# linkedin/gdmix

Hardware: AMD Instinct MI355X
Metric: random-effect entities converged/sec (higher is better)
Workload: dtype f64; 1 GPU; C2: synthetic 1000000 entities/GPU x avg 64 nnz (n~max(1,Poisson(16)), k=4 distinct uniform columns of D=1024, SURVEY 8(d) generator), per-entity L2 LR, L-BFGS m=10; build_id=8021e6e25780712a, workload_key=c2, entities_per_gpu=1000000, step=pack+solve, theta on device, parallelism=entity-shard x1

## Files before the change

gdmix_amd/csrc/re_api.hip:

```cpp
#include <stdarg.h>
#include <stdio.h>
#include <stdlib.h>
#include <string.h>
#include <time.h>

#include <errno.h>
#include <fcntl.h>
#include <sys/file.h>
#include <sys/stat.h>
#include <unistd.h>

#include <condition_variable>
#include <map>
#include <new>
#include <string>

#include <mutex>

#include "re_internal.hpp"
#include "re_solve_team.hpp"

namespace gdmix {

static thread_local char g_err[512] = "";

void set_error(const char* fmt, ...) {
  va_list ap;
  va_start(ap, fmt);
  vsnprintf(g_err, sizeof(g_err), fmt, ap);
  va_end(ap);
}

bool loss_code_ok(int code, const char* who) {
  if (code == GDMIX_RE_LOSS_LOGISTIC || code == GDMIX_RE_LOSS_SQUARED || code == GDMIX_RE_LOSS_POISSON) return true;
  set_error("%s: opts->loss = %d is no loss code (GDMIX_RE_LOSS_LOGISTIC 0, GDMIX_RE_LOSS_SQUARED 1, GDMIX_RE_LOSS_POISSON 2)", who, code);
  return false;
}

__global__ __launch_bounds__(WAVE) void publish_kernel(const uint32_t* __restrict__ src, int words, uint32_t* box_data, uint32_t* box_flag, uint32_t seq) {
  for (int i = threadIdx.x; i < words; i += WAVE) __hip_atomic_store(box_data + i, src[i], __ATOMIC_RELAXED, __HIP_MEMORY_SCOPE_SYSTEM);
  asm volatile("s_waitcnt vmcnt(0)" ::: "memory");
  if (threadIdx.x == 0) __hip_atomic_store(box_flag, seq, __ATOMIC_RELAXED, __HIP_MEMORY_SCOPE_SYSTEM);
}

static inline void cpu_relax() {
#if !defined(__HIP_DEVICE_COMPILE__)
  asm volatile("pause" ::: "memory");
#endif
}

static int mailbox_on() {
  static const int on = [] { const char* e = getenv("GDMIX_RE_MAILBOX"); return (e && atoi(e) == 0) ? 0 : 1; }();
  return on;
}

hipError_t post_small(gdmix_ctx_impl* ctx, int box, const void* dev_src, size_t bytes, void* host_dst, hipStream_t s, SmallFetch* f) {
  f->box = -1; f->seq = 0; f->bytes = bytes; f->host_dst = host_dst; f->s = s;
  if (!mailbox_on() || bytes % 4 || bytes > MAILBOX_BYTES - MAILBOX_DATA || box < 0 || box >= 4)
    return hipMemcpyAsync(host_dst, dev_src, bytes, hipMemcpyDeviceToHost, s);
  char* const base = reinterpret_cast<char*>(ctx->host_pinned) + MAILBOX_OFFSET + (size_t)box * MAILBOX_BYTES;
  uint32_t seq = ++ctx->mail_seq[box];
  if (seq == 0) seq = ++ctx->mail_seq[box];
  hipLaunchKernelGGL(publish_kernel, dim3(1), dim3(WAVE), 0, s, static_cast<const uint32_t*>(dev_src), (int)(bytes / 4),
                     reinterpret_cast<uint32_t*>(base + MAILBOX_DATA), reinterpret_cast<uint32_t*>(base), seq);
  f->box = box; f->seq = seq;
  return hipGetLastError();
}

hipError_t wait_small(gdmix_ctx_impl* ctx, const SmallFetch& f) {
  if (f.box < 0) return hipStreamSynchronize(f.s);
  char* const base = reinterpret_cast<char*>(ctx->host_pinned) + MAILBOX_OFFSET + (size_t)f.box * MAILBOX_BYTES;
  uint32_t* const flag = reinterpret_cast<uint32_t*>(base);
  timespec t0, t1;
  clock_gettime(CLOCK_MONOTONIC, &t0);
  while (__atomic_load_n(flag, __ATOMIC_ACQUIRE) != f.seq) {
    for (int k = 0; k < 16; ++k) cpu_relax();
    clock_gettime(CLOCK_MONOTONIC, &t1);
    if ((t1.tv_sec - t0.tv_sec) * 1000000L + (t1.tv_nsec - t0.tv_nsec) / 1000L > FETCH_SPIN_US) {
      hipError_t rc = hipStreamSynchronize(f.s);
      if (rc != hipSuccess) return rc;
      if (__atomic_load_n(flag, __ATOMIC_ACQUIRE) != f.seq) return hipErrorUnknown;
      break;
    }
  }
  memcpy(f.host_dst, base + MAILBOX_DATA, f.bytes);
  return hipSuccess;
}

}

using namespace gdmix;


namespace gdmix {
namespace {
constexpr int GATE_DEVICES = 64;
std::mutex g_gate_mu[GATE_DEVICES];
hipEvent_t g_gate_ev[GATE_DEVICES] = {};
bool g_gate_armed[GATE_DEVICES] = {};
}

class GridLock {
 public:
  explicit GridLock(const std::string& base) : base_(base) {}
  bool acquire() {
    std::unique_lock<std::mutex> g(mu_);
    if (!open_files()) return false;
    for (;;) {
      if (state_ == HELD) {
        if (!somebody_waits()) { ++count_; ++rides_; return true; }
        cv_.wait(g);
      } else if (state_ == ACQUIRING) {
        cv_.wait(g);
      } else {
        state_ = ACQUIRING;
        g.unlock();
        const bool ok = flock_retry(turn_fd_, LOCK_EX) && flock_retry(dev_fd_, LOCK_EX);
        flock_retry(turn_fd_, LOCK_UN);
        g.lock();
        if (!ok) { state_ = FREE; cv_.notify_all(); return false; }
        state_ = HELD;
        count_ = 1;
        ++takes_;
        cv_.notify_all();
        return true;
      }
    }
  }
  void release() {
    std::lock_guard<std::mutex> g(mu_);
    if (state_ != HELD || count_ <= 0) return;
    if (--count_ == 0) {
      flock_retry(dev_fd_, LOCK_UN);
      state_ = FREE;
      cv_.notify_all();
    }
  }
  void stats(long* takes, long* rides) {
    std::lock_guard<std::mutex> g(mu_);
    *takes = takes_;
    *rides = rides_;
  }

 private:
  enum State { FREE, ACQUIRING, HELD };
  static bool flock_retry(int fd, int op) {
    int rc;
    do rc = flock(fd, op); while (rc != 0 && errno == EINTR);
    return rc == 0;
  }
  static int open_one(const std::string& path) {
    const int fd = open(path.c_str(), O_RDWR | O_CREAT | O_CLOEXEC, 0666);
    if (fd >= 0) (void)fchmod(fd, 0666);
    return fd;
  }
  bool open_files() {
    if (dev_fd_ >= 0) return true;
    if (failed_) return false;
    dev_fd_ = open_one(base_ + ".lock");
    turn_fd_ = open_one(base_ + ".turn");
    probe_fd_ = open_one(base_ + ".turn");
    if (dev_fd_ < 0 || turn_fd_ < 0 || probe_fd_ < 0) {
      fprintf(stderr, "gdmix_re: cannot open %s.lock (%s): persistent grids of several processes on this device are not chained\n", base_.c_str(), strerror(errno));
      for (int* fd : {&dev_fd_, &turn_fd_, &probe_fd_}) { if (*fd >= 0) close(*fd); *fd = -1; }
      failed_ = true;
      return false;
    }
    return true;
  }
  bool somebody_waits() {
    if (flock(probe_fd_, LOCK_SH | LOCK_NB) == 0) { flock_retry(probe_fd_, LOCK_UN); return false; }
    return errno == EWOULDBLOCK;
  }
  std::string base_;
  std::mutex mu_;
  std::condition_variable cv_;
  State state_ = FREE;
  int count_ = 0, dev_fd_ = -1, turn_fd_ = -1, probe_fd_ = -1;
  bool failed_ = false;
  long takes_ = 0, rides_ = 0;
};

namespace {
std::mutex g_locks_mu;
std::map<std::string, GridLock*> g_locks;
GridLock* g_dev_lock[GATE_DEVICES] = {};
hipStream_t g_rel_stream[GATE_DEVICES] = {};
bool g_dev_lock_off[GATE_DEVICES] = {};

GridLock* grid_lock_by_key(const char* key) {
  std::lock_guard<std::mutex> g(g_locks_mu);
  auto it = g_locks.find(key);
  if (it != g_locks.end()) return it->second;
  const char* dir = getenv("GDMIX_RE_LOCK_DIR");
  std::string base = std::string(dir && *dir ? dir : "/tmp") + "/gdmix_re_grid_";
  for (const char* c = key; *c; ++c) base += (isalnum((unsigned char)*c) || *c == '.' || *c == '-') ? *c : '_';
  return g_locks[key] = new GridLock(base);
}

GridLock* grid_lock_of_device(int device) {
  if (g_dev_lock_off[device]) return nullptr;
  if (g_dev_lock[device]) return g_dev_lock[device];
  const char* e = getenv("GDMIX_RE_GRID_LOCK");
  char bus[64] = "";
  if ((e && atoi(e) == 0) || hipDeviceGetPCIBusId(bus, sizeof(bus), device) != hipSuccess || !bus[0] ||
      hipStreamCreateWithFlags(&g_rel_stream[device], hipStreamNonBlocking) != hipSuccess) {
    g_dev_lock_off[device] = true;
    return nullptr;
  }
  return g_dev_lock[device] = grid_lock_by_key(bus);
}

void grid_lock_release_cb(void* p) { static_cast<GridLock*>(p)->release(); }

std::mutex g_here_mu;
std::map<std::string, int> g_here_fd;

int presence_fd(int device) {
  char bus[64] = "";
  if (hipDeviceGetPCIBusId(bus, sizeof(bus), device) != hipSuccess || !bus[0]) return -1;
  std::lock_guard<std::mutex> g(g_here_mu);
  auto it = g_here_fd.find(bus);
  if (it != g_here_fd.end()) return it->second;
  const char* dir = getenv("GDMIX_RE_LOCK_DIR");
  std::string path = std::string(dir && *dir ? dir : "/tmp") + "/gdmix_re_grid_";
  for (const char* c = bus; *c; ++c) path += (isalnum((unsigned char)*c) || *c == '.' || *c == '-') ? *c : '_';
  path += ".here";
  const int fd = open(path.c_str(), O_RDWR | O_CREAT | O_CLOEXEC, 0666);
  if (fd >= 0) {
    (void)fchmod(fd, 0666);
    struct flock fl = {};
    fl.l_type = F_RDLCK; fl.l_whence = SEEK_SET; fl.l_start = 0; fl.l_len = 1;
    (void)fcntl(fd, F_SETLK, &fl);
  }
  return g_here_fd[bus] = fd;
}
}

void device_register_process(int device) {
  const char* e = getenv("GDMIX_RE_GRID_LOCK");
  if (!(e && atoi(e) == 0)) (void)presence_fd(device);
}

bool device_has_another_process(int device) {
  const char* e = getenv("GDMIX_RE_GRID_LOCK");
  if (e && atoi(e) == 0) return false;
  const int fd = presence_fd(device);
  if (fd < 0) return false;
  struct flock fl = {};
  fl.l_type = F_WRLCK; fl.l_whence = SEEK_SET; fl.l_start = 0; fl.l_len = 1;
  return fcntl(fd, F_GETLK, &fl) == 0 && fl.l_type != F_UNLCK;
}

ScopedGridGate::ScopedGridGate(int device, hipStream_t s) : device_(device >= 0 && device < GATE_DEVICES ? device : 0), s_(s), err_(hipSuccess), held_(nullptr) {
  g_gate_mu[device_].lock();
  if (!g_gate_ev[device_]) err_ = hipEventCreateWithFlags(&g_gate_ev[device_], hipEventDisableTiming);
  if (err_ == hipSuccess && g_gate_armed[device_]) err_ = hipStreamWaitEvent(s_, g_gate_ev[device_], 0);
  if (err_ == hipSuccess) {
    GridLock* const L = grid_lock_of_device(device_);
    if (L && L->acquire()) held_ = L;
  }
}

ScopedGridGate::~ScopedGridGate() {
  const bool recorded = g_gate_ev[device_] && hipEventRecord(g_gate_ev[device_], s_) == hipSuccess;
  if (recorded) g_gate_armed[device_] = true;
  if (held_) {
    GridLock* const L = static_cast<GridLock*>(held_);
    if (!(recorded && hipStreamWaitEvent(g_rel_stream[device_], g_gate_ev[device_], 0) == hipSuccess &&
          hipLaunchHostFunc(g_rel_stream[device_], grid_lock_release_cb, L) == hipSuccess)) {
      (void)hipStreamSynchronize(s_);
      L->release();
    }
  }
  g_gate_mu[device_].unlock();
}
}

extern "C" {

static int spread_default() {
  const char* e = getenv("GDMIX_RE_SPREAD");
  const int n = e ? atoi(e) : 4;
  return n > 1 ? n : 0;
}
GDMIX_API int gdmix_re_abi_version(void) { return GDMIX_RE_ABI_VERSION; }

GDMIX_API int gdmix_re_grid_lock_acquire(const char* key) {
  if (!key || !*key) { set_error("key is empty"); return GDMIX_RE_EINVAL; }
  return grid_lock_by_key(key)->acquire() ? GDMIX_RE_OK : GDMIX_RE_EINVAL;
}
GDMIX_API int gdmix_re_grid_lock_release(const char* key) {
  if (!key || !*key) { set_error("key is empty"); return GDMIX_RE_EINVAL; }
  grid_lock_by_key(key)->release();
  return GDMIX_RE_OK;
}
GDMIX_API int gdmix_re_grid_lock_stats(const char* key, int64_t* takes, int64_t* rides) {
  if (!key || !*key || !takes || !rides) { set_error("bad argument"); return GDMIX_RE_EINVAL; }
  long t = 0, r = 0;
  grid_lock_by_key(key)->stats(&t, &r);
  *takes = t;
  *rides = r;
  return GDMIX_RE_OK;
}

GDMIX_API const char* gdmix_re_last_error(void) { return g_err; }

GDMIX_API void gdmix_re_default_opts(gdmix_re_opts* o) {
  if (!o) return;
  o->l2 = 1.0; o->regularize_bias = 1; o->has_intercept = 1; o->m = 10; o->max_iter = 100;
  o->maxfun = 15000; o->maxls = 20; o->ftol = 1e-12; o->pgtol = 1e-5;
  o->variance_mode = GDMIX_RE_VAR_NONE; o->threshold = 1e-4;
  o->sum_loss = 0; o->loss = 0;
}

GDMIX_API int gdmix_re_create(int hip_device, gdmix_re_ctx** out) {
  if (!out) { set_error("out is NULL"); return GDMIX_RE_EINVAL; }
  *out = nullptr;
  int count = 0;
  HIP_TRY(hipGetDeviceCount(&count));
  if (hip_device < 0 || hip_device >= count) {
    set_error("HIP device %d not present (%d visible)", hip_device, count);
    return GDMIX_RE_EHIP;
  }
  HIP_TRY(hipSetDevice(hip_device));
  hipDeviceProp_t prop;
  HIP_TRY(hipGetDeviceProperties(&prop, hip_device));
  if (strncmp(prop.gcnArchName, "gfx950", 6) != 0) {
    set_error("device %d is %s; this library only carries gfx950 (MI355X) code", hip_device, prop.gcnArchName);
    return GDMIX_RE_EHIP;
  }
  gdmix_re_ctx* c = new (std::nothrow) gdmix_re_ctx();
  if (!c) { set_error("out of host memory"); return GDMIX_RE_ENOMEM; }
  c->impl.device = hip_device;
  c->impl.num_cus = prop.multiProcessorCount;
  device_register_process(hip_device);
  c->impl.tall_adapt_limit = c->impl.num_cus * 3 / 2;
  if (const char* e = getenv("GDMIX_RE_TALL_ADAPT")) c->impl.tall_adapt_limit = atoi(e) > 0 ? atoi(e) : 0;
  c->impl.scratch = nullptr;
  c->impl.scratch_bytes = 0;
  c->impl.host_pinned = nullptr;
  c->impl.wave_lds_limit = 65536;
  c->impl.kernel_mask = 7;
  c->impl.timing = 0;
  c->impl.giant_nnz = 16777216;
  c->impl.team_nnz = 16384;
  c->impl.tall_min_n = GDMIX_RE_TALL_MIN_N_DEFAULT;
  c->impl.tall_split_n = GDMIX_RE_TALL_SPLIT_N_DEFAULT;
  c->impl.tall_split_set = 0;
  c->impl.tall_team_n = GDMIX_RE_TALL_TEAM_N_DEFAULT;
  c->impl.tall_team_limit = c->impl.num_cus / 4 < TALL_TEAM_MAX ? c->impl.num_cus / 4 : TALL_TEAM_MAX;
  c->impl.tall_mid_n = 0;
  if (const char* e = getenv("GDMIX_RE_TALL_MID")) { if (atoi(e) == 1) c->impl.tall_mid_n = -(c->impl.num_cus * TALL_MID_WGS); else if (atoi(e) > 1) c->impl.tall_mid_n = -atoi(e); }
  if (c->impl.num_cus < 8 * TALL_TEAM_C) c->impl.tall_team_n = 0;
  if (const char* e = getenv("GDMIX_RE_TALL_TEAM")) { if (atoi(e) == 0) c->impl.tall_team_n = 0; }
  if (const char* e = getenv("GDMIX_RE_TALL_TEAM_LIMIT")) { if (atoi(e) > 0 && atoi(e) <= TALL_TEAM_MAX) c->impl.tall_team_limit = atoi(e); }
  c->impl.spread = spread_default();
  c->impl.narrow = 1;
  if (const char* e = getenv("GDMIX_RE_NARROW")) c->impl.narrow = atoi(e) != 0 ? 1 : 0;
  c->impl.grid_sync = nullptr;
  c->impl.big_tmp = nullptr;
  c->impl.big_tmp_bytes = 0;
  c->impl.eval_small_set = 0; c->impl.eval_small_max = 64;
  c->impl.eval_tmp = nullptr; c->impl.eval_tmp_bytes = 0;
  c->impl.sel_small_set = 0; c->impl.sel_small_max = 1024; c->impl.sel_plan_ws = nullptr;
  c->impl.cap_small_set = 0; c->impl.cap_small_max = 128; c->impl.cap_plan_ws = nullptr;
  c->impl.n_side = 0; c->impl.side_fork = nullptr;
  c->impl.aux_ev[0] = c->impl.aux_ev[1] = nullptr;
  c->impl.defer_unique = 0; c->impl.unique_pending = false; c->impl.unique_ev = nullptr;
  for (int k = 0; k < gdmix_ctx_impl::MAX_SIDE; ++k) { c->impl.side[k] = nullptr; c->impl.side_join[k] = nullptr; }
  for (int k = 0; k < GDMIX_RE_NUM_CLASSES; ++k) { c->impl.ev0[k] = nullptr; c->impl.ev1[k] = nullptr; c->impl.ev_used[k] = false; }
  for (uint32_t& q : c->impl.mail_seq) q = 0;
  hipError_t rc = hipHostMalloc(reinterpret_cast<void**>(&c->impl.host_pinned), HOST_PINNED_BYTES, hipHostMallocMapped | hipHostMallocCoherent);
  if (rc == hipSuccess) memset(c->impl.host_pinned, 0, HOST_PINNED_BYTES);
  if (rc != hipSuccess) {
    set_error("hipHostMalloc failed: %s", hipGetErrorString(rc));
    delete c;
    return GDMIX_RE_EHIP;
  }
  {
    const char* e = getenv("GDMIX_RE_SIDE_STREAM");
    int want = e ? atoi(e) : 3;
    if (want > gdmix_ctx_impl::MAX_SIDE) want = gdmix_ctx_impl::MAX_SIDE;
    if (want > 0) {
      rc = hipEventCreateWithFlags(&c->impl.side_fork, hipEventDisableTiming);
      for (int k = 0; k < 2 && rc == hipSuccess; ++k) rc = hipEventCreateWithFlags(&c->impl.aux_ev[k], hipEventDisableTiming);
      if (rc == hipSuccess) rc = hipEventCreateWithFlags(&c->impl.unique_ev, hipEventDisableTiming);
      for (int k = 0; k < want && rc == hipSuccess; ++k) {
        rc = hipStreamCreateWithFlags(&c->impl.side[k], hipStreamNonBlocking);
        if (rc == hipSuccess) rc = hipEventCreateWithFlags(&c->impl.side_join[k], hipEventDisableTiming);
        if (rc == hipSuccess) c->impl.n_side = k + 1;
      }
      if (rc != hipSuccess) {
        set_error("creating the side streams failed: %s", hipGetErrorString(rc));
        gdmix_re_destroy(c);
        return GDMIX_RE_EHIP;
      }
    }
  }
  rc = hipMalloc(&c->impl.grid_sync, GridSyncLayout::BYTES);
  if (rc != hipSuccess) {
    set_error("hipMalloc failed: %s", hipGetErrorString(rc));
    (void)hipHostFree(c->impl.host_pinned);
    delete c;
    return GDMIX_RE_EHIP;
  }
  *out = c;
  return GDMIX_RE_OK;
}

GDMIX_API void gdmix_re_destroy(gdmix_re_ctx* ctx) {
  if (!ctx) return;
  if (ctx->impl.unique_pending && ctx->impl.unique_ev) (void)hipEventSynchronize(ctx->impl.unique_ev);
  if (ctx->impl.unique_ev) (void)hipEventDestroy(ctx->impl.unique_ev);
  if (ctx->impl.grid_sync) (void)hipFree(ctx->impl.grid_sync);
  if (ctx->impl.big_tmp) (void)hipFree(ctx->impl.big_tmp);
  if (ctx->impl.eval_tmp) (void)hipFree(ctx->impl.eval_tmp);
  if (ctx->impl.host_pinned) (void)hipHostFree(ctx->impl.host_pinned);
  if (ctx->impl.side_fork) (void)hipEventDestroy(ctx->impl.side_fork);
  for (int k = 0; k < 2; ++k) if (ctx->impl.aux_ev[k]) (void)hipEventDestroy(ctx->impl.aux_ev[k]);
  for (int k = 0; k < gdmix_ctx_impl::MAX_SIDE; ++k) {
    if (ctx->impl.side_join[k]) (void)hipEventDestroy(ctx->impl.side_join[k]);
    if (ctx->impl.side[k]) (void)hipStreamDestroy(ctx->impl.side[k]);
  }
  for (int k = 0; k < GDMIX_RE_NUM_CLASSES; ++k) {
    if (ctx->impl.ev0[k]) (void)hipEventDestroy(ctx->impl.ev0[k]);
    if (ctx->impl.ev1[k]) (void)hipEventDestroy(ctx->impl.ev1[k]);
  }
  delete ctx;
}

GDMIX_API size_t gdmix_re_pack_workspace_bytes(int64_t E, int64_t N, int64_t Z) {
  if (E < 0 || N < 0 || Z < 0) return 0;
  return pack_workspace_bytes(E, N, Z);
}

GDMIX_API int gdmix_re_pack(gdmix_re_ctx* ctx, const gdmix_re_raw_batch* raw_dev, int has_intercept, void* workspace,
                  size_t workspace_bytes, gdmix_re_packed* out, void* stream) {
  if (!ctx || !raw_dev || !out || (!workspace && workspace_bytes)) { set_error("NULL argument"); return GDMIX_RE_EINVAL; }
  if (raw_dev->E > 0 && (!raw_dev->ent_row_ptr || !raw_dev->row_nnz_ptr || !raw_dev->y || !raw_dev->offset)) {
    set_error("raw batch has NULL arrays");
    return GDMIX_RE_EINVAL;
  }
  if (raw_dev->Z > 0 && (!raw_dev->col_global || !raw_dev->val)) { set_error("raw batch has NULL arrays"); return GDMIX_RE_EINVAL; }
  HIP_TRY(hipSetDevice(ctx->impl.device));
  HIP_TRY(join_unique(&ctx->impl, static_cast<hipStream_t>(stream)));
  return pack_impl(&ctx->impl, raw_dev, has_intercept, workspace, workspace_bytes, out, static_cast<hipStream_t>(stream));
}

GDMIX_API int gdmix_re_set_defer_unique(gdmix_re_ctx* ctx, int enabled) {
  if (!ctx) { set_error("ctx is NULL"); return GDMIX_RE_EINVAL; }
  ctx->impl.defer_unique = (enabled && ctx->impl.n_side > 0) ? 1 : 0;
  return GDMIX_RE_OK;
}

GDMIX_API int gdmix_re_pack_join(gdmix_re_ctx* ctx, void* stream) {
  if (!ctx) { set_error("ctx is NULL"); return GDMIX_RE_EINVAL; }
  HIP_TRY(hipSetDevice(ctx->impl.device));
  HIP_TRY(join_unique(&ctx->impl, static_cast<hipStream_t>(stream)));
  return GDMIX_RE_OK;
}

static int slots_for(const gdmix_re_packed* b, const gdmix_re_opts* o, size_t* slot_doubles) {
  *slot_doubles = block_slot_doubles(b->max_p, b->max_n, o->m);
  size_t bytes = *slot_doubles * 8;
  size_t by_budget = ((size_t)4 << 30) / (bytes ? bytes : 1);
  size_t slots = 1024;
  if (slots > by_budget) slots = by_budget;
  if (slots < 8) slots = 8;
  if ((int64_t)slots > b->E) slots = (size_t)(b->E > 0 ? b->E : 1);
  return (int)slots;
}

static int64_t var_small_p(const gdmix_re_packed* b) { return b->max_p < VAR_FULL_MAX_P ? b->max_p : VAR_FULL_MAX_P; }

static int var_slots_for(const gdmix_re_packed* b) {
  size_t bytes = var_full_slot_doubles(var_small_p(b)) * 8;
  size_t slots = ((size_t)2 << 30) / (bytes ? bytes : 1);
  if (slots > 2048) slots = 2048;
  if (slots < 4) slots = 4;
  slots &= ~(size_t)3;
  return (int)slots;
}

GDMIX_API size_t gdmix_re_solve_scratch_bytes(const gdmix_re_packed* batch, const gdmix_re_opts* opts) {
  if (!batch || !opts || batch->E == 0) return 0;
  size_t slot_doubles;
  int slots = slots_for(batch, opts, &slot_doubles);
  size_t need = (size_t)slots * slot_doubles * 8;
  if (opts->variance_mode == GDMIX_RE_VAR_FULL && batch->max_p <= VAR_FULL_BIG_MAX_P) {
    size_t v = (size_t)var_slots_for(batch) * var_full_slot_doubles(var_small_p(batch)) * 8;
    if (v > need) need = v;
    if (batch->max_p > VAR_FULL_MAX_P) {
      v = var_full_big_doubles(batch->max_p, batch->max_n) * 8;
      if (v > need) need = v;
    }
  }
  return need;
}

GDMIX_API int gdmix_re_set_wave_lds_limit(gdmix_re_ctx* ctx, int bytes) {
  if (!ctx || bytes < 0) { set_error("bad argument"); return GDMIX_RE_EINVAL; }
  ctx->impl.wave_lds_limit = bytes > 65536 ? 65536 : bytes;
  return GDMIX_RE_OK;
}

GDMIX_API int gdmix_re_set_kernel_mask(gdmix_re_ctx* ctx, int mask) {
  if (!ctx) { set_error("ctx is NULL"); return GDMIX_RE_EINVAL; }
  ctx->impl.kernel_mask = mask & 7;
  return GDMIX_RE_OK;
}

GDMIX_API int gdmix_re_set_giant_nnz(gdmix_re_ctx* ctx, int64_t nnz) {
  if (!ctx || nnz < 0) { set_error("bad argument"); return GDMIX_RE_EINVAL; }
  ctx->impl.giant_nnz = nnz;
  return GDMIX_RE_OK;
}

GDMIX_API int gdmix_re_set_team_nnz(gdmix_re_ctx* ctx, int64_t nnz) {
  if (!ctx || nnz < 0) { set_error("bad argument"); return GDMIX_RE_EINVAL; }
  ctx->impl.team_nnz = nnz;
  return GDMIX_RE_OK;
}

GDMIX_API int gdmix_re_set_tall_min_n(gdmix_re_ctx* ctx, int min_n) {
  if (!ctx || min_n < 0) { set_error("bad argument"); return GDMIX_RE_EINVAL; }
  ctx->impl.tall_min_n = min_n;
  return GDMIX_RE_OK;
}

GDMIX_API int gdmix_re_set_spread(gdmix_re_ctx* ctx, int queues) {
  if (!ctx || queues < 0) { set_error("bad argument"); return GDMIX_RE_EINVAL; }
  ctx->impl.spread = queues > 1 ? queues : 0;
  return GDMIX_RE_OK;
}

GDMIX_API int gdmix_re_set_narrow(gdmix_re_ctx* ctx, int on) {
  if (!ctx) { set_error("ctx is NULL"); return GDMIX_RE_EINVAL; }
  ctx->impl.narrow = on ? 1 : 0;
  return GDMIX_RE_OK;
}

GDMIX_API int gdmix_re_set_tall_team_n(gdmix_re_ctx* ctx, int team_n) {
  if (!ctx) { set_error("bad argument"); return GDMIX_RE_EINVAL; }
  ctx->impl.tall_team_n = ctx->impl.num_cus < 8 * TALL_TEAM_C ? 0 : team_n;
  return GDMIX_RE_OK;
}

GDMIX_API int gdmix_re_device_shared(gdmix_re_ctx* ctx) {
  if (!ctx) { set_error("ctx is NULL"); return GDMIX_RE_EINVAL; }
  return device_has_another_process(ctx->impl.device) ? 1 : 0;
}

GDMIX_API int gdmix_re_set_tall_mid_n(gdmix_re_ctx* ctx, int mid_n) {
  if (!ctx) { set_error("bad argument"); return GDMIX_RE_EINVAL; }
  ctx->impl.tall_mid_n = mid_n < 0 ? -(ctx->impl.num_cus * TALL_MID_WGS) : mid_n;
  return GDMIX_RE_OK;
}

GDMIX_API int gdmix_re_set_tall_split_n(gdmix_re_ctx* ctx, int split_n) {
  if (!ctx || split_n < 0) { set_error("bad argument"); return GDMIX_RE_EINVAL; }
  ctx->impl.tall_split_n = split_n > 0 ? split_n : GDMIX_RE_TALL_SPLIT_N_DEFAULT;
  ctx->impl.tall_split_set = split_n > 0 ? 1 : 0;
  return GDMIX_RE_OK;
}

GDMIX_API int gdmix_re_set_timing(gdmix_re_ctx* ctx, int enabled) {
  if (!ctx) { set_error("ctx is NULL"); return GDMIX_RE_EINVAL; }
  if (enabled && !ctx->impl.ev0[0]) {
    HIP_TRY(hipSetDevice(ctx->impl.device));
    for (int k = 0; k < GDMIX_RE_NUM_CLASSES; ++k) {
      HIP_TRY(hipEventCreate(&ctx->impl.ev0[k]));
      HIP_TRY(hipEventCreate(&ctx->impl.ev1[k]));
    }
  }
  ctx->impl.timing = enabled ? 1 : 0;
  return GDMIX_RE_OK;
}

GDMIX_API int gdmix_re_last_solve_ms(gdmix_re_ctx* ctx, float* ms_out) {
  if (!ctx || !ms_out) { set_error("NULL argument"); return GDMIX_RE_EINVAL; }
  for (int k = 0; k < GDMIX_RE_NUM_CLASSES; ++k) {
    ms_out[k] = 0.0f;
    if (ctx->impl.ev_used[k]) {
      HIP_TRY(hipEventSynchronize(ctx->impl.ev1[k]));
      HIP_TRY(hipEventElapsedTime(&ms_out[k], ctx->impl.ev0[k], ctx->impl.ev1[k]));
    }
  }
  return GDMIX_RE_OK;
}

GDMIX_API int gdmix_re_set_scratch(gdmix_re_ctx* ctx, void* scratch, size_t bytes) {
  if (!ctx) { set_error("ctx is NULL"); return GDMIX_RE_EINVAL; }
  ctx->impl.scratch = scratch;
  ctx->impl.scratch_bytes = bytes;
  return GDMIX_RE_OK;
}

static int run_variance_full(gdmix_re_ctx* ctx, const gdmix_re_packed* b, const BatchDev& B, const SolveParams& P, const double* theta,
                             double* variance, hipStream_t s) {
  const size_t vslot = var_full_slot_doubles(var_small_p(b));
  int vslots = var_slots_for(b);
  size_t avail = ctx->impl.scratch ? ctx->impl.scratch_bytes : 0;
  void* base = ctx->impl.scratch;
  if (b->scratch_bytes > avail) { avail = b->scratch_bytes; base = b->scratch; }
  if ((size_t)vslots * vslot * 8 > avail) vslots = (int)(avail / (vslot * 8)) & ~3;
  if (vslots < 4) {
    set_error("variance_mode FULL needs >= %zu bytes of scratch (gdmix_re_set_scratch)", 4 * vslot * 8);
    return GDMIX_RE_ENOMEM;
  }
  HIP_TRY(launch_variance_full(B, b->E, P, theta, variance, static_cast<double*>(base), vslot, vslots, var_small_p(b), s));
  if (b->max_p > VAR_FULL_MAX_P) {
    if (var_full_big_doubles(b->max_p, b->max_n) * 8 > avail) {
      set_error("variance_mode FULL with p = %d needs >= %zu bytes of scratch (gdmix_re_set_scratch)", b->max_p,
                var_full_big_doubles(b->max_p, b->max_n) * 8);
      return GDMIX_RE_ENOMEM;
    }
    HIP_TRY(launch_variance_full_big(&ctx->impl, B, b->E, P, theta, variance, static_cast<double*>(base), b->max_p, b->max_n, s));
  }
  return GDMIX_RE_OK;
}

}

namespace {

struct Slots { double* scratch = nullptr; size_t doubles = 0; int n = 0; };

int size_slots(const gdmix_ctx_impl* ci, const gdmix_re_packed* b, const gdmix_re_opts* opts, int n_slot_users, Slots* out) {
  if (n_slot_users <= 0) return GDMIX_RE_OK;
  out->n = slots_for(b, opts, &out->doubles);
  const size_t need = (size_t)out->n * out->doubles * 8;
  if (ci->scratch && ci->scratch_bytes >= need) out->scratch = static_cast<double*>(ci->scratch);
  else if (b->scratch && b->scratch_bytes >= need) out->scratch = static_cast<double*>(b->scratch);
  else {
    size_t avail = ci->scratch ? ci->scratch_bytes : 0;
    void* base = ci->scratch;
    if (b->scratch_bytes > avail) { avail = b->scratch_bytes; base = b->scratch; }
    out->n = (int)(avail / (out->doubles * 8));
    if (out->n < 1) {
      set_error("%d entities need a scratch slot: provide >= %zu bytes via gdmix_re_set_scratch", n_slot_users, out->doubles * 8);
      return GDMIX_RE_ENOMEM;
    }
    out->scratch = static_cast<double*>(base);
  }
  return GDMIX_RE_OK;
}

template <class F>
int timed(gdmix_ctx_impl* ci, int c, hipStream_t s, F&& launch) {
  if (ci->timing) HIP_TRY(hipEventRecord(ci->ev0[c], s));
  const hipError_t rc = launch();
  if (rc != hipSuccess) { set_error("launch of class %d (%s) failed: %s", c, kClasses[c].name, hipGetErrorString(rc)); return GDMIX_RE_EHIP; }
  if (ci->timing) { HIP_TRY(hipEventRecord(ci->ev1[c], s)); ci->ev_used[c] = true; }
  return GDMIX_RE_OK;
}

hipError_t launch_class(const gdmix_ctx_impl* ci, const gdmix_re_packed* b, const BatchDev& B, const OutDev& O, const SolveParams& P,
                        const double* theta0, const Launch& L, int lean_merged, hipStream_t s) {
  const ClassDesc& d = kClasses[L.c];
  switch (d.kind) {
    case KIND_WLDS:
      return launch_solve_wave(B, O, P, theta0, L.begin, L.count, d.lds, s);
    case KIND_TALL_T: {
      const char* xe = getenv("GDMIX_RE_XCD_BARRIER");
      return launch_solve_tall_team(B, O, P, theta0, L.begin, L.count, ci->num_cus, b->Z, GridSyncLayout::tall_tail(ci, d.tall_variant),
                                    GridSyncLayout::tall_team_buf(ci), (xe && atoi(xe) == 0) ? 0 : 1, s);
    }
    case KIND_TALL_L: case KIND_TALL_S: case KIND_TALL_M: case KIND_TALL:
      return launch_solve_tall(d.tall_variant, B, O, P, theta0, L.begin, L.count, ci->num_cus, b->Z, GridSyncLayout::tall_tail(ci, d.tall_variant),
                               GridSyncLayout::tall_ticket(ci, d.tall_variant), d.kind == KIND_TALL_S ? lean_merged : 0, s);
    default: {
      if (d.lanes <= 0) return hipErrorInvalidValue;
      const int nn = (L.c == NARROW_HOST_CLASS && L.narrow > 0) ? (L.narrow < L.count ? L.narrow : L.count) : 0;
      if (hipError_t rc = launch_solve_quad(NARROW_LANES, NARROW_EPL, B, O, P, theta0, L.begin, nn, NARROW_NCAP, NARROW_ZCAP, s); rc != hipSuccess) return rc;
      return launch_solve_quad(d.lanes, d.epl, B, O, P, theta0, L.begin + nn, L.count - nn, d.ncap, d.zcap, s);
    }
  }
}

int team_count(int tier_max, unsigned long long total_nnz, unsigned long long largest_nnz, int entities, int slots, int num_cus) {
  const unsigned long long ratio = largest_nnz ? total_nnz / largest_nnz : 1;
  int teams = 1;
  while (teams * 2 <= tier_max && (unsigned long long)(teams * 2) <= ratio) teams *= 2;
  if (entities <= 16) {
    int want = 1;
    while (want * 2 <= entities && want * 2 <= tier_max && want * 2 <= teams * 4) want *= 2;
    if (want > teams) teams = want;
  }
  if (const char* ev = getenv("GDMIX_RE_TEAMS")) teams = atoi(ev);
  if (teams > TEAM_MAX_TEAMS) teams = TEAM_MAX_TEAMS;
  while (teams > 1 && (slots < teams || num_cus % teams)) teams >>= 1;
// ... 153 lines not shown
```

gdmix_amd/csrc/re_internal.hpp:

```cpp
#pragma once
#include <hip/hip_runtime.h>
#include <stdint.h>
#include <stddef.h>

#include <type_traits>

#include "../../include/gdmix_re.h"
#include "re_solve_core.hpp"
#include "re_solve_wreg.hpp"
#include "re_solve_quad.hpp"

namespace gdmix {

enum { KIND_WREG1 = 0, KIND_WREG2 = 1, KIND_WREG4 = 2, KIND_WLDS = 3, KIND_BLOCK = 4, KIND_QUAD2 = 5, KIND_QUAD4 = 6, KIND_PAIR4 = 7, KIND_QUAD3 = 8, KIND_PAIR3 = 9, KIND_WREG8 = 10,
       KIND_G64_3 = 11, KIND_G64_4 = 12, KIND_G128_4 = 13, KIND_G256_4 = 14, KIND_G512_4 = 15, KIND_GRID = 16, KIND_G128_3 = 17, KIND_G256_3 = 18,
       KIND_TALL = 20, KIND_TALL_S = 21, KIND_TALL_L = 22, KIND_TALL_T = 23, KIND_TALL_M = 24 };

__host__ __device__ constexpr int group_lanes(int kind) {
  return (kind == KIND_QUAD2 || kind == KIND_QUAD3 || kind == KIND_QUAD4) ? 16 : ((kind == KIND_PAIR3 || kind == KIND_PAIR4) ? 32 :
         ((kind == KIND_G64_3 || kind == KIND_G64_4) ? 64 : ((kind == KIND_G128_4 || kind == KIND_G128_3) ? 128 : ((kind == KIND_G256_4 || kind == KIND_G256_3) ? 256 : (kind == KIND_G512_4 ? 512 : 0)))));
}
__host__ __device__ constexpr int group_epl(int kind) {
  return kind == KIND_QUAD2 ? 2 : ((kind == KIND_QUAD3 || kind == KIND_PAIR3 || kind == KIND_G64_3 || kind == KIND_G128_3 || kind == KIND_G256_3) ? 3 : (group_lanes(kind) > 0 ? 4 : 0));
}
// ... 59 lines not shown
    grp_class(KIND_G128_4, 128, 4, 128, 1024, "re_solve_grp_kernel<128,4> n<=128 nnz<=1024"),
    grp_class(KIND_G128_4, 128, 4, 1024, 3072, "re_solve_grp_kernel<128,4> n<=1024 nnz<=3072"),
    grp_class(KIND_G256_3, 256, 3, 256, 2048, "re_solve_grp_kernel<256,3> n<=256 nnz<=2048"),
    grp_class(KIND_G256_3, 256, 3, 2048, 4096, "re_solve_grp_kernel<256,3> n<=2048 nnz<=4096"),
    grp_class(KIND_G256_4, 256, 4, 256, 2048, "re_solve_grp_kernel<256,4> n<=256 nnz<=2048"),
    grp_class(KIND_G256_4, 256, 4, 2048, 4096, "re_solve_grp_kernel<256,4> n<=2048 nnz<=4096"),
    grp_class(KIND_G512_4, 512, 4, 512, 4096, "re_solve_grp_kernel<512,4> n<=512 nnz<=4096"),
    wave_class(24576, "re_solve_wave_kernel lds<=24K"),
    wave_class(65536, "re_solve_wave_kernel lds<=64K"),
    tall_class(KIND_TALL_T, TALL_VARIANT_TEAM, 0, 0, 0, "re_solve_tall_team_kernel<8> x4 p<=64"),
    tall_class(KIND_TALL_L, TALL_VARIANT_LEAN, 4, WAVE, 0, "re_solve_tall_kernel<1> lean p<=64"),
    tall_class(KIND_TALL_S, TALL_VARIANT_SMALL, 3, WAVE, 2, "re_solve_tall_kernel<1> p<=64"),
    tall_class(KIND_TALL_M, TALL_VARIANT_MID, 2, 8 / TALL_MID_WGS * WAVE, -1, "re_solve_tall_kernel<4> p<=64"),
    tall_class(KIND_TALL, TALL_VARIANT_LARGE, 1, 4 * TALL_NW / 8 * WAVE, 1, "re_solve_tall_kernel<8> p<=64"),
    team_class(KIND_BLOCK, "re_solve_team_kernel workgroup"),
    team_class(KIND_GRID, "re_solve_team_kernel 128 teams"),
    team_class(KIND_GRID, "re_solve_team_kernel 32 teams"),
    team_class(KIND_GRID, "re_solve_team_kernel 8 teams"),
    team_class(KIND_GRID, "re_solve_team_kernel device-wide")};
constexpr int class_of_kind(int kind) {
  for (int c = 0; c < GDMIX_RE_NUM_CLASSES; ++c)
    if (kClasses[c].kind == kind) return c;
  return -1;
}
constexpr int TALL_T_CLASS = class_of_kind(KIND_TALL_T);
constexpr int TALL_L_CLASS = class_of_kind(KIND_TALL_L);
constexpr int TALL_S_CLASS = class_of_kind(KIND_TALL_S);
constexpr int TALL_M_CLASS = class_of_kind(KIND_TALL_M);
constexpr int TALL_CLASS = class_of_kind(KIND_TALL);
constexpr int BLOCK_CLASS = class_of_kind(KIND_BLOCK);
constexpr int TEAM128_CLASS = BLOCK_CLASS + 1;
constexpr int TEAM32_CLASS = BLOCK_CLASS + 2;
constexpr int TEAM8_CLASS = BLOCK_CLASS + 3;
constexpr int GIANT_CLASS = BLOCK_CLASS + 4;
constexpr int tall_class_of_rank(int rank) {
  for (int c = 0; c < GDMIX_RE_NUM_CLASSES; ++c)
    if (kClasses[c].tall_rank == rank) return c;
  return -1;
}
constexpr bool class_table_consistent() {
  for (int k = 0; k < TALL_VARIANTS; ++k)
    if (tall_class_of_rank(k) < 0) return false;

  for (int c = 0; c < GDMIX_RE_NUM_CLASSES; ++c) {
    const ClassDesc& d = kClasses[c];
    if (d.lanes != group_lanes(d.kind) || d.epl != group_epl(d.kind)) return false;
    if ((d.tall_variant >= 0) != (c >= TALL_T_CLASS && c < BLOCK_CLASS) || (d.tall_variant >= 0) != (d.tall_rank >= 0)) return false;
    if (c > BLOCK_CLASS && d.kind != KIND_GRID) return false;
    if (c < TALL_T_CLASS && d.lds <= 0) return false;
  }
  return true;
}
static_assert(class_table_consistent(), "group_lanes / group_epl and the class constants describe kClasses");
static_assert(GIANT_CLASS == GDMIX_RE_NUM_CLASSES - 1 && BLOCK_CLASS - TALL_T_CLASS == TALL_VARIANTS, "the tall classes, the block class, three tiers and the giant class end the table");
static_assert(TALL_L_CLASS + 1 == TALL_S_CLASS, "a merged lean class sits right in front of the one-wavefront class in `order`");
constexpr int NARROW_HOST_CLASS = 9;
static_assert(kClasses[NARROW_HOST_CLASS].kind == KIND_PAIR3 && kClasses[NARROW_HOST_CLASS].ncap == 32 && kClasses[NARROW_HOST_CLASS].zcap == 128 &&
              class_of_kind(KIND_PAIR3) == NARROW_HOST_CLASS, "the narrow kernel takes its entities from <32,3> n<=32 nnz<=128");
constexpr int NARROW_LANES = 16, NARROW_EPL = 5, NARROW_NCAP = 24, NARROW_ZCAP = 96;
constexpr int NARROW_FLAG = 0x100;
static_assert(NARROW_FLAG > GDMIX_RE_NUM_CLASSES, "the mark is no class index");
__host__ __device__ constexpr bool narrow_fits(int p, int n, int z) { return p <= NARROW_LANES * NARROW_EPL && n <= NARROW_NCAP && z <= NARROW_ZCAP; }
constexpr int BLOCK_NW = 4;
#ifndef GDMIX_TEAM_BLOCK_NW
#define GDMIX_TEAM_BLOCK_NW 8
#endif
constexpr int TEAM_BLOCK_NW = GDMIX_TEAM_BLOCK_NW;
constexpr int TEAM_GRID_NW = 8;

struct ClassTable {
  int kind[GDMIX_RE_NUM_CLASSES];
  int lds_bytes[GDMIX_RE_NUM_CLASSES];
  int ncap[GDMIX_RE_NUM_CLASSES];
  int zcap[GDMIX_RE_NUM_CLASSES];
  int64_t giant_nnz;
  int64_t team_nnz;
  int tall_min_n;
  int tall_split_n;
  int tall_adapt_limit;
  int tall_team_n;
  int tall_team_limit;
  int narrow;
  int tall_mid_n;
};
constexpr int TALL_ADAPT_STEPS = 3;
__host__ __device__ constexpr int tall_adapt_n(int k) { return k == 0 ? 512 : (k == 1 ? 1024 : 2048); }
constexpr int TALL_TEAM_STEPS = 3;
constexpr int TALL_MID_STEPS = 6;
__host__ __device__ constexpr int tall_mid_step(int k) { return k == 0 ? 256 : (k == 1 ? 384 : (k == 2 ? 512 : (k == 3 ? 768 : (k == 4 ? 1024 : 1536)))); }
struct TallRouting {
  int32_t tall_ge[TALL_ADAPT_STEPS];
  int32_t split;
  int32_t team_ge[TALL_TEAM_STEPS];
  int32_t team_from;
  int32_t mid_ge[TALL_MID_STEPS];
  int32_t mid_from;
};
struct ClassCounts {
  int32_t count[GDMIX_RE_NUM_CLASSES];
  int32_t base[GDMIX_RE_NUM_CLASSES];
  int32_t cursor[GDMIX_RE_NUM_CLASSES];
  TallRouting tall;
  int32_t narrow_count;
  int32_t row3_free[TEAM128_CLASS - 1 - (int)(sizeof(TallRouting) / sizeof(int32_t))];
  int32_t team_largest_nnz[GDMIX_RE_NUM_CLASSES - TEAM128_CLASS];
  unsigned long long team_nnz_total[GDMIX_RE_NUM_CLASSES];
  __host__ __device__ int32_t& largest_nnz(int c) { return team_largest_nnz[c - TEAM128_CLASS]; }
  __host__ __device__ const int32_t& largest_nnz(int c) const { return team_largest_nnz[c - TEAM128_CLASS]; }
};
static_assert(sizeof(ClassCounts) == 6 * GDMIX_RE_NUM_CLASSES * sizeof(int32_t), "gdmix_re_packed::class_count is documented as [6*NUM_CLASSES]");
static_assert(offsetof(ClassCounts, count) == 0 && offsetof(ClassCounts, base) == 1 * GDMIX_RE_NUM_CLASSES * sizeof(int32_t) &&
              offsetof(ClassCounts, cursor) == 2 * GDMIX_RE_NUM_CLASSES * sizeof(int32_t) && offsetof(ClassCounts, tall) == 3 * GDMIX_RE_NUM_CLASSES * sizeof(int32_t) &&
              offsetof(ClassCounts, team_largest_nnz) == (3 * GDMIX_RE_NUM_CLASSES + TEAM128_CLASS) * sizeof(int32_t) &&
              offsetof(ClassCounts, team_nnz_total) == 4 * GDMIX_RE_NUM_CLASSES * sizeof(int32_t), "the rows of the count record");
static_assert(offsetof(TallRouting, mid_from) / sizeof(int32_t) < (size_t)TEAM128_CLASS, "row 3: the last threshold slot stays below the team tiers' columns");
static_assert(offsetof(ClassCounts, narrow_count) == (3 * GDMIX_RE_NUM_CLASSES + GDMIX_RE_NARROW_COUNT_WORD) * sizeof(int32_t) && GDMIX_RE_NARROW_COUNT_WORD < TEAM128_CLASS,
              "row 3: the narrow count sits where include/gdmix_re.h says, below the team tiers' columns");

struct BatchDev {
  const int64_t* ent_row_ptr;
  const int64_t* ent_nnz_ptr;
  const int64_t* ent_feat_ptr;
  const int32_t* row_ptr;
  const int32_t* csr_col;
  const float* csr_val;
  const int32_t* col_ptr;
  const int32_t* csc_row;
  const float* csc_val;
  const float* y;
  const float* offset;
  const float* weight;
  const int32_t* order;
};
inline BatchDev batch_dev(const gdmix_re_packed* b) {
  BatchDev B;
  B.ent_row_ptr = b->ent_row_ptr; B.ent_nnz_ptr = b->ent_nnz_ptr; B.ent_feat_ptr = b->ent_feat_ptr;
  B.row_ptr = b->row_ptr; B.csr_col = b->csr_col; B.csr_val = b->csr_val;
  B.col_ptr = b->col_ptr; B.csc_row = b->csc_row; B.csc_val = b->csc_val;
  B.y = b->y; B.offset = b->offset; B.weight = b->weight; B.order = b->order;
  return B;
}

struct OutDev {
  double* theta;
  double* theta_thr;
  double* variance;
  double* fval;
  double* gnorm;
  int32_t* nit;
  int32_t* nfev;
  int32_t* status;
};

struct gdmix_ctx_impl {
  int device;
  int num_cus;
  void* scratch;
  size_t scratch_bytes;
  int32_t* host_pinned;
  uint32_t mail_seq[4];
  int wave_lds_limit;
  int kernel_mask;
  int timing;
  int64_t giant_nnz;
  int64_t team_nnz;
  int tall_min_n;
  int tall_split_n;
  int tall_adapt_limit;
  int tall_split_set;
  int tall_team_n;
  int tall_team_limit;
  int tall_mid_n;
  int narrow;
  int spread;
  void* grid_sync;
  void* big_tmp;
  size_t big_tmp_bytes;
  static constexpr int MAX_SIDE = 4;
  hipStream_t side[MAX_SIDE];
  int n_side;
  hipEvent_t side_fork, side_join[MAX_SIDE];
  hipEvent_t aux_ev[2];
  int defer_unique;
  bool unique_pending;
  hipEvent_t unique_ev;
  hipEvent_t ev0[GDMIX_RE_NUM_CLASSES], ev1[GDMIX_RE_NUM_CLASSES];
  bool ev_used[GDMIX_RE_NUM_CLASSES];
  int eval_small_set, eval_small_max;
  void* eval_tmp;
  size_t eval_tmp_bytes;
  const void* ds_plan_ws;
  int64_t ds_plan_rows, ds_plan_kept, ds_plan_nnz;
  int sel_small_set, sel_small_max;
  const void* sel_plan_ws;
  int64_t sel_plan_E, sel_plan_N, sel_plan_Z, sel_plan_D, sel_plan_nnz;
  int cap_small_set, cap_small_max;
  const void* cap_plan_ws;
  int64_t cap_plan_rows, cap_plan_entities, cap_plan_bound, cap_plan_kept, cap_plan_nnz;
};

constexpr size_t HOST_PINNED_BYTES = 8192;
constexpr size_t MAILBOX_OFFSET = 4096, MAILBOX_BYTES = 1024, MAILBOX_DATA = 64;
constexpr int FETCH_SPIN_US = 400;
constexpr size_t COUNTS_READBACK_WORDS = 256;
static_assert(sizeof(ClassCounts) <= MAILBOX_BYTES - MAILBOX_DATA, "a larger count record falls back to copy + synchronise in post_small");
static_assert(COUNTS_READBACK_WORDS * sizeof(int32_t) + sizeof(ClassCounts) <= MAILBOX_OFFSET, "the read-back areas end where the mailboxes begin");
struct SmallFetch { int box; uint32_t seq; size_t bytes; void* host_dst; hipStream_t s; };
hipError_t post_small(gdmix_ctx_impl* ctx, int box, const void* dev_src, size_t bytes, void* host_dst, hipStream_t s, SmallFetch* f);
hipError_t wait_small(gdmix_ctx_impl* ctx, const SmallFetch& f);
inline hipError_t fetch_small(gdmix_ctx_impl* ctx, int box, const void* dev_src, size_t bytes, void* host_dst, hipStream_t s) {
  SmallFetch f;
  hipError_t rc = post_small(ctx, box, dev_src, bytes, host_dst, s, &f);
  return rc != hipSuccess ? rc : wait_small(ctx, f);
}

}

struct gdmix_re_ctx {
  gdmix::gdmix_ctx_impl impl;
};

namespace gdmix {

__host__ __device__ inline size_t wave_lds_bytes(int p, int n, int nnz, int d, int m, bool has_w) {
  size_t dbl = (size_t)(5 + 2 * m) * p + n + 2 * m;
  size_t w32 = (size_t)4 * nnz + (n + 1) + (d + 1) + (has_w ? 3 : 2) * (size_t)n;
  return ((dbl * 8 + w32 * 4) + 15) & ~(size_t)15;
}

inline size_t block_slot_doubles(int64_t max_p, int64_t max_n, int m) {
  return (size_t)5 * max_p + (size_t)2 * m * ((max_p + 63) & ~(int64_t)63) + max_n + 2 * m + 8 + 256 * 64;
}

struct SideJoin {
  gdmix_ctx_impl* ci; hipStream_t main; unsigned used = 0;
  hipError_t use(int k) {
    if (used & (1u << k)) return hipSuccess;
    const hipError_t rc = hipStreamWaitEvent(ci->side[k], ci->side_fork, 0);
    if (rc == hipSuccess) used |= 1u << k;
    return rc;
  }
  void join() {
    for (int k = 0; k < ci->n_side; ++k) {
      if (!(used & (1u << k))) continue;
      if (hipEventRecord(ci->side_join[k], ci->side[k]) != hipSuccess || hipStreamWaitEvent(main, ci->side_join[k], 0) != hipSuccess)
        (void)hipStreamSynchronize(ci->side[k]);
    }
    used = 0;
  }
  ~SideJoin() { join(); }
};

int make_class_table(const gdmix_ctx_impl* ci, const gdmix_re_opts* opts, ClassTable* out);
int route(gdmix_ctx_impl* ci, const gdmix_re_packed* b, const ClassTable& tab, const gdmix_re_opts* opts, hipStream_t s, const ClassCounts** host);
struct Launch { int c, begin, count, stream, narrow; };
struct LaunchPlan {
  Launch launch[GDMIX_RE_NUM_CLASSES];
  int n;
  int lean_merged;
  bool fork;
};
LaunchPlan plan_launches(const ClassCounts& counts, int num_cus, int n_side, int spread, int lean_rounds);
hipError_t launch_solve_quad(int g, int epl, const BatchDev& B, const OutDev& O, const SolveParams& o, const double* theta0,
                             int begin, int count, int ncap, int zcap, hipStream_t s);
hipError_t launch_solve_wave(const BatchDev& B, const OutDev& O, const SolveParams& o, const double* theta0,
                             int begin, int count, int lds_bytes, hipStream_t s);
hipError_t launch_solve_block(const BatchDev& B, const OutDev& O, const SolveParams& o, const double* theta0,
                              int begin, int count, double* scratch, size_t slot_doubles, int slots,
                              int64_t max_p, hipStream_t s);
hipError_t launch_solve_grid(const BatchDev& B, const OutDev& O, const SolveParams& o, const double* theta0,
                             int begin, int count, double* scratch, size_t slot_doubles, int64_t max_p,
                             void* sync_buf, int blocks, int teams, hipStream_t s);
constexpr int TALL_TAIL_BYTES = 256;
hipError_t launch_solve_tall(int variant, const BatchDev& B, const OutDev& O, const SolveParams& o, const double* theta0, int begin, int count,
                             int num_cus, int64_t Z, void* tail_buf, unsigned* ticket, int front_small, hipStream_t s);
hipError_t launch_solve_tall_team(const BatchDev& B, const OutDev& O, const SolveParams& o, const double* theta0, int begin, int count,
                                  int num_cus, int64_t Z, void* tail_buf, void* team_buf, int xcd_fast, hipStream_t s);
void launch_sort_class(int32_t* list, int count, const int64_t* ent_nnz_ptr, hipStream_t s);
static_assert(LOSS_LOGISTIC == GDMIX_RE_LOSS_LOGISTIC && LOSS_SQUARED == GDMIX_RE_LOSS_SQUARED && LOSS_POISSON == GDMIX_RE_LOSS_POISSON,
              "the device's loss codes are the header's");
bool loss_code_ok(int code, const char* who);
template <class F>
inline hipError_t with_loss(int code, F&& f) {
  switch (code) {
    case LOSS_LOGISTIC: return f(std::integral_constant<int, LOSS_LOGISTIC>{});
    case LOSS_SQUARED: return f(std::integral_constant<int, LOSS_SQUARED>{});
    case LOSS_POISSON: return f(std::integral_constant<int, LOSS_POISSON>{});
    default: return hipErrorInvalidValue;
  }
}
template <class F>
inline void with_flag(bool flag, F&& f) {
  if (flag) f(std::bool_constant<true>{});
  else f(std::bool_constant<false>{});
}
inline int grid_for(int64_t count, int per_block, int cap) {
  const int64_t g = (count + per_block - 1) / per_block;
  return g > cap ? cap : (g < 1 ? 1 : (int)g);
}
inline SolveParams solve_params(const gdmix_re_opts& o) {
  SolveParams P;
  P.l2 = o.l2; P.ftol = o.ftol; P.pgtol = o.pgtol; P.threshold = o.threshold;
  P.regularize_bias = o.regularize_bias; P.has_intercept = o.has_intercept ? 1 : 0; P.m = o.m; P.max_iter = o.max_iter;
  P.maxfun = o.maxfun; P.maxls = o.maxls; P.variance_mode = o.variance_mode;
  P.sum_loss = o.sum_loss ? 1 : 0; P.loss = o.loss;
  return P;
}
inline SolveParams fe_solve_params(const gdmix_re_opts& o) {
  SolveParams P = solve_params(o);
  P.threshold = 0.0; P.variance_mode = 0; P.sum_loss = 1;
  return P;
}

template <bool PINNED>
class HipBuf {
 public:
  HipBuf() = default;
  HipBuf(HipBuf&& o) noexcept : p_(o.release()) {}
  HipBuf& operator=(HipBuf&& o) noexcept {
    if (this != &o) { reset(); p_ = o.release(); }
    return *this;
  }
  HipBuf(const HipBuf&) = delete;
  HipBuf& operator=(const HipBuf&) = delete;
  ~HipBuf() { reset(); }
  hipError_t alloc(size_t bytes) {
    reset();
    const hipError_t rc = PINNED ? hipHostMalloc(&p_, bytes, hipHostMallocDefault) : hipMalloc(&p_, bytes);
    if (rc != hipSuccess) p_ = nullptr;
    return rc;
  }
  void* get() const { return p_; }
  template <class T>
  T* as(size_t byte_offset = 0) const { return reinterpret_cast<T*>(static_cast<char*>(p_) + byte_offset); }
  explicit operator bool() const { return p_ != nullptr; }
  void* release() { void* p = p_; p_ = nullptr; return p; }
  void reset() {
    if (p_) (void)(PINNED ? hipHostFree(p_) : hipFree(p_));
    p_ = nullptr;
  }
 private:
  void* p_ = nullptr;
};
using DevBuf = HipBuf<false>;
using PinnedBuf = HipBuf<true>;

hipError_t launch_variance_simple(const BatchDev& B, const SolveParams& o, const double* theta, double* variance, int begin, int count,
                                  double* scratch, size_t slot_doubles, int slots, hipStream_t s);
hipError_t launch_variance_full(const BatchDev& B, int64_t E, const SolveParams& o, const double* theta, double* variance,
                                double* scratch, size_t slot_doubles, int slots, int64_t max_p, hipStream_t s);
constexpr int64_t VAR_FULL_MAX_P = 2048;
constexpr int64_t VAR_FULL_BIG_MAX_P = 16384;
constexpr int VAR_BIG_BUILD_GROUPS = 128;
size_t var_full_big_doubles(int64_t max_p, int64_t max_n);
hipError_t launch_variance_full_big(gdmix_ctx_impl* ci, const BatchDev& B, int64_t E, const SolveParams& o, const double* theta,
                                    double* variance, double* scratch, int64_t max_p, int64_t max_n, hipStream_t s);
size_t hessian_dense_scratch_doubles(int64_t n);
hipError_t launch_hessian_dense(gdmix_ctx_impl* ci, const BatchDev& B, int64_t n, int64_t d, int ic, const double* theta, double* H, int64_t ld,
                                double* scratch, hipStream_t s, int loss = LOSS_LOGISTIC);
hipError_t launch_variance_of_hessian(gdmix_ctx_impl* ci, double* H, double* M, int64_t p, int64_t ld, double l2, int64_t unreg, double* variance,
                                      hipStream_t s);
inline size_t var_full_slot_doubles(int64_t max_p) { return (size_t)2 * max_p * max_p + max_p + 8; }
hipError_t launch_score(const BatchDev& B, int64_t E, int64_t N, int ic, const double* theta, const uint8_t* has_model,
                        float* logit, float* per_coord, hipStream_t s);

inline hipError_t join_unique(gdmix_ctx_impl* ci, hipStream_t s) {
  if (!ci->unique_pending) return hipSuccess;
  const hipError_t q = hipEventQuery(ci->unique_ev);
  if (q == hipSuccess) { ci->unique_pending = false; return hipSuccess; }
  if (q != hipErrorNotReady) return q;
  return hipStreamWaitEvent(s, ci->unique_ev, 0);
}

size_t pack_workspace_bytes(int64_t E, int64_t N, int64_t Z);
int pack_impl(gdmix_ctx_impl* ctx, const gdmix_re_raw_batch* raw, int has_intercept, void* ws, size_t ws_bytes,
              gdmix_re_packed* out, hipStream_t s);
struct BigPackArgs {
  const int64_t* ent_row_ptr;
  const int64_t* ent_nnz_ptr;
  const int64_t* row_nnz_ptr;
  const int64_t* col_global;
  const float* val;
  int ic;
  int32_t* row_ptr;
  int32_t* csr_col;
  int32_t* col_ptr;
  int32_t* csc_row;
  float* csc_val;
  int32_t* uniq_sparse;
  int32_t* d_cnt;
  const int32_t* big_list;
  int n_big;
  int64_t big_nnz;
  int* max_p;
  int* err;
};
int pack_big_entities(gdmix_ctx_impl* ctx, const BigPackArgs& a, hipStream_t s, hipStream_t aux);

hipError_t launch_partition_ids(const int64_t* ids, int64_t count, int32_t num_partitions, int32_t* out,
                                hipStream_t s);

void set_error(const char* fmt, ...);
int eval_tmp(gdmix_ctx_impl* ci, size_t bytes, hipStream_t s, void** out);

#define HIP_TRY(expr)                                                                        \
  do {                                                                                       \
    hipError_t _rc = (expr);                                                                 \
// ... 36 lines not shown
```

gdmix_amd/csrc/re_owlqn.hip:

```cpp
#include <math.h>

#include "re_internal.hpp"
#include "re_owlqn.hpp"

namespace gdmix {

__host__ __device__ inline size_t owlqn_lds_bytes(int p, int n, int nnz, int d, int m, bool has_w) {
  return (wave_lds_bytes(p, n, nnz, d, m, has_w) + (size_t)(OWL_P_VECTORS - 5) * 8 * p + 15) & ~(size_t)15;
}

inline size_t owlqn_slot_doubles(int64_t max_p, int64_t max_n, int m) {
  return (size_t)(OWL_P_VECTORS + 2 * m) * max_p + (size_t)2 * m + max_n + 8;
}

static int owlqn_slots_for(const gdmix_re_packed* b, const gdmix_re_opts* o, size_t* slot_doubles) {
  *slot_doubles = owlqn_slot_doubles(b->max_p, b->max_n, o->m);
  const size_t bytes = *slot_doubles * 8;
  size_t slots = 1024;
  const size_t by_budget = ((size_t)4 << 30) / (bytes ? bytes : 1);
  if (slots > by_budget) slots = by_budget;
  if (slots < 8) slots = 8;
  if ((int64_t)slots > b->E) slots = (size_t)(b->E > 0 ? b->E : 1);
  return (int)slots;
}
// ... 73 lines not shown
  W.x = dp; dp += p;
  W.g = dp; dp += p;
  W.pg = dp; dp += p;
  W.d = dp; dp += p;
  W.xt = dp; dp += p;
  W.gt = dp; dp += p;
  W.ws = dp; dp += (size_t)m * p;
  W.wy = dp; dp += (size_t)m * p;
  W.rs = dp; dp += n;
  W.alpha = dp; dp += m;
  W.rho = dp; dp += m;
  float* fp = reinterpret_cast<float*>(dp);
  float* s_csr_val = fp; fp += nnz;
  float* s_csc_val = fp; fp += nnz;
  float* s_y = fp; fp += n;
  float* s_o = fp; fp += n;
  float* s_w = nullptr;
  if (B.weight) { s_w = fp; fp += n; }
  int32_t* ip = reinterpret_cast<int32_t*>(fp);
  int32_t* s_csr_col = ip; ip += nnz;
  int32_t* s_csc_row = ip; ip += nnz;
  int32_t* s_row_ptr = ip; ip += n + 1;
  int32_t* s_col_ptr = ip; ip += d + 1;

  for (int k = lane; k < nnz; k += WAVE) {
    s_csr_val[k] = B.csr_val[z0 + k];
    s_csr_col[k] = B.csr_col[z0 + k];
    s_csc_val[k] = B.csc_val[z0 + k];
    s_csc_row[k] = B.csc_row[z0 + k];
  }
  for (int i = lane; i < n; i += WAVE) {
    s_y[i] = B.y[r0 + i];
    s_o[i] = B.offset[r0 + i];
    if (s_w) s_w[i] = B.weight[r0 + i];
  }
  for (int i = lane; i <= n; i += WAVE) s_row_ptr[i] = B.row_ptr[r0 + e + i];
  for (int i = lane; i <= d; i += WAVE) s_col_ptr[i] = B.col_ptr[z0 + e + i];
  for (int j = lane; j < p; j += WAVE) W.xt[j] = theta0 ? theta0[c0 + j] : 0.0;

  WaveGroup grp{lane};
  grp.sync();
  EntityView P{n, d, p, ic, s_row_ptr, s_csr_col, s_csr_val, s_col_ptr, s_csc_row, s_csc_val, s_y, s_o, s_w};
  SolveStats st;
  owlqn_solve<LOSS>(grp, P, o, l1, W, st);
  owlqn_write_results(grp, O, o, e, c0, p, W.x, st);
  if (o.variance_mode == GDMIX_RE_VAR_SIMPLE && O.variance) {
    Work V{};
    V.x = W.x; V.rs = W.rs;
    variance_simple<false, LOSS>(grp, P, o, V, O.variance + c0);
  }
}

template <int LOSS>
__global__ __launch_bounds__(WAVE* BLOCK_NW) void re_owlqn_block_kernel(BatchDev B, OutDev O, SolveParams o, double l1, const double* __restrict__ theta0,
                                                                         int64_t last, int count, double* scratch, size_t slot_doubles, int64_t max_p) {
  __shared__ double red[2 * BLOCK_NW];
  const int ic = o.has_intercept ? 1 : 0;
  const int m = o.m;
  double* slot = scratch + (size_t)blockIdx.x * slot_doubles;
  for (int idx = blockIdx.x; idx < count; idx += gridDim.x) {
    const int64_t e = B.order[last - idx];
    const int64_t r0 = B.ent_row_ptr[e], z0 = B.ent_nnz_ptr[e], f0 = B.ent_feat_ptr[e];
    const int n = (int)(B.ent_row_ptr[e + 1] - r0);
    const int d = (int)(B.ent_feat_ptr[e + 1] - f0);
    const int p = d + ic;
    const int64_t c0 = f0 + e * ic;
    double* dp = slot;
    OwlWork W;
    W.x = dp; dp += max_p;
    W.g = dp; dp += max_p;
    W.pg = dp; dp += max_p;
    W.d = dp; dp += max_p;
    W.xt = dp; dp += max_p;
    W.gt = dp; dp += max_p;
    W.ws = dp; dp += (size_t)m * max_p;
    W.wy = dp; dp += (size_t)m * max_p;
    W.alpha = dp; dp += m;
    W.rho = dp; dp += m;
    W.rs = dp;
    BlockGroup<BLOCK_NW> grp{(int)threadIdx.x, red, 0};
    for (int j = grp.tid; j < p; j += grp.NT) W.xt[j] = theta0 ? theta0[c0 + j] : 0.0;
    grp.sync();
    EntityView P{n, d, p, ic, B.row_ptr + r0 + e, B.csr_col + z0, B.csr_val + z0, B.col_ptr + z0 + e,
                 B.csc_row + z0, B.csc_val + z0, B.y + r0, B.offset + r0, B.weight ? B.weight + r0 : nullptr};
    SolveStats st;
    owlqn_solve<LOSS>(grp, P, o, l1, W, st);
    owlqn_write_results(grp, O, o, e, c0, p, W.x, st);
    if (o.variance_mode == GDMIX_RE_VAR_SIMPLE && O.variance) {
      Work V{};
      V.x = W.x; V.rs = W.rs;
      variance_simple<false, LOSS>(grp, P, o, V, O.variance + c0);
    }
    grp.sync();
  }
}

static hipError_t launch_owlqn_wave(const BatchDev& B, const OutDev& O, const SolveParams& o, double l1, const double* theta0, const int32_t* list, int count,
                                    int lds_bytes, hipStream_t s) {
  if (count <= 0) return hipSuccess;
  return with_loss(o.loss, [&](auto L) {
    constexpr int LOSS = decltype(L)::value;
    static DynLdsOnce lds_attr;
    if (hipError_t rc = lds_attr.set(reinterpret_cast<const void*>(re_owlqn_wave_kernel<LOSS>)); rc != hipSuccess) return rc;
    hipLaunchKernelGGL(re_owlqn_wave_kernel<LOSS>, dim3(count), dim3(WAVE), (size_t)lds_bytes, s, B, O, o, l1, theta0, list, count);
    return hipGetLastError();
  });
}

static hipError_t launch_owlqn_block(const BatchDev& B, const OutDev& O, const SolveParams& o, double l1, const double* theta0, int64_t last, int count,
                                     double* scratch, size_t slot_doubles, int slots, int64_t max_p, hipStream_t s) {
  if (count <= 0) return hipSuccess;
  const int grid = count < slots ? count : slots;
  return with_loss(o.loss, [&](auto L) {
    hipLaunchKernelGGL(re_owlqn_block_kernel<decltype(L)::value>, dim3(grid), dim3(WAVE * BLOCK_NW), 0, s, B, O, o, l1, theta0, last, count, scratch,
                       slot_doubles, max_p);
    return hipGetLastError();
  });
}

}

using namespace gdmix;

extern "C" {

GDMIX_API size_t gdmix_re_solve_l1_scratch_bytes(const gdmix_re_packed* batch, const gdmix_re_opts* opts) {
  if (!batch || !opts || batch->E == 0) return 0;
  size_t slot_doubles;
  const int slots = owlqn_slots_for(batch, opts, &slot_doubles);
  const size_t own = (size_t)slots * slot_doubles * 8;
  const size_t plain = gdmix_re_solve_scratch_bytes(batch, opts);
  return own > plain ? own : plain;
}

GDMIX_API int gdmix_re_solve_l1(gdmix_re_ctx* ctx, const gdmix_re_packed* b, const gdmix_re_opts* opts, double l1, const double* theta0,
                                const gdmix_re_result* out, void* stream) {
  if (!ctx || !b || !opts || !out) { set_error("NULL argument"); return GDMIX_RE_EINVAL; }
  if (!(l1 >= 0.0) || isinf(l1)) { set_error("gdmix_re_solve_l1: l1 must be finite and >= 0"); return GDMIX_RE_EINVAL; }
  if (l1 == 0.0) return gdmix_re_solve(ctx, b, opts, theta0, out, stream);
  if (opts->sum_loss) { set_error("gdmix_re_solve_l1: sum_loss is the fixed effect's objective (gdmix_fe_set_l1 is its elastic net)"); return GDMIX_RE_EINVAL; }
  if (opts->m < 1 || opts->max_iter < 0 || opts->maxls < 1) { set_error("bad solver options (m, max_iter, maxls)"); return GDMIX_RE_EINVAL; }
  if (!loss_code_ok(opts->loss, "gdmix_re_solve_l1")) return GDMIX_RE_EINVAL;
  if (opts->variance_mode == GDMIX_RE_VAR_FULL && !out->theta) { set_error("variance_mode FULL needs out->theta"); return GDMIX_RE_EINVAL; }
  if (opts->variance_mode != GDMIX_RE_VAR_NONE && !out->variance) { set_error("variance requested but out->variance is NULL"); return GDMIX_RE_EINVAL; }
  if (b->E == 0) return GDMIX_RE_OK;
  if (b->E > 0x7fffffffLL) { set_error("gdmix_re_solve_l1: 2^31 entities or more"); return GDMIX_RE_ERANGE; }
  gdmix_ctx_impl* const ci = &ctx->impl;
  hipStream_t const s = static_cast<hipStream_t>(stream);
  HIP_TRY(hipSetDevice(ci->device));
  for (int c = 0; c < GDMIX_RE_NUM_CLASSES; ++c) ci->ev_used[c] = false;

  const int ic = opts->has_intercept ? 1 : 0;
  int32_t* const counts = b->class_count;
  const int small_lds = ci->wave_lds_limit < OWL_SMALL_LDS ? ci->wave_lds_limit : OWL_SMALL_LDS;
  HIP_TRY(hipMemsetAsync(counts, 0, sizeof(ClassCounts), s));
  hipLaunchKernelGGL(re_owlqn_route_kernel, dim3(grid_for(b->E, 256, 2048)), dim3(256), 0, s, b->ent_row_ptr, b->ent_nnz_ptr, b->ent_feat_ptr, b->E, ic,
                     opts->m, b->weight != nullptr, ci->wave_lds_limit, small_lds, b->order, b->cls_tmp, counts);
  HIP_TRY(hipGetLastError());
  int32_t* const hc = ci->host_pinned + COUNTS_READBACK_WORDS;
  HIP_TRY(fetch_small(ci, 0, counts, OWL_COUNT_WORDS * sizeof(int32_t), hc, s));
  const int n_wave = hc[OWL_COUNT_WAVE], n_block = hc[OWL_COUNT_BLOCK], wave_lds = hc[OWL_MAX_WAVE_LDS];
  const int n_small = hc[OWL_COUNT_WAVE_SMALL], n_large = hc[OWL_COUNT_WAVE_LARGE];
  if (n_small < 0 || n_large < 0 || n_block < 0 || n_small + n_large != n_wave || (int64_t)n_wave + n_block != b->E || wave_lds < 0 || wave_lds > 65536) {
    set_error("gdmix_re_solve_l1: the routing counted %d + %d of %lld entities (LDS %d)", n_wave, n_block, (long long)b->E, wave_lds);
    return GDMIX_RE_EHIP;
  }

  SolveParams P = solve_params(*opts);
  P.sum_loss = 0;
  const BatchDev B = batch_dev(b);
  const OutDev O{out->theta, out->theta_thr, opts->variance_mode == GDMIX_RE_VAR_SIMPLE ? out->variance : nullptr, out->fval, out->gnorm, out->nit,
                 out->nfev, out->status};

  double* scratch = nullptr;
  size_t slot_doubles = 0;
  int slots = 0;
  if (n_block > 0) {
    slots = owlqn_slots_for(b, opts, &slot_doubles);
    size_t avail = ci->scratch ? ci->scratch_bytes : 0;
    void* base = ci->scratch;
    if (b->scratch_bytes > avail) { avail = b->scratch_bytes; base = b->scratch; }
    if ((size_t)slots * slot_doubles * 8 > avail) slots = (int)(avail / (slot_doubles * 8));
    if (slots < 1) {
      set_error("%d entities need a scratch slot: provide >= %zu bytes via gdmix_re_set_scratch", n_block, slot_doubles * 8);
      return GDMIX_RE_ENOMEM;
    }
    scratch = static_cast<double*>(base);
  }

  {
    SideJoin side_join{ci, s};
    hipStream_t q[3] = {s, s, s};
    const int live = (n_block > 0) + (n_large > 0) + (n_small > 0);
    if (live > 1 && ci->n_side > 0) {
      HIP_TRY(hipEventRecord(ci->side_fork, s));
      int k = 0;
      if (n_block > 0) { HIP_TRY(side_join.use(k)); q[0] = ci->side[k]; k = k + 1 < ci->n_side ? k + 1 : k; }
      if (n_large > 0 && n_small > 0) { HIP_TRY(side_join.use(k)); q[1] = ci->side[k]; }
    }
    hipError_t rc = launch_owlqn_block(B, O, P, l1, theta0, b->E - 1, n_block, scratch, slot_doubles, slots, b->max_p, q[0]);
    if (rc != hipSuccess) { set_error("launch of re_owlqn_block_kernel failed: %s", hipGetErrorString(rc)); return GDMIX_RE_EHIP; }
    rc = launch_owlqn_wave(B, O, P, l1, theta0, b->order, n_large, wave_lds, q[1]);
    if (rc == hipSuccess) rc = launch_owlqn_wave(B, O, P, l1, theta0, b->cls_tmp, n_small, small_lds, q[2]);
    if (rc != hipSuccess) { set_error("launch of re_owlqn_wave_kernel failed: %s", hipGetErrorString(rc)); return GDMIX_RE_EHIP; }
  }
  if (opts->variance_mode == GDMIX_RE_VAR_FULL) {
    const int rc = gdmix_re_variance_full(ctx, b, opts, out->theta, out->variance, stream);
    if (rc != GDMIX_RE_OK) return rc;
  }
  HIP_TRY(join_unique(ci, s));
  return GDMIX_RE_OK;
}

}
```

gdmix_amd/csrc/re_pack.hip:

```cpp
#include <stdarg.h>
#include <stdio.h>
#include <stdlib.h>

#include "re_internal.hpp"

namespace gdmix {

constexpr int PACK_WAVES = 4;
#ifndef GDMIX_PACK_LDS_KEYS
#define GDMIX_PACK_LDS_KEYS 256
#endif
constexpr int PACK_LDS_KEYS = GDMIX_PACK_LDS_KEYS;

struct PackStats {
  unsigned long long D;
  int max_p, max_n, max_nnz, err;
  int n_big, n_mid;
  unsigned long long big_nnz;
  int n_mid2, pad;
};

constexpr int64_t PACK_FAN_MAX_ENTITIES = 1 << 18;
constexpr int PACK_CAP1 = PACK_LDS_KEYS, PACK_CAP2 = 512, PACK_CAP3 = 1024;
__device__ __forceinline__ unsigned long long wave_sum_u64(unsigned long long v) {
// ... 545 lines not shown
        for (int l = lane + WAVE; l < d[q]; l += WAVE) unique_global[f0[q] + l] = uniq_sparse[z0[q] + l];
      }
    }
  }
}

constexpr int SCAN_CHUNK = 2048;

__global__ __launch_bounds__(256) void scan_reduce_kernel(const int32_t* __restrict__ in, int64_t count,
                                                          long long* __restrict__ block_sums) {
  __shared__ long long part[4];
  const int64_t base = (int64_t)blockIdx.x * SCAN_CHUNK;
  long long s = 0;
  for (int k = threadIdx.x; k < SCAN_CHUNK; k += 256) {
    const int64_t i = base + k;
    if (i < count) s += in[i];
  }
  double sd = wave_sum((double)s);
  if ((threadIdx.x & 63) == 0) part[threadIdx.x >> 6] = (long long)sd;
  __syncthreads();
  if (threadIdx.x == 0) block_sums[blockIdx.x] = part[0] + part[1] + part[2] + part[3];
}

__global__ __launch_bounds__(1024) void scan_blocksums_kernel(long long* __restrict__ block_sums, int nb, PackStats* __restrict__ stats) {
  __shared__ long long tsum[1024];
  const int tid = threadIdx.x;
  const int per = (nb + 1023) / 1024;
  const int b0 = tid * per, b1 = (b0 + per < nb) ? b0 + per : nb;
  long long mine = 0;
  for (int b = b0; b < b1; ++b) mine += block_sums[b];
  tsum[tid] = mine;
  __syncthreads();
  for (int off = 1; off < 1024; off <<= 1) {
    const long long v = (tid >= off) ? tsum[tid - off] : 0;
    __syncthreads();
    tsum[tid] += v;
    __syncthreads();
  }
  long long run = tsum[tid] - mine;
  for (int b = b0; b < b1; ++b) { const long long v = block_sums[b]; block_sums[b] = run; run += v; }
  if (tid == 1023) stats->D = (unsigned long long)tsum[1023];
}

__global__ __launch_bounds__(256) void scan_apply_kernel(const int32_t* __restrict__ in, int64_t count,
                                                         const long long* __restrict__ block_sums,
                                                         int64_t* __restrict__ out ) {
  __shared__ long long tsum[256];
  const int64_t base = (int64_t)blockIdx.x * SCAN_CHUNK + (int64_t)threadIdx.x * 8;
  long long v[8], s = 0;
#pragma unroll
  for (int k = 0; k < 8; ++k) { v[k] = (base + k < count) ? in[base + k] : 0; s += v[k]; }
  tsum[threadIdx.x] = s;
  __syncthreads();
  for (int off = 1; off < 256; off <<= 1) {
    long long add = (threadIdx.x >= off) ? tsum[threadIdx.x - off] : 0;
    __syncthreads();
    tsum[threadIdx.x] += add;
    __syncthreads();
  }
  long long run = block_sums[blockIdx.x] + tsum[threadIdx.x] - s;
#pragma unroll
  for (int k = 0; k < 8; ++k) {
    if (base + k < count) out[base + k] = run;
    run += v[k];
    if (base + k == count - 1) out[count] = run;
  }
}

static size_t align_up(size_t x) { return (x + 255) & ~(size_t)255; }

struct PackLayout {
  size_t ent_nnz_ptr, ent_feat_ptr, row_ptr, csr_col, col_ptr, csc_row, csc_val, unique_global, order, cls_tmp,
      d_cnt, class_count, block_sums, stats, sort_key, uniq_sparse, big_list, mid_list, mid2_list, total;
};

static PackLayout pack_layout(int64_t E, int64_t N, int64_t Z) {
  PackLayout L;
  size_t off = 0;
  auto take = [&](size_t bytes) { size_t o = off; off = align_up(off + bytes); return o; };
  L.ent_nnz_ptr = take((size_t)(E + 1) * 8);
  L.ent_feat_ptr = take((size_t)(E + 1) * 8);
  L.row_ptr = take((size_t)(N + E + 1) * 4);
  L.csr_col = take((size_t)(Z + 1) * 4);
  L.col_ptr = take((size_t)(Z + E + 1) * 4);
  L.csc_row = take((size_t)(Z + 1) * 4);
  L.csc_val = take((size_t)(Z + 1) * 4);
  L.unique_global = take((size_t)(Z + 1) * 4);
  L.order = take((size_t)(E + 1) * 4);
  L.cls_tmp = take((size_t)(E + 1) * 4);
  L.d_cnt = take((size_t)(E + 1) * 4);
  L.class_count = take(sizeof(ClassCounts));
  L.block_sums = take((size_t)((E + 1) / SCAN_CHUNK + 2) * 8);
  L.stats = take(sizeof(PackStats));
  L.sort_key = take((size_t)(Z + 1) * 8);
  L.uniq_sparse = take((size_t)(Z + 1) * 4);
  L.big_list = take((size_t)(E + 1) * 4);
  L.mid_list = take((size_t)(E + 1) * 4);
  L.mid2_list = take((size_t)(E + 1) * 4);
  L.total = off;
  return L;
}

size_t pack_workspace_bytes(int64_t E, int64_t N, int64_t Z) { return pack_layout(E, N, Z).total; }

static bool debug_sync() {
  static int v = -1;
  if (v < 0) { const char* e = getenv("GDMIX_RE_DEBUG_SYNC"); v = (e && e[0] == '1') ? 1 : 0; }
  return v == 1;
}
#define DBG_STAGE(name)                                                        \
  do {                                                                         \
    if (debug_sync()) {                                                        \
      hipError_t _e = hipStreamSynchronize(s);                                 \
      fprintf(stderr, "[gdmix_re] %s: %s\n", name, hipGetErrorString(_e));     \
      fflush(stderr);                                                          \
    }                                                                          \
  } while (0)

static int pack_bitmap_on() {
  const char* e = getenv("GDMIX_PACK_BITMAP");
  return (e && atoi(e) == 0) ? 0 : 1;
}

int pack_impl(gdmix_ctx_impl* ctx, const gdmix_re_raw_batch* raw, int has_intercept, void* ws, size_t ws_bytes,
              gdmix_re_packed* out, hipStream_t s) {
  const int64_t E = raw->E, N = raw->N, Z = raw->Z;
  if (E < 0 || N < 0 || Z < 0) { set_error("negative batch dimension"); return GDMIX_RE_EINVAL; }
  if (E > 0x7ffffff0ll) { set_error("more than 2^31 entities in one batch"); return GDMIX_RE_ERANGE; }
  const PackLayout L = pack_layout(E, N, Z);
  if (ws_bytes < L.total) {
    set_error("pack workspace too small: %zu < %zu", ws_bytes, L.total);
    return GDMIX_RE_ENOMEM;
  }
  char* base = static_cast<char*>(ws);
  const int ic = has_intercept ? 1 : 0;
  out->E = E; out->N = N; out->Z = Z; out->D = 0;
  out->ent_row_ptr = raw->ent_row_ptr;
  out->ent_nnz_ptr = reinterpret_cast<int64_t*>(base + L.ent_nnz_ptr);
  out->ent_feat_ptr = reinterpret_cast<int64_t*>(base + L.ent_feat_ptr);
  out->row_ptr = reinterpret_cast<int32_t*>(base + L.row_ptr);
  out->csr_col = reinterpret_cast<int32_t*>(base + L.csr_col);
  out->csr_val = const_cast<float*>(raw->val);
  out->col_ptr = reinterpret_cast<int32_t*>(base + L.col_ptr);
  out->csc_row = reinterpret_cast<int32_t*>(base + L.csc_row);
  out->csc_val = reinterpret_cast<float*>(base + L.csc_val);
  out->unique_global = reinterpret_cast<int32_t*>(base + L.unique_global);
  out->y = raw->y; out->offset = raw->offset; out->weight = raw->weight;
  out->order = reinterpret_cast<int32_t*>(base + L.order);
  out->class_count = reinterpret_cast<int32_t*>(base + L.class_count);
  out->cls_tmp = reinterpret_cast<int32_t*>(base + L.cls_tmp);
  out->scratch = base + L.sort_key;
  out->scratch_bytes = (size_t)(Z + 1) * 8;
  out->max_p = ic; out->max_n = 0; out->max_nnz = 0;
  if (E == 0) return GDMIX_RE_OK;

  int32_t* d_cnt = reinterpret_cast<int32_t*>(base + L.d_cnt);
  long long* block_sums = reinterpret_cast<long long*>(base + L.block_sums);
  PackStats* stats = reinterpret_cast<PackStats*>(base + L.stats);
  unsigned long long* sort_key = reinterpret_cast<unsigned long long*>(base + L.sort_key);

  HIP_TRY(hipMemsetAsync(stats, 0, sizeof(PackStats), s));
  int32_t* uniq_sparse = reinterpret_cast<int32_t*>(base + L.uniq_sparse);
  int32_t* big_list = reinterpret_cast<int32_t*>(base + L.big_list);
  int32_t* mid_list = reinterpret_cast<int32_t*>(base + L.mid_list);
  int32_t* mid2_list = reinterpret_cast<int32_t*>(base + L.mid2_list);
  {
    int grid = (int)((E + 1 + ENTNNZ_THREADS - 1) / ENTNNZ_THREADS);
    if (grid > 1024) grid = 1024;
    hipLaunchKernelGGL(pack_entnnz_kernel, dim3(grid), dim3(ENTNNZ_THREADS), 0, s, raw->ent_row_ptr, raw->row_nnz_ptr, E,
                       out->ent_nnz_ptr, mid_list, mid2_list, big_list, stats);
  }
  DBG_STAGE("pack_entnnz_kernel");
  SideJoin side_join{ctx, s};
  PackStats* hs = reinterpret_cast<PackStats*>(ctx->host_pinned);
  const int ns = E <= PACK_FAN_MAX_ENTITIES ? ctx->n_side : 0;
  hipStream_t const sb = ns >= 1 ? ctx->side[0] : s;
  hipStream_t const s2 = ns >= 2 ? ctx->side[1] : (ns == 1 ? ctx->side[0] : s);
  hipStream_t const s3 = ns >= 3 ? ctx->side[2] : s2;
  SmallFetch counts;
  if (ns >= 1) {
    HIP_TRY(post_small(ctx, 3, stats, sizeof(PackStats), hs, s, &counts));
    HIP_TRY(hipEventRecord(ctx->side_fork, s));
    HIP_TRY(side_join.use(0));
  }
  static int pack_occupancy = 0;
  if (pack_occupancy == 0) {
    int occ = 0;
    if (hipOccupancyMaxActiveBlocksPerMultiprocessor(&occ, pack_entity_kernel<PACK_LDS_KEYS, PACK_WAVES>, WAVE * PACK_WAVES, 0) != hipSuccess || occ < 1) occ = 4;
    pack_occupancy = occ;
  }
  int eblocks = (int)((E + PACK_WAVES - 1) / PACK_WAVES);
  if (eblocks > ctx->num_cus * pack_occupancy) eblocks = ctx->num_cus * pack_occupancy;
  hipLaunchKernelGGL((pack_entity_kernel<PACK_LDS_KEYS, PACK_WAVES>), dim3(eblocks), dim3(WAVE * PACK_WAVES), 0, s,
                     (const int32_t*)nullptr, (const int*)nullptr, raw->ent_row_ptr,
                     raw->row_nnz_ptr, out->ent_nnz_ptr, raw->col_global, raw->val, E, ic, out->row_ptr, sort_key,
                     out->csr_col, out->col_ptr, out->csc_row, out->csc_val, uniq_sparse, d_cnt, stats, pack_bitmap_on());
  DBG_STAGE("pack_entity_kernel<256>");
  if (ns >= 1) HIP_TRY(wait_small(ctx, counts));
  if (ns == 0 || hs->n_mid > 0) {
    if (ns >= 2) HIP_TRY(side_join.use(1));
    hipLaunchKernelGGL((pack_entity_kernel<PACK_CAP2, 4>), dim3(ctx->num_cus * 4), dim3(WAVE * 4), 0, s2,
                       (const int32_t*)mid_list, (const int*)&stats->n_mid, raw->ent_row_ptr,
                       raw->row_nnz_ptr, out->ent_nnz_ptr, raw->col_global, raw->val, E, ic, out->row_ptr, sort_key,
                       out->csr_col, out->col_ptr, out->csc_row, out->csc_val, uniq_sparse, d_cnt, stats, pack_bitmap_on());
  }
  DBG_STAGE("pack_entity_kernel<512>");
  if (ns == 0 || hs->n_mid2 > 0) {
    if (ns >= 2) HIP_TRY(side_join.use(ns >= 3 ? 2 : 1));
    hipLaunchKernelGGL((pack_entity_kernel<PACK_CAP3, 2>), dim3(ctx->num_cus * 4), dim3(WAVE * 2), 0, s3,
                       (const int32_t*)mid2_list, (const int*)&stats->n_mid2, raw->ent_row_ptr,
                       raw->row_nnz_ptr, out->ent_nnz_ptr, raw->col_global, raw->val, E, ic, out->row_ptr, sort_key,
                       out->csr_col, out->col_ptr, out->csc_row, out->csc_val, uniq_sparse, d_cnt, stats, pack_bitmap_on());
  }
  DBG_STAGE("pack_entity_kernel<1024>");
  {
    if (ns == 0) HIP_TRY(fetch_small(ctx, 1, stats, sizeof(PackStats), hs, s));
    if (hs->n_big > 0) {
      BigPackArgs A{raw->ent_row_ptr, out->ent_nnz_ptr, raw->row_nnz_ptr, raw->col_global, raw->val, ic, out->row_ptr, out->csr_col,
                    out->col_ptr, out->csc_row, out->csc_val, uniq_sparse, d_cnt, big_list, hs->n_big,
                    (int64_t)hs->big_nnz, &stats->max_p, &stats->err};
      const int rc = pack_big_entities(ctx, A, sb, ns >= 1 ? s : sb);
      if (rc != GDMIX_RE_OK) return rc;
    }
  }
  side_join.join();
  DBG_STAGE("pack_big_entities");
  const int nb = (int)((E + SCAN_CHUNK - 1) / SCAN_CHUNK);
  hipLaunchKernelGGL(scan_reduce_kernel, dim3(nb), dim3(256), 0, s, d_cnt, E, block_sums);
  hipLaunchKernelGGL(scan_blocksums_kernel, dim3(1), dim3(1024), 0, s, block_sums, nb, stats);
  hipLaunchKernelGGL(scan_apply_kernel, dim3(nb), dim3(256), 0, s, d_cnt, E, block_sums, out->ent_feat_ptr);
  DBG_STAGE("scan kernels");
  const bool defer = ctx->defer_unique && ctx->n_side > 0;
  hipStream_t const sc = defer ? ctx->side[ctx->n_side - 1] : s;
  SmallFetch tail_fetch;
  if (defer) {
    HIP_TRY(post_small(ctx, 1, stats, sizeof(PackStats), hs, s, &tail_fetch));
    HIP_TRY(hipEventRecord(ctx->side_fork, s));
    HIP_TRY(hipStreamWaitEvent(sc, ctx->side_fork, 0));
  }
  {
    static int defer_wgs = 0;
    if (defer_wgs == 0) { const char* e = getenv("GDMIX_RE_DEFER_WGS"); defer_wgs = (e && atoi(e) > 0) ? atoi(e) : 4; }
    const int per_cu = defer ? defer_wgs : 16;
    int grid = (int)((E + 3) / 4);
    if (grid > ctx->num_cus * per_cu) grid = ctx->num_cus * per_cu;
    hipLaunchKernelGGL(pack_compact_unique_kernel, dim3(grid), dim3(256), 0, sc, out->ent_nnz_ptr, out->ent_feat_ptr, E,
                       uniq_sparse, out->unique_global);
  }
  DBG_STAGE("pack_compact_unique_kernel");
  HIP_TRY(hipGetLastError());
  if (defer) {
    HIP_TRY(hipEventRecord(ctx->unique_ev, sc));
    ctx->unique_pending = true;
    HIP_TRY(wait_small(ctx, tail_fetch));
  } else {
    HIP_TRY(fetch_small(ctx, 1, stats, sizeof(PackStats), hs, s));
  }
  if (hs->err) {
    if (defer) HIP_TRY(join_unique(ctx, s));
    set_error("pack: an entity exceeds a per-entity int32 limit or a feature index is outside [0, 2^31)");
    return hs->err;
  }
  out->D = (int64_t)hs->D;
  out->max_p = hs->max_p; out->max_n = hs->max_n; out->max_nnz = hs->max_nnz;
  return GDMIX_RE_OK;
}

__global__ void partition_ids_kernel(const int64_t* __restrict__ ids, int64_t count, int32_t num_partitions,
                                     int32_t* __restrict__ out) {
  for (int64_t i = (int64_t)blockIdx.x * blockDim.x + threadIdx.x; i < count; i += (int64_t)gridDim.x * blockDim.x) {
    const int64_t v = ids[i];
    unsigned long long mag = v < 0 ? (unsigned long long)(-(v + 1)) + 1ull : (unsigned long long)v;
    char digits[20];
    int nd = 0;
    do { digits[nd++] = (char)('0' + (int)(mag % 10ull)); mag /= 10ull; } while (mag);
    uint32_t h = 0;
    if (v < 0) h = 31u * h + (uint32_t)'-';
    for (int k = nd - 1; k >= 0; --k) h = 31u * h + (uint32_t)digits[k];
    const int32_t hs = (int32_t)h;
    const int32_t a = (hs == INT32_MIN) ? hs : (hs < 0 ? -hs : hs);
    out[i] = (int32_t)((int64_t)a % (int64_t)num_partitions);
  }
}

hipError_t launch_partition_ids(const int64_t* ids, int64_t count, int32_t num_partitions, int32_t* out,
                                hipStream_t s) {
  if (count <= 0) return hipSuccess;
  int grid = (int)((count + 255) / 256);
  if (grid > 4096) grid = 4096;
  hipLaunchKernelGGL(partition_ids_kernel, dim3(grid), dim3(256), 0, s, ids, count, num_partitions, out);
  return hipGetLastError();
}

}
```

gdmix_amd/csrc/re_prior.hip:

```cpp
#include <stdint.h>
#include <math.h>

#include "re_internal.hpp"
#include "re_search.hpp"

namespace gdmix {

constexpr int PRIOR_LONG_ROW = 32;

__device__ __forceinline__ float prior_one(float x, int32_t col, const double* __restrict__ mu, const double* __restrict__ sc, double& acc) {
  acc = fma((double)x, mu[col], acc);
  return (float)__dmul_rn((double)x, sc[col]);
}

__device__ __forceinline__ void prior_four(const float* __restrict__ val, const int32_t* __restrict__ col, int64_t j, const double* __restrict__ mu,
                                           const double* __restrict__ sc, float* __restrict__ out, double& acc) {
  const float4 v = *reinterpret_cast<const float4*>(val + j);
  const int4 c = *reinterpret_cast<const int4*>(col + j);
  float4 r;
  r.x = prior_one(v.x, c.x, mu, sc, acc);
  r.y = prior_one(v.y, c.y, mu, sc, acc);
  r.z = prior_one(v.z, c.z, mu, sc, acc);
  r.w = prior_one(v.w, c.w, mu, sc, acc);
  *reinterpret_cast<float4*>(out + j) = r;
// ... 13 lines not shown
  if (live) {
    const int64_t r0 = B.ent_row_ptr[e], z0 = B.ent_nnz_ptr[e];
    const int64_t c0 = B.ent_feat_ptr[e] + e * ic;
    const int32_t* rp = B.row_ptr + r0 + e + (g - r0);
    a = z0 + rp[0];
    b = z0 + rp[1];
    cb = c0 + ic;
    off = (double)B.offset[g];
    if (ic) acc = mean[c0];
  }
  const bool long_row = live && (b - a) > PRIOR_LONG_ROW;
  if (live && !long_row) {
    const double* __restrict__ mu = mean + cb;
    const double* __restrict__ sc = scale + cb;
    int64_t j = a;
    while (j < b) {
      if (VEC && (j & 3) == 0 && j + 4 <= b) {
        prior_four(B.csr_val, B.csr_col, j, mu, sc, val_out, acc);
        j += 4;
      } else {
        val_out[j] = prior_one(B.csr_val[j], B.csr_col[j], mu, sc, acc);
        ++j;
      }
    }
  }
  unsigned long long todo = __ballot(long_row);
  while (todo) {
    const int src = __ffsll((long long)todo) - 1;
    todo &= todo - 1;
    const int64_t ra = __shfl(a, src), rb = __shfl(b, src), rc = __shfl(cb, src);
    const double* __restrict__ mu = mean + rc;
    const double* __restrict__ sc = scale + rc;
    double part = 0.0;
    for (int64_t j = (ra & ~(int64_t)3) + 4 * lane; j < rb; j += 4 * WAVE) {
      if (VEC && j >= ra && j + 4 <= rb) {
        prior_four(B.csr_val, B.csr_col, j, mu, sc, val_out, part);
      } else {
        for (int k = 0; k < 4; ++k) {
          const int64_t jj = j + k;
          if (jj >= ra && jj < rb) val_out[jj] = prior_one(B.csr_val[jj], B.csr_col[jj], mu, sc, part);
        }
      }
    }
    const double total = wave_sum(part);
    if (lane == src) acc += total;
  }
  if (live) offset_out[g] = (float)(acc + off);
}

struct PriorColumn { int64_t e; int64_t col_end; double s; };
__device__ __forceinline__ PriorColumn prior_locate(const BatchDev& B, int64_t e_lo, int64_t e_hi, int ic, const double* __restrict__ scale, int64_t k) {
  PriorColumn L;
  L.e = entity_of_sample(B.ent_nnz_ptr, e_lo, e_hi, k);
  const int64_t z0 = B.ent_nnz_ptr[L.e], f0 = B.ent_feat_ptr[L.e];
  const int d = (int)(B.ent_feat_ptr[L.e + 1] - f0);
  const int32_t* __restrict__ cp = B.col_ptr + z0 + L.e;
  const int32_t rel = (int32_t)(k - z0);
  int lo = 0, hi = d - 1;
  while (lo < hi) {
    const int mid = (lo + hi + 1) >> 1;
    if (cp[mid] <= rel) lo = mid; else hi = mid - 1;
  }
  L.col_end = z0 + cp[lo + 1];
  L.s = scale[f0 + L.e * ic + ic + lo];
  return L;
}

template <bool VEC>
__global__ __launch_bounds__(256) void prior_csc_kernel(BatchDev B, int64_t E, int64_t Z, int ic, const double* __restrict__ scale,
                                                        float* __restrict__ val_out) {
  const int lane = threadIdx.x & (WAVE - 1);
  const int64_t t = (int64_t)blockIdx.x * blockDim.x + threadIdx.x;
  const int64_t kf = (t - lane) * 4;
  if (kf >= Z) return;
  const int64_t kl = (kf + 4 * WAVE - 1 < Z) ? kf + 4 * WAVE - 1 : Z - 1;
  const int64_t e_lo = wave_entity_of_sample(B.ent_nnz_ptr, 0, E - 1, kf, lane);
  const int64_t e_hi = wave_entity_of_sample(B.ent_nnz_ptr, e_lo, E - 1, kl, lane);
  const int64_t k0 = t * 4;
  if (k0 >= Z) return;
  PriorColumn L = prior_locate(B, e_lo, e_hi, ic, scale, k0);
  if (VEC && k0 + 4 <= Z && k0 + 4 <= L.col_end) {
    const float4 v = *reinterpret_cast<const float4*>(B.csc_val + k0);
    float4 r;
    r.x = (float)__dmul_rn((double)v.x, L.s);
    r.y = (float)__dmul_rn((double)v.y, L.s);
    r.z = (float)__dmul_rn((double)v.z, L.s);
    r.w = (float)__dmul_rn((double)v.w, L.s);
    *reinterpret_cast<float4*>(val_out + k0) = r;
    return;
  }
  const int64_t k1 = (k0 + 4 < Z) ? k0 + 4 : Z;
  for (int64_t k = k0; k < k1; ++k) {
    if (k >= L.col_end) L = prior_locate(B, L.e, e_hi, ic, scale, k);
    val_out[k] = (float)__dmul_rn((double)B.csc_val[k], L.s);
  }
}

__global__ __launch_bounds__(256) void prior_restore_kernel(int64_t P, const double* __restrict__ mean, const double* __restrict__ scale, double threshold,
                                                            const double* phi, const double* var_phi, double* theta, double* theta_thr, double* variance) {
#pragma clang fp contract(off)
  const int64_t j = (int64_t)blockIdx.x * blockDim.x + threadIdx.x;
  if (j >= P) return;
  const double s = scale[j];
  const double v = mean[j] + s * phi[j];
  const double var = (variance && var_phi) ? (s * s) * var_phi[j] : 0.0;
  if (theta) theta[j] = v;
  if (theta_thr) theta_thr[j] = (fabs(v) <= threshold) ? 0.0 : v;
  if (variance && var_phi) variance[j] = var;
}

static inline size_t prior_align(size_t bytes) { return (bytes + 255) & ~(size_t)255; }
static inline bool prior_aligned16(const void* p) { return (reinterpret_cast<uintptr_t>(p) & 15) == 0; }

}

using namespace gdmix;

extern "C" {

GDMIX_API size_t gdmix_re_prior_workspace_bytes(const gdmix_re_packed* packed) {
  if (!packed || packed->Z < 0 || packed->N < 0) return 0;
  return 2 * prior_align((size_t)packed->Z * sizeof(float)) + prior_align((size_t)packed->N * sizeof(float));
}

GDMIX_API int gdmix_re_prior_apply(gdmix_re_ctx* ctx, const gdmix_re_packed* packed, int has_intercept, const double* mean, const double* scale,
                                   void* workspace, size_t workspace_bytes, gdmix_re_packed* out, void* stream) {
  if (!ctx || !packed || !out) { set_error("gdmix_re_prior_apply: NULL argument"); return GDMIX_RE_EINVAL; }
  if (packed->E < 0 || packed->N < 0 || packed->Z < 0 || packed->D < 0) { set_error("gdmix_re_prior_apply: bad batch"); return GDMIX_RE_EINVAL; }
  const size_t need = gdmix_re_prior_workspace_bytes(packed);
  if (need > 0 && (!workspace || workspace_bytes < need)) {
    set_error("gdmix_re_prior_apply: workspace of %zu bytes, %zu needed (gdmix_re_prior_workspace_bytes)", workspace ? workspace_bytes : (size_t)0, need);
    return GDMIX_RE_ENOMEM;
  }
  if (!prior_aligned16(workspace)) { set_error("gdmix_re_prior_apply: the workspace must be 16-byte aligned"); return GDMIX_RE_EINVAL; }
  const int64_t E = packed->E, N = packed->N, Z = packed->Z;
  const int ic = has_intercept ? 1 : 0;
  if (E > 0 && N > 0) {
    if (!packed->ent_row_ptr || !packed->ent_nnz_ptr || !packed->ent_feat_ptr || !packed->row_ptr || !packed->offset ||
        (Z > 0 && (!packed->csr_col || !packed->csr_val || !packed->col_ptr || !packed->csc_val))) {
      set_error("gdmix_re_prior_apply: NULL array in the packed batch");
      return GDMIX_RE_EINVAL;
    }
    if ((packed->D + E * ic > 0) && (!mean || !scale)) { set_error("gdmix_re_prior_apply: NULL mean or scale"); return GDMIX_RE_EINVAL; }
    if ((N + 255) / 256 > 0x7fffffffLL || (Z + 1023) / 1024 > 0x7fffffffLL) { set_error("gdmix_re_prior_apply: too many samples or non-zeros"); return GDMIX_RE_ERANGE; }
  }
  char* w = static_cast<char*>(workspace);
  float* csr_out = reinterpret_cast<float*>(w);
  float* csc_out = reinterpret_cast<float*>(w + prior_align((size_t)Z * sizeof(float)));
  float* off_out = reinterpret_cast<float*>(w + 2 * prior_align((size_t)Z * sizeof(float)));
  gdmix_re_packed result = *packed;
  result.csr_val = csr_out;
  result.csc_val = csc_out;
  result.offset = off_out;
  if (E > 0 && N > 0) {
    HIP_TRY(hipSetDevice(ctx->impl.device));
    hipStream_t s = static_cast<hipStream_t>(stream);
    const BatchDev B = batch_dev(packed);
    const unsigned row_blocks = (unsigned)((N + 255) / 256);
    if (prior_aligned16(packed->csr_val) && prior_aligned16(packed->csr_col))
      hipLaunchKernelGGL((prior_csr_kernel<true>), dim3(row_blocks), dim3(256), 0, s, B, E, N, ic, mean, scale, csr_out, off_out);
    else
      hipLaunchKernelGGL((prior_csr_kernel<false>), dim3(row_blocks), dim3(256), 0, s, B, E, N, ic, mean, scale, csr_out, off_out);
    if (Z > 0) {
      const unsigned nz_blocks = (unsigned)((Z + 1023) / 1024);
      if (prior_aligned16(packed->csc_val))
        hipLaunchKernelGGL((prior_csc_kernel<true>), dim3(nz_blocks), dim3(256), 0, s, B, E, Z, ic, scale, csc_out);
      else
        hipLaunchKernelGGL((prior_csc_kernel<false>), dim3(nz_blocks), dim3(256), 0, s, B, E, Z, ic, scale, csc_out);
    }
    HIP_TRY(hipGetLastError());
  }
  *out = result;
  return GDMIX_RE_OK;
}

GDMIX_API int gdmix_re_prior_restore(gdmix_re_ctx* ctx, const gdmix_re_packed* packed, int has_intercept, const double* mean, const double* scale,
                                     double threshold, const double* phi, const double* var_phi, double* theta, double* theta_thr,
                                     double* variance, void* stream) {
  if (!ctx || !packed) { set_error("gdmix_re_prior_restore: NULL argument"); return GDMIX_RE_EINVAL; }
  if (packed->E < 0 || packed->D < 0) { set_error("gdmix_re_prior_restore: bad batch"); return GDMIX_RE_EINVAL; }
  const int64_t P = packed->D + (has_intercept ? packed->E : 0);
  if (P == 0) return GDMIX_RE_OK;
  if (!mean || !scale || !phi) { set_error("gdmix_re_prior_restore: NULL mean, scale or phi"); return GDMIX_RE_EINVAL; }
  if (variance && !var_phi) { set_error("gdmix_re_prior_restore: variance asked for without var_phi"); return GDMIX_RE_EINVAL; }
  if ((P + 255) / 256 > 0x7fffffffLL) { set_error("gdmix_re_prior_restore: too many coefficients"); return GDMIX_RE_ERANGE; }
  HIP_TRY(hipSetDevice(ctx->impl.device));
  hipLaunchKernelGGL(prior_restore_kernel, dim3((unsigned)((P + 255) / 256)), dim3(256), 0, static_cast<hipStream_t>(stream), P, mean, scale, threshold, phi,
                     var_phi, theta, theta_thr, variance);
  HIP_TRY(hipGetLastError());
  return GDMIX_RE_OK;
}

}
```

gdmix_amd/csrc/re_route.hip:

```cpp
#include <stdlib.h>

#include "re_internal.hpp"
#include "re_solve_team.hpp"

namespace gdmix {

int make_class_table(const gdmix_ctx_impl* ci, const gdmix_re_opts* opts, ClassTable* out) {
  ClassTable& tab = *out;
  for (int c = 0; c < GDMIX_RE_NUM_CLASSES; ++c) {
    const ClassDesc& d = kClasses[c];
    tab.kind[c] = d.kind;
    tab.ncap[c] = d.ncap;
    tab.zcap[c] = d.zcap;
    int lds = d.lds;
    const int gl = d.lanes;
    if (lds > 0 && gl > 0)
      lds = (gl >= WAVE ? 1 : WAVE / gl) * quad_layout(gl * d.epl, d.ncap, d.zcap, gl > WAVE ? gl / WAVE : 1).bytes;
    bool on = lds > 0 && (lds <= ci->wave_lds_limit || (gl > WAVE && ci->wave_lds_limit >= 65536 && lds <= 160 * 1024));
    if (gl > 0 && !(ci->kernel_mask & 4)) on = false;
    if (d.kind == KIND_WLDS && !(ci->kernel_mask & 2)) on = false;
    tab.lds_bytes[c] = on ? lds : 0;
  }
  tab.giant_nnz = opts->m <= TEAM_MCAP ? ci->giant_nnz : 0;
  tab.team_nnz = opts->m <= TEAM_MCAP ? ci->team_nnz : 0;
  tab.tall_min_n = ci->tall_min_n;
  tab.tall_split_n = ci->tall_split_n;
  tab.tall_adapt_limit = ci->tall_split_set ? 0 : ci->tall_adapt_limit;
  {
    const int tn = ci->tall_team_n;
    tab.tall_team_n = tn > 0 ? tn : -tn;
    if (tab.tall_team_n > 0 && tab.tall_team_n < TALL_TEAM_MIN_N) tab.tall_team_n = TALL_TEAM_MIN_N;
    tab.tall_team_limit = tn > 0 ? ci->tall_team_limit : 0;
  }
  tab.tall_mid_n = (ci->tall_mid_n < 0 && ci->tall_split_set) ? 0 : ci->tall_mid_n;
  tab.narrow = (ci->narrow && tab.lds_bytes[NARROW_HOST_CLASS] > 0 &&
                (WAVE / NARROW_LANES) * quad_layout(NARROW_LANES * NARROW_EPL, NARROW_NCAP, NARROW_ZCAP).bytes <= ci->wave_lds_limit) ? 1 : 0;
  if (opts->sum_loss) {
    if (opts->m > TEAM_MCAP) { set_error("sum_loss needs m <= %d", TEAM_MCAP); return GDMIX_RE_EINVAL; }
    if (opts->variance_mode != GDMIX_RE_VAR_NONE) { set_error("variance is not available with sum_loss"); return GDMIX_RE_EINVAL; }
    tab.giant_nnz = 1;
  }
  return GDMIX_RE_OK;
}

__global__ void re_classify_kernel(const int64_t* __restrict__ ent_row_ptr, const int64_t* __restrict__ ent_nnz_ptr,
                                   const int64_t* __restrict__ ent_feat_ptr, int64_t E, int ic, int m, bool has_w,
                                   ClassTable tab, int32_t* __restrict__ cls_out, ClassCounts* __restrict__ counts) {
  __shared__ int32_t local[GDMIX_RE_NUM_CLASSES];
  __shared__ int32_t tall_ge[TALL_ADAPT_STEPS], team_ge[TALL_TEAM_STEPS], mid_ge[TALL_MID_STEPS];
  if (threadIdx.x < GDMIX_RE_NUM_CLASSES) local[threadIdx.x] = 0;
  if (threadIdx.x < TALL_ADAPT_STEPS) tall_ge[threadIdx.x] = 0;
  if (threadIdx.x < TALL_TEAM_STEPS) team_ge[threadIdx.x] = 0;
  if (threadIdx.x < TALL_MID_STEPS) mid_ge[threadIdx.x] = 0;
  __syncthreads();
  for (int64_t e = (int64_t)blockIdx.x * blockDim.x + threadIdx.x; e < E; e += (int64_t)gridDim.x * blockDim.x) {
    const int n = (int)(ent_row_ptr[e + 1] - ent_row_ptr[e]);
    const int z = (int)(ent_nnz_ptr[e + 1] - ent_nnz_ptr[e]);
    const int d = (int)(ent_feat_ptr[e + 1] - ent_feat_ptr[e]);
    const int p = d + ic;
    int c = BLOCK_CLASS;
    const size_t wlds_bytes = wave_lds_bytes(p, n, z, d, m, has_w);
    for (int k = 0; k < BLOCK_CLASS; ++k) {
      if (tab.lds_bytes[k] <= 0) continue;
      const int kind = tab.kind[k];
      if (group_lanes(kind) > 0) {
        const int cap = group_lanes(kind) * group_epl(kind);
        if (m <= M_REG && p <= cap && n <= tab.ncap[k] && z <= tab.zcap[k]) { c = k; break; }
      } else if (kind == KIND_WLDS) {
        if (wlds_bytes <= (size_t)tab.lds_bytes[k]) { c = k; break; }
      }
    }
    if (tab.tall_min_n > 0 && m <= M_REG && p <= TALL_MAX_P && n >= tab.tall_min_n && !(tab.giant_nnz > 0 && z >= tab.giant_nnz)) c = (n >= tab.tall_split_n) ? TALL_CLASS
        : (tall_resident_bytes(1, tall_sets(1, p), d, n, z, has_w) <= (size_t)TALL_LEAN_ARENA ? TALL_L_CLASS : TALL_S_CLASS);
    else if (tab.giant_nnz > 0 && z >= tab.giant_nnz) c = GIANT_CLASS;
    else if (c == BLOCK_CLASS || (tab.team_nnz > 0 && z >= tab.team_nnz)) {
      if (tab.team_nnz > 0 && z >= tab.team_nnz)
        c = (z >= 128 * tab.team_nnz) ? TEAM8_CLASS : ((z >= 8 * tab.team_nnz) ? TEAM32_CLASS : TEAM128_CLASS);
    }
    cls_out[e] = (c == NARROW_HOST_CLASS && tab.narrow && narrow_fits(p, n, z)) ? (c | NARROW_FLAG) : c;
    atomicAdd(&local[c], 1);
    if (c == TALL_S_CLASS && tab.tall_adapt_limit > 0 && n >= tall_adapt_n(0)) {
#pragma unroll
      for (int k = 0; k < TALL_ADAPT_STEPS; ++k)
        if (n >= tall_adapt_n(k)) atomicAdd(&tall_ge[k], 1);
    }
    if (c == TALL_S_CLASS && tab.tall_mid_n < 0 && n >= tall_mid_step(0)) {
#pragma unroll
      for (int k = 0; k < TALL_MID_STEPS; ++k)
        if (n >= tall_mid_step(k)) atomicAdd(&mid_ge[k], 1);
    }
    if (c == TALL_S_CLASS && tab.tall_mid_n > 0 && n >= tab.tall_mid_n) atomicAdd(&mid_ge[0], 1);
    if (c == TALL_CLASS && tab.tall_team_n > 0 && n >= tab.tall_team_n) {
#pragma unroll
      for (int k = 0; k < TALL_TEAM_STEPS; ++k)
        if ((int64_t)n >= ((int64_t)tab.tall_team_n << k)) atomicAdd(&team_ge[k], 1);
    }
    if (c >= TEAM128_CLASS && c <= TEAM8_CLASS) {
      atomicAdd(&counts->team_nnz_total[c], (unsigned long long)z);
      atomicMax(&counts->largest_nnz(c), z);
    }
  }
  __syncthreads();
  if (threadIdx.x < GDMIX_RE_NUM_CLASSES && local[threadIdx.x]) atomicAdd(&counts->count[threadIdx.x], local[threadIdx.x]);
  if (threadIdx.x < TALL_ADAPT_STEPS && tall_ge[threadIdx.x]) atomicAdd(&counts->tall.tall_ge[threadIdx.x], tall_ge[threadIdx.x]);
  if (threadIdx.x < TALL_TEAM_STEPS && team_ge[threadIdx.x]) atomicAdd(&counts->tall.team_ge[threadIdx.x], team_ge[threadIdx.x]);
  if (threadIdx.x < TALL_MID_STEPS && mid_ge[threadIdx.x]) atomicAdd(&counts->tall.mid_ge[threadIdx.x], mid_ge[threadIdx.x]);
}

__global__ void class_base_kernel(ClassCounts* cc, int tall_adapt_limit, int tall_adapt_small, int tall_team_n, int tall_team_limit, int tall_mid_n) {
  if (threadIdx.x == 0 && blockIdx.x == 0) {
    int32_t* const count = cc->count;
    TallRouting& t = cc->tall;
    int team_from = 0;
    if (tall_team_n > 0) {
      if (tall_team_limit <= 0) { if (t.team_ge[0] > 0) team_from = tall_team_n; }
      else
        for (int k = 0; k < TALL_TEAM_STEPS && team_from == 0; ++k)
          if (t.team_ge[k] > 0 && t.team_ge[k] <= tall_team_limit) team_from = tall_team_n << k;
      if (team_from > 0) {
        const int moved = t.team_ge[team_from == tall_team_n ? 0 : (team_from == 2 * tall_team_n ? 1 : 2)];
        count[TALL_T_CLASS] += moved;
        count[TALL_CLASS] -= moved;
      }
    }
    t.team_from = team_from;
    int split = 0;
    if (tall_adapt_limit > 0 && count[TALL_S_CLASS] <= tall_adapt_small) {
      for (int k = 0; k < TALL_ADAPT_STEPS && split == 0; ++k)
        if (t.tall_ge[k] > 0 && count[TALL_CLASS] + t.tall_ge[k] <= tall_adapt_limit) {
          split = tall_adapt_n(k);
          count[TALL_CLASS] += t.tall_ge[k];
          count[TALL_S_CLASS] -= t.tall_ge[k];
        }
    }
    t.split = split;
    int mid_from = 0;
    const int gone = split > 0 ? t.tall_ge[split == tall_adapt_n(0) ? 0 : (split == tall_adapt_n(1) ? 1 : 2)] : 0;
    if (tall_mid_n > 0) {
      const int cnt = (split > 0 && split <= tall_mid_n) ? 0 : t.mid_ge[0] - gone;
      if (cnt > 0) { mid_from = tall_mid_n; count[TALL_M_CLASS] += cnt; count[TALL_S_CLASS] -= cnt; }
    } else if (tall_mid_n < 0 && count[TALL_S_CLASS] <= tall_adapt_small) {
      for (int k = 0; k < TALL_MID_STEPS && mid_from == 0; ++k) {
        if (split > 0 && tall_mid_step(k) >= split) break;
        const int cnt = t.mid_ge[k] - gone;
        if (cnt > 0 && cnt <= -tall_mid_n) { mid_from = tall_mid_step(k); count[TALL_M_CLASS] += cnt; count[TALL_S_CLASS] -= cnt; }
      }
    }
    t.mid_from = mid_from;
    int run = 0;
#pragma unroll
    for (int c = 0; c < GDMIX_RE_NUM_CLASSES; ++c) { cc->base[c] = run; run += count[c]; cc->cursor[c] = 0; }
  }
}

__global__ __launch_bounds__(256) void re_order_kernel(int32_t* __restrict__ cls, int64_t E, ClassCounts* __restrict__ cc,
                                                       int32_t* __restrict__ order, const int64_t* __restrict__ ent_row_ptr) {
  __shared__ int32_t cnt[GDMIX_RE_NUM_CLASSES], base[GDMIX_RE_NUM_CLASSES];
  __shared__ int32_t nar_cnt, nar_base;
  const int split = cc->tall.split;
  const int team_from = cc->tall.team_from;
  const int mid_from = cc->tall.mid_from;
  const int64_t chunk = (int64_t)blockDim.x * 8;
  for (int64_t start = (int64_t)blockIdx.x * chunk; start < E; start += (int64_t)gridDim.x * chunk) {
    if (threadIdx.x < GDMIX_RE_NUM_CLASSES) cnt[threadIdx.x] = 0;
    if (threadIdx.x == 0) nar_cnt = 0;
    __syncthreads();
    int c[8], pos[8];
    unsigned nar = 0;
#pragma unroll
    for (int k = 0; k < 8; ++k) {
      const int64_t e = start + (int64_t)k * blockDim.x + threadIdx.x;
      c[k] = (e < E) ? cls[e] : -1;
      if (c[k] >= NARROW_FLAG) { c[k] -= NARROW_FLAG; cls[e] = c[k]; nar |= 1u << k; }
      if (split > 0 && c[k] == TALL_S_CLASS && ent_row_ptr[e + 1] - ent_row_ptr[e] >= split) { c[k] = TALL_CLASS; cls[e] = TALL_CLASS; }
      else if (team_from > 0 && c[k] == TALL_CLASS && ent_row_ptr[e + 1] - ent_row_ptr[e] >= team_from) { c[k] = TALL_T_CLASS; cls[e] = TALL_T_CLASS; }
      else if (mid_from > 0 && c[k] == TALL_S_CLASS && ent_row_ptr[e + 1] - ent_row_ptr[e] >= mid_from) { c[k] = TALL_M_CLASS; cls[e] = TALL_M_CLASS; }
      pos[k] = (c[k] >= 0) ? atomicAdd((nar >> k) & 1u ? &nar_cnt : &cnt[c[k]], 1) : 0;
    }
    __syncthreads();
    if (threadIdx.x < GDMIX_RE_NUM_CLASSES)
      base[threadIdx.x] = cnt[threadIdx.x] ? atomicAdd(&cc->cursor[threadIdx.x], cnt[threadIdx.x]) : 0;
    if (threadIdx.x == GDMIX_RE_NUM_CLASSES) nar_base = nar_cnt ? atomicAdd(&cc->narrow_count, nar_cnt) : 0;
    __syncthreads();
#pragma unroll
    for (int k = 0; k < 8; ++k) {
      const int64_t e = start + (int64_t)k * blockDim.x + threadIdx.x;
      if (c[k] < 0) continue;
      const int seg = cc->base[c[k]];
      if ((nar >> k) & 1u) order[seg + nar_base + pos[k]] = (int32_t)e;
      else if (c[k] == NARROW_HOST_CLASS) order[seg + cc->count[c[k]] - 1 - (base[c[k]] + pos[k])] = (int32_t)e;
      else order[seg + base[c[k]] + pos[k]] = (int32_t)e;
    }
    __syncthreads();
  }
}

static hipError_t launch_classify(const gdmix_re_packed* b, int ic, int m, const ClassTable& tab, ClassCounts* counts, hipStream_t s) {
  int grid = (int)((b->E + 255) / 256);
  if (grid > 2048) grid = 2048;
  hipLaunchKernelGGL(re_classify_kernel, dim3(grid), dim3(256), 0, s, b->ent_row_ptr, b->ent_nnz_ptr,
                     b->ent_feat_ptr, b->E, ic, m, b->weight != nullptr, tab, b->cls_tmp, counts);
  return hipGetLastError();
}

static hipError_t launch_order(const gdmix_re_packed* b, ClassCounts* counts, hipStream_t s) {
  int grid = (int)((b->E + 2047) / 2048);
  if (grid > 2048) grid = 2048;
  hipLaunchKernelGGL(re_order_kernel, dim3(grid), dim3(256), 0, s, b->cls_tmp, b->E, counts, b->order, b->ent_row_ptr);
  return hipGetLastError();
}

int route(gdmix_ctx_impl* ci, const gdmix_re_packed* b, const ClassTable& tab, const gdmix_re_opts* opts, hipStream_t s,
          const ClassCounts** host) {
  ClassCounts* const cc = reinterpret_cast<ClassCounts*>(b->class_count);
  HIP_TRY(hipMemsetAsync(cc, 0, sizeof(ClassCounts), s));
  HIP_TRY(launch_classify(b, opts->has_intercept ? 1 : 0, opts->m, tab, cc, s));
  hipLaunchKernelGGL(class_base_kernel, dim3(1), dim3(1), 0, s, cc, tab.tall_adapt_limit, 16 * ci->num_cus, tab.tall_team_n, tab.tall_team_limit, tab.tall_mid_n);
  HIP_TRY(hipGetLastError());
  HIP_TRY(launch_order(b, cc, s));
  ClassCounts* const hc = reinterpret_cast<ClassCounts*>(ci->host_pinned + COUNTS_READBACK_WORDS);
  HIP_TRY(fetch_small(ci, 0, cc, sizeof(ClassCounts), hc, s));
  *host = hc;
  return GDMIX_RE_OK;
}

static bool class_is_small(const ClassDesc& d, int count, int num_cus) {
  const long waves = ((long)count * d.occ_lanes + WAVE - 1) / WAVE;
  return waves < (long)num_cus * 6;
}

LaunchPlan plan_launches(const ClassCounts& counts, int num_cus, int n_side, int spread, int lean_rounds) {
  LaunchPlan plan;
  plan.n = 0;
  const int lean = counts.count[TALL_L_CLASS];
  plan.lean_merged = (lean > 0 && lean < lean_rounds * num_cus * TALL_LEAN_WGS) ? lean : 0;
  int begin[GDMIX_RE_NUM_CLASSES], count[GDMIX_RE_NUM_CLASSES], n_launch_classes = 0;
  for (int c = 0; c < GDMIX_RE_NUM_CLASSES; ++c) { begin[c] = counts.base[c]; count[c] = counts.count[c]; }
  if (plan.lean_merged) { count[TALL_L_CLASS] = 0; begin[TALL_S_CLASS] -= plan.lean_merged; count[TALL_S_CLASS] += plan.lean_merged; }
  for (int c = 0; c < GDMIX_RE_NUM_CLASSES; ++c) n_launch_classes += (counts.count[c] > 0 && !(c == TALL_L_CLASS && plan.lean_merged)) ? 1 : 0;
  plan.fork = false;
  if (n_side > 0 && n_launch_classes > 1) {
    for (int c = 0; c < BLOCK_CLASS && !plan.fork; ++c) plan.fork = count[c] > 0 && class_is_small(kClasses[c], count[c], num_cus);
    if (spread > 1) plan.fork = true;
  }
  bool small[GDMIX_RE_NUM_CLASSES], any_large = false;
  for (int k = 0; k < TALL_VARIANTS + BLOCK_CLASS; ++k) {
    const int c = k < TALL_VARIANTS ? tall_class_of_rank(k) : k - TALL_VARIANTS;
    if (k >= TALL_VARIANTS && kClasses[c].tall_rank >= 0) continue;
    if (count[c] <= 0) continue;
    small[plan.n] = plan.fork && class_is_small(kClasses[c], count[c], num_cus);
    any_large = any_large || !small[plan.n];
    plan.launch[plan.n++] = Launch{c, begin[c], count[c], -1, c == NARROW_HOST_CLASS ? counts.narrow_count : 0};
  }
  int spread_rr = 0;
  for (int k = 0; k < plan.n; ++k) {
    Launch& L = plan.launch[k];
    if (small[k]) {
      const int side = kClasses[L.c].small_side;
      L.stream = side >= 0 ? side % n_side : (any_large ? 0 : -1);
    } else if (plan.fork && spread > 1) {
      const int nq = spread < n_side + 1 ? spread : n_side + 1;
      L.stream = spread_rr++ % nq - 1;
    }
  }
  return plan;
}

}
```

gdmix_amd/solver.py:

```python
import ctypes as C
import functools
import os
from dataclasses import dataclass
from typing import Optional

import numpy as np

from .batch import RawBatch, WireRawBatch

_HERE = os.path.dirname(os.path.abspath(__file__))
LIB_PATH = os.path.join(_HERE, "libgdmix_re.so")

NUM_CLASSES = 40
STATUS_NAMES = ("PGTOL", "FACTR", "MAXITER", "MAXFUN", "ABNORMAL")
VAR_NONE, VAR_SIMPLE, VAR_FULL = 0, 1, 2
VARIANCE_MODES = {None: VAR_NONE, "simple": VAR_SIMPLE, "SIMPLE": VAR_SIMPLE, "full": VAR_FULL, "FULL": VAR_FULL,
                  0: VAR_NONE, 1: VAR_SIMPLE, 2: VAR_FULL}


class GdmixReError(RuntimeError):
    pass


class _RawBatch(C.Structure):
    _fields_ = [("E", C.c_int64), ("N", C.c_int64), ("Z", C.c_int64),
                ("ent_row_ptr", C.c_void_p), ("row_nnz_ptr", C.c_void_p), ("col_global", C.c_void_p),
                ("val", C.c_void_p), ("y", C.c_void_p), ("offset", C.c_void_p), ("weight", C.c_void_p)]


class _WireBatch(C.Structure):
    _fields_ = [("E", C.c_int64), ("N", C.c_int64), ("Z", C.c_int64), ("ent_n", C.c_void_p), ("row_nnz", C.c_void_p),
                ("row_nnz_width", C.c_int32), ("y_width", C.c_int32), ("col_width", C.c_int32), ("reserved", C.c_int32),
                ("col_global", C.c_void_p), ("val", C.c_void_p),
                ("y", C.c_void_p), ("offset", C.c_void_p), ("weight", C.c_void_p)]


class _Packed(C.Structure):
    _fields_ = [("E", C.c_int64), ("N", C.c_int64), ("Z", C.c_int64), ("D", C.c_int64),
                ("ent_row_ptr", C.c_void_p), ("ent_nnz_ptr", C.c_void_p), ("ent_feat_ptr", C.c_void_p),
                ("row_ptr", C.c_void_p), ("csr_col", C.c_void_p), ("csr_val", C.c_void_p),
                ("col_ptr", C.c_void_p), ("csc_row", C.c_void_p), ("csc_val", C.c_void_p),
                ("unique_global", C.c_void_p), ("y", C.c_void_p), ("offset", C.c_void_p), ("weight", C.c_void_p),
                ("order", C.c_void_p), ("cls_tmp", C.c_void_p), ("class_count", C.c_void_p),
                ("scratch", C.c_void_p), ("scratch_bytes", C.c_size_t),
                ("max_p", C.c_int32), ("max_n", C.c_int32), ("max_nnz", C.c_int32)]


class _Opts(C.Structure):
    _fields_ = [("l2", C.c_double), ("regularize_bias", C.c_int32), ("has_intercept", C.c_int32),
                ("m", C.c_int32), ("max_iter", C.c_int32), ("maxfun", C.c_int32), ("maxls", C.c_int32),
                ("ftol", C.c_double), ("pgtol", C.c_double), ("variance_mode", C.c_int32),
                ("threshold", C.c_double), ("sum_loss", C.c_int32), ("loss", C.c_int32)]


class _Result(C.Structure):
    _fields_ = [("theta", C.c_void_p), ("theta_thr", C.c_void_p), ("variance", C.c_void_p),
                ("fval", C.c_void_p), ("gnorm", C.c_void_p), ("nit", C.c_void_p), ("nfev", C.c_void_p),
                ("status", C.c_void_p)]


class _EvalOut(C.Structure):
    _fields_ = [("two_u", C.c_void_p), ("n_pos", C.c_void_p), ("n_neg", C.c_void_p), ("n_nan", C.c_void_p), ("sse", C.c_void_p), ("auc", C.c_void_p)]


class _EvalAcc(C.Structure):
    _fields_ = [("keys", C.c_void_p), ("capacity", C.c_int64), ("count", C.c_int64), ("state", C.c_void_p)]


EVAL_ACC_STATE_BYTES = 33024


class _EvalPlOut(C.Structure):
    _fields_ = [("pl", C.c_void_p), ("n", C.c_void_p), ("n_nan", C.c_void_p)]


class _EvalPlAcc(C.Structure):
    _fields_ = [("state", C.c_void_p), ("count", C.c_int64)]


class _EvalPlTotals(C.Structure):
    _fields_ = [("pl", C.c_double), ("n", C.c_int64), ("n_nan", C.c_int64)]


EVAL_PL_STATE_BYTES = 33024
EVAL_LL_STATE_BYTES = EVAL_PL_STATE_BYTES
EVAL_LL_TERM_EPS = 1.5e-16
EVAL_TOPK_MAX = 4


class _EvalTopkOut(C.Structure):
    _fields_ = [("hits_sure", C.c_void_p), ("slots", C.c_void_p), ("tie_pos", C.c_void_p), ("tie_size", C.c_void_p)]


class _DownsampleOpts(C.Structure):
    _fields_ = [("rate", C.c_double), ("seed", C.c_uint64), ("negatives_only", C.c_int32), ("reserved", C.c_int32)]


class _DownsampleCounts(C.Structure):
    _fields_ = [("rows", C.c_int64), ("kept", C.c_int64), ("kept_nnz", C.c_int64), ("positives", C.c_int64), ("negatives_kept", C.c_int64)]


class _DownsampleOut(C.Structure):
    _fields_ = [("N", C.c_int64), ("Z", C.c_int64), ("ent_row_ptr", C.c_void_p), ("row_nnz_ptr", C.c_void_p), ("col_global", C.c_void_p),
                ("val", C.c_void_p), ("y", C.c_void_p), ("offset", C.c_void_p), ("weight", C.c_void_p)]


class _CapOpts(C.Structure):
    _fields_ = [("upper_bound", C.c_int64), ("seed", C.c_uint64)]


class _CapCounts(C.Structure):
    _fields_ = [("entities", C.c_int64), ("capped", C.c_int64), ("rows", C.c_int64), ("kept", C.c_int64), ("kept_nnz", C.c_int64),
                ("largest", C.c_int64)]


class _SelectCounts(C.Structure):
    _fields_ = [("entities", C.c_int64), ("affected", C.c_int64), ("features", C.c_int64), ("kept", C.c_int64), ("dropped", C.c_int64),
                ("kept_nnz", C.c_int64)]


class _SelectOut(C.Structure):
    _fields_ = [("Z", C.c_int64), ("row_nnz_ptr", C.c_void_p), ("col_global", C.c_void_p), ("val", C.c_void_p)]


class _GroupOut(C.Structure):
    _fields_ = [("row_of", C.c_void_p), ("present", C.c_void_p), ("ent_row_ptr", C.c_void_p), ("row_nnz_ptr", C.c_void_p), ("col_global", C.c_void_p),
                ("val", C.c_void_p)]


class _GroupCounts(C.Structure):
    _fields_ = [("rows", C.c_int64), ("grouped", C.c_int64), ("grouped_nnz", C.c_int64), ("entities", C.c_int64), ("left_out", C.c_int64)]


COMBINE_MAX = 8


class _EvalTotals(C.Structure):
    _fields_ = [("two_u", C.c_uint64), ("n", C.c_int64), ("n_pos", C.c_int64), ("n_neg", C.c_int64), ("n_nan", C.c_int64), ("sse", C.c_double)]


EXPORTED_SYMBOLS = (
    "gdmix_re_abi_version", "gdmix_re_build_id", "gdmix_re_device_shared", "gdmix_re_grid_lock_acquire", "gdmix_re_grid_lock_release", "gdmix_re_grid_lock_stats", "gdmix_re_last_error", "gdmix_re_default_opts", "gdmix_re_create",
    "gdmix_re_destroy", "gdmix_re_pack_workspace_bytes", "gdmix_re_pack", "gdmix_re_set_defer_unique", "gdmix_re_pack_join", "gdmix_re_solve",
    "gdmix_re_solve_l1", "gdmix_re_solve_l1_scratch_bytes",
    "gdmix_re_solve_scratch_bytes", "gdmix_re_set_scratch", "gdmix_re_variance_full", "gdmix_re_set_wave_lds_limit", "gdmix_re_score",
    "gdmix_re_widen_workspace_bytes", "gdmix_re_widen", "gdmix_re_set_timing", "gdmix_re_last_solve_ms", "gdmix_re_set_kernel_mask", "gdmix_re_set_giant_nnz", "gdmix_re_set_team_nnz", "gdmix_re_set_tall_min_n", "gdmix_re_set_tall_split_n", "gdmix_re_set_tall_team_n", "gdmix_re_set_tall_mid_n", "gdmix_re_set_spread", "gdmix_re_set_narrow",
    "gdmix_fe_create", "gdmix_fe_destroy", "gdmix_fe_eval", "gdmix_fe_reduce_buffer", "gdmix_fe_step", "gdmix_fe_step_async", "gdmix_fe_step_status", "gdmix_fe_solve", "gdmix_fe_result",
    "gdmix_fe_last_eval_ms", "gdmix_fe_stream_bytes", "gdmix_fe_score", "gdmix_fe_hessian_diag", "gdmix_fe_hessian_dense_scratch_bytes", "gdmix_fe_hessian_dense", "gdmix_fe_hessian_dense_loss",
    "gdmix_fe_variance_of_hessian", "gdmix_fe_restart", "gdmix_fe_set_prior", "gdmix_fe_set_l1", "gdmix_fe_set_optimizer", "gdmix_fe_set_bounds", "gdmix_fe_products", "gdmix_fe_hessian_vec", "gdmix_fe_score_models_workspace_bytes", "gdmix_fe_score_models",
    "gdmix_re_eval_workspace_bytes", "gdmix_re_eval_entities", "gdmix_re_set_eval_small_max", "gdmix_re_eval_acc_reset", "gdmix_re_eval_acc_add",
    "gdmix_re_eval_acc_workspace_bytes", "gdmix_re_eval_acc_finish",
    "gdmix_re_eval_pl_entities", "gdmix_re_eval_pl_acc_reset", "gdmix_re_eval_pl_acc_add", "gdmix_re_eval_pl_acc_finish",
    "gdmix_re_eval_topk_workspace_bytes", "gdmix_re_eval_topk_entities",
    "gdmix_re_eval_ll_entities", "gdmix_re_eval_ll_acc_reset", "gdmix_re_eval_ll_acc_add", "gdmix_re_eval_ll_acc_finish",
    "gdmix_re_join_features", "gdmix_re_score_models_workspace_bytes", "gdmix_re_score_models",
    "gdmix_re_prior_workspace_bytes", "gdmix_re_prior_apply", "gdmix_re_prior_restore",
    "gdmix_re_feature_extent", "gdmix_re_feature_moments", "gdmix_re_feature_scale_expand",
    "gdmix_re_downsample_workspace_bytes", "gdmix_re_downsample_plan", "gdmix_re_downsample_apply",
    "gdmix_re_select_workspace_bytes", "gdmix_re_select_plan", "gdmix_re_select_apply", "gdmix_re_set_select_small_max",
    "gdmix_re_cap_workspace_bytes", "gdmix_re_cap_plan", "gdmix_re_cap_apply", "gdmix_re_set_cap_small_max",
    "gdmix_re_group_workspace_bytes", "gdmix_re_group_rows", "gdmix_re_rows_gather_f32", "gdmix_re_rows_scatter_f32", "gdmix_re_offsets_combine",
    "gdmix_re_class_kernel_name", "gdmix_java_string_hash", "gdmix_java_partition_id",
    "gdmix_java_partition_ids_i64")

_lib = None


def load_library():
    global _lib
    if _lib is not None:
        return _lib
    if not os.path.exists(LIB_PATH):
        raise GdmixReError(
            f"{LIB_PATH} is missing: build it with `python -m gdmix_amd.build` "
            "(there is no CPU fallback for the random-effect solve)")
    try:
        import torch
    except Exception:
        pass
    from . import build as _build
    stale = _build.check_library(LIB_PATH, _build.source_id, "csrc/*.hip, *.hpp")
    if stale:
        raise GdmixReError(stale)
    lib = C.CDLL(LIB_PATH)
    lib.gdmix_re_abi_version.restype = C.c_int
    lib.gdmix_re_build_id.restype = C.c_char_p
    lib.gdmix_re_device_shared.argtypes = [C.c_void_p]
    lib.gdmix_re_grid_lock_acquire.argtypes = [C.c_char_p]
    lib.gdmix_re_grid_lock_release.argtypes = [C.c_char_p]
    lib.gdmix_re_grid_lock_stats.argtypes = [C.c_char_p, C.POINTER(C.c_int64), C.POINTER(C.c_int64)]
    lib.gdmix_re_last_error.restype = C.c_char_p
    lib.gdmix_re_default_opts.argtypes = [C.POINTER(_Opts)]
    lib.gdmix_re_default_opts.restype = None
    lib.gdmix_re_create.argtypes = [C.c_int, C.POINTER(C.c_void_p)]
    lib.gdmix_re_destroy.argtypes = [C.c_void_p]
    lib.gdmix_re_destroy.restype = None
    lib.gdmix_re_pack_workspace_bytes.argtypes = [C.c_int64, C.c_int64, C.c_int64]
    lib.gdmix_re_pack_workspace_bytes.restype = C.c_size_t
    lib.gdmix_re_pack.argtypes = [C.c_void_p, C.POINTER(_RawBatch), C.c_int, C.c_void_p, C.c_size_t,
                                  C.POINTER(_Packed), C.c_void_p]
    lib.gdmix_re_set_defer_unique.argtypes = [C.c_void_p, C.c_int]
    lib.gdmix_re_pack_join.argtypes = [C.c_void_p, C.c_void_p]
    lib.gdmix_re_widen_workspace_bytes.argtypes = [C.c_int64, C.c_int64, C.c_int64]
    lib.gdmix_re_widen_workspace_bytes.restype = C.c_size_t
    lib.gdmix_re_widen.argtypes = [C.c_void_p, C.POINTER(_WireBatch), C.c_void_p, C.c_size_t, C.POINTER(_RawBatch), C.c_void_p]
    lib.gdmix_re_solve.argtypes = [C.c_void_p, C.POINTER(_Packed), C.POINTER(_Opts), C.c_void_p,
                                   C.POINTER(_Result), C.c_void_p]
    lib.gdmix_re_variance_full.argtypes = [C.c_void_p, C.POINTER(_Packed), C.POINTER(_Opts), C.c_void_p, C.c_void_p, C.c_void_p]
    lib.gdmix_re_solve_scratch_bytes.argtypes = [C.POINTER(_Packed), C.POINTER(_Opts)]
    lib.gdmix_re_solve_scratch_bytes.restype = C.c_size_t
    lib.gdmix_re_solve_l1.argtypes = [C.c_void_p, C.POINTER(_Packed), C.POINTER(_Opts), C.c_double, C.c_void_p,
                                      C.POINTER(_Result), C.c_void_p]
    lib.gdmix_re_solve_l1_scratch_bytes.argtypes = [C.POINTER(_Packed), C.POINTER(_Opts)]
    lib.gdmix_re_solve_l1_scratch_bytes.restype = C.c_size_t
    lib.gdmix_re_set_scratch.argtypes = [C.c_void_p, C.c_void_p, C.c_size_t]
    lib.gdmix_re_set_wave_lds_limit.argtypes = [C.c_void_p, C.c_int]
    lib.gdmix_re_set_kernel_mask.argtypes = [C.c_void_p, C.c_int]
    lib.gdmix_re_set_giant_nnz.argtypes = [C.c_void_p, C.c_int64]
    lib.gdmix_fe_create.argtypes = [C.c_void_p, C.POINTER(_Packed), C.c_int64, C.POINTER(_Opts), C.c_void_p,
                                    C.POINTER(C.c_void_p), C.c_void_p]
    lib.gdmix_fe_destroy.argtypes = [C.c_void_p]
    lib.gdmix_fe_destroy.restype = None
    lib.gdmix_fe_eval.argtypes = [C.c_void_p, C.c_void_p]
    lib.gdmix_fe_reduce_buffer.argtypes = [C.c_void_p, C.POINTER(C.c_int64)]
    lib.gdmix_fe_reduce_buffer.restype = C.c_void_p
    lib.gdmix_fe_step.argtypes = [C.c_void_p, C.c_void_p, C.POINTER(C.c_int32)]
    lib.gdmix_fe_step_async.argtypes = [C.c_void_p, C.c_void_p, C.POINTER(C.c_int64)]
    lib.gdmix_fe_step_status.argtypes = [C.c_void_p, C.c_int64, C.POINTER(C.c_int32)]
    lib.gdmix_fe_solve.argtypes = [C.c_void_p, C.c_void_p, C.c_int32, C.c_int64, C.POINTER(C.c_int32), C.POINTER(C.c_int64)]
    lib.gdmix_fe_hessian_diag.argtypes = [C.c_void_p, C.c_void_p, C.c_void_p]
    lib.gdmix_fe_stream_bytes.argtypes = [C.c_void_p, C.POINTER(C.c_int64), C.POINTER(C.c_int64)]
    lib.gdmix_fe_result.argtypes = [C.c_void_p, C.c_void_p, C.POINTER(C.c_double), C.POINTER(C.c_double),
                                    C.POINTER(C.c_int32), C.POINTER(C.c_int32), C.c_void_p]
    lib.gdmix_fe_score.argtypes = [C.c_void_p, C.c_int64, C.c_void_p, C.c_void_p, C.c_void_p, C.c_void_p, C.c_void_p, C.c_int64, C.c_int,
                                   C.c_void_p, C.c_void_p, C.c_void_p]
    lib.gdmix_fe_hessian_dense_scratch_bytes.argtypes = [C.POINTER(_Packed)]
    lib.gdmix_fe_hessian_dense_scratch_bytes.restype = C.c_size_t
    lib.gdmix_fe_hessian_dense.argtypes = [C.c_void_p, C.POINTER(_Packed), C.c_int, C.c_void_p, C.c_void_p, C.c_int64, C.c_void_p, C.c_size_t, C.c_void_p]
    lib.gdmix_fe_hessian_dense_loss.argtypes = [C.c_void_p, C.POINTER(_Packed), C.c_int, C.c_int, C.c_void_p, C.c_void_p, C.c_int64, C.c_void_p, C.c_size_t,
                                                C.c_void_p]
    lib.gdmix_fe_variance_of_hessian.argtypes = [C.c_void_p, C.c_void_p, C.c_int64, C.c_int64, C.c_double, C.c_int64, C.c_void_p, C.c_void_p, C.c_void_p]
    lib.gdmix_fe_last_eval_ms.argtypes = [C.c_void_p, C.POINTER(C.c_float), C.POINTER(C.c_float)]
    lib.gdmix_fe_restart.argtypes = [C.c_void_p, C.POINTER(_Opts), C.c_void_p, C.c_void_p]
    lib.gdmix_fe_set_prior.argtypes = [C.c_void_p, C.c_void_p, C.c_void_p, C.c_void_p]
    lib.gdmix_fe_set_l1.argtypes = [C.c_void_p, C.c_double, C.c_void_p]
    lib.gdmix_fe_set_optimizer.argtypes = [C.c_void_p, C.c_int, C.c_void_p]
    lib.gdmix_fe_set_bounds.argtypes = [C.c_void_p, C.c_void_p, C.c_void_p, C.c_void_p]
    lib.gdmix_fe_products.argtypes = [C.c_void_p, C.POINTER(C.c_int64), C.c_void_p]
    lib.gdmix_fe_hessian_vec.argtypes = [C.c_void_p, C.c_void_p, C.c_void_p, C.c_void_p]
    lib.gdmix_fe_score_models_workspace_bytes.argtypes = [C.c_int64, C.c_int]
    lib.gdmix_fe_score_models_workspace_bytes.restype = C.c_size_t
    lib.gdmix_fe_score_models.argtypes = [C.c_void_p, C.c_int64, C.c_void_p, C.c_void_p, C.c_void_p, C.c_void_p, C.POINTER(C.c_void_p), C.c_int, C.c_int64,
                                          C.c_int, C.c_void_p, C.c_void_p, C.c_void_p, C.c_size_t, C.c_void_p]
    lib.gdmix_re_set_team_nnz.argtypes = [C.c_void_p, C.c_int64]
    lib.gdmix_re_set_tall_min_n.argtypes = [C.c_void_p, C.c_int]
    lib.gdmix_re_set_tall_split_n.argtypes = [C.c_void_p, C.c_int]
    lib.gdmix_re_set_tall_team_n.argtypes = [C.c_void_p, C.c_int]
    lib.gdmix_re_set_tall_mid_n.argtypes = [C.c_void_p, C.c_int]
    lib.gdmix_re_set_spread.argtypes = [C.c_void_p, C.c_int]
    lib.gdmix_re_set_narrow.argtypes = [C.c_void_p, C.c_int]
    lib.gdmix_re_set_timing.argtypes = [C.c_void_p, C.c_int]
    lib.gdmix_re_last_solve_ms.argtypes = [C.c_void_p, C.POINTER(C.c_float)]
    lib.gdmix_re_score.argtypes = [C.c_void_p, C.POINTER(_Packed), C.c_int, C.c_void_p, C.c_void_p,
                                   C.c_void_p, C.c_void_p, C.c_void_p]
    lib.gdmix_re_class_kernel_name.argtypes = [C.c_int]
    lib.gdmix_re_class_kernel_name.restype = C.c_char_p
    lib.gdmix_java_string_hash.argtypes = [C.c_void_p, C.c_int64]
    lib.gdmix_java_string_hash.restype = C.c_int32
    lib.gdmix_java_partition_id.argtypes = [C.c_void_p, C.c_int64, C.c_int32]
    lib.gdmix_java_partition_id.restype = C.c_int32
    lib.gdmix_java_partition_ids_i64.argtypes = [C.c_void_p, C.c_void_p, C.c_int64, C.c_int32, C.c_void_p, C.c_void_p]
    lib.gdmix_re_eval_workspace_bytes.argtypes = [C.c_int64, C.c_int64]
    lib.gdmix_re_eval_workspace_bytes.restype = C.c_size_t
    lib.gdmix_re_eval_entities.argtypes = [C.c_void_p, C.c_void_p, C.c_int64, C.c_int64, C.c_void_p, C.c_void_p, C.POINTER(_EvalOut), C.c_void_p,
                                           C.c_size_t, C.c_void_p]
    lib.gdmix_re_set_eval_small_max.argtypes = [C.c_void_p, C.c_int]
    lib.gdmix_re_eval_acc_reset.argtypes = [C.c_void_p, C.POINTER(_EvalAcc), C.c_void_p]
    lib.gdmix_re_eval_acc_add.argtypes = [C.c_void_p, C.POINTER(_EvalAcc), C.c_void_p, C.c_void_p, C.c_int64, C.c_void_p]
    lib.gdmix_re_eval_acc_workspace_bytes.argtypes = [C.c_int64]
    lib.gdmix_re_eval_acc_workspace_bytes.restype = C.c_size_t
    lib.gdmix_re_eval_acc_finish.argtypes = [C.c_void_p, C.POINTER(_EvalAcc), C.c_void_p, C.c_size_t, C.POINTER(_EvalTotals), C.c_void_p]
    lib.gdmix_re_eval_pl_entities.argtypes = [C.c_void_p, C.c_void_p, C.c_int64, C.c_int64, C.c_void_p, C.c_void_p, C.POINTER(_EvalPlOut), C.c_void_p]
    lib.gdmix_re_eval_pl_acc_reset.argtypes = [C.c_void_p, C.POINTER(_EvalPlAcc), C.c_void_p]
    lib.gdmix_re_eval_pl_acc_add.argtypes = [C.c_void_p, C.POINTER(_EvalPlAcc), C.c_void_p, C.c_void_p, C.c_int64, C.c_void_p]
    lib.gdmix_re_eval_pl_acc_finish.argtypes = [C.c_void_p, C.POINTER(_EvalPlAcc), C.POINTER(_EvalPlTotals), C.c_void_p]
    lib.gdmix_re_eval_ll_entities.argtypes = lib.gdmix_re_eval_pl_entities.argtypes
    lib.gdmix_re_eval_ll_acc_reset.argtypes = lib.gdmix_re_eval_pl_acc_reset.argtypes
    lib.gdmix_re_eval_ll_acc_add.argtypes = lib.gdmix_re_eval_pl_acc_add.argtypes
    lib.gdmix_re_eval_ll_acc_finish.argtypes = lib.gdmix_re_eval_pl_acc_finish.argtypes
    lib.gdmix_re_eval_topk_workspace_bytes.argtypes = [C.c_int64, C.c_int64]
    lib.gdmix_re_eval_topk_workspace_bytes.restype = C.c_size_t
    lib.gdmix_re_eval_topk_entities.argtypes = [C.c_void_p, C.c_void_p, C.c_int64, C.c_int64, C.c_void_p, C.c_void_p, C.POINTER(C.c_int32), C.c_int,
                                                C.POINTER(_EvalTopkOut), C.POINTER(_EvalOut), C.c_void_p, C.c_size_t, C.c_void_p]
    lib.gdmix_re_join_features.argtypes = [C.c_void_p, C.POINTER(_Packed), C.POINTER(_Packed), C.c_int, C.c_void_p, C.c_void_p, C.c_void_p, C.c_void_p]
    lib.gdmix_re_score_models_workspace_bytes.argtypes = [C.c_int64, C.c_int]
    lib.gdmix_re_score_models_workspace_bytes.restype = C.c_size_t
    lib.gdmix_re_score_models.argtypes = [C.c_void_p, C.POINTER(_Packed), C.c_int, C.POINTER(C.c_void_p), C.c_int, C.c_int64, C.c_void_p, C.c_void_p,
                                          C.c_void_p, C.c_void_p, C.c_void_p, C.c_size_t, C.c_void_p]
    lib.gdmix_re_prior_workspace_bytes.argtypes = [C.POINTER(_Packed)]
    lib.gdmix_re_prior_workspace_bytes.restype = C.c_size_t
    lib.gdmix_re_prior_apply.argtypes = [C.c_void_p, C.POINTER(_Packed), C.c_int, C.c_void_p, C.c_void_p, C.c_void_p, C.c_size_t, C.POINTER(_Packed), C.c_void_p]
    lib.gdmix_re_prior_restore.argtypes = [C.c_void_p, C.POINTER(_Packed), C.c_int, C.c_void_p, C.c_void_p, C.c_double, C.c_void_p, C.c_void_p, C.c_void_p,
                                           C.c_void_p, C.c_void_p, C.c_void_p]
    lib.gdmix_re_feature_extent.argtypes = [C.c_void_p, C.c_void_p, C.c_int, C.c_void_p, C.c_int64, C.c_int64, C.c_void_p, C.c_void_p, C.c_void_p, C.c_void_p]
    lib.gdmix_re_feature_moments.argtypes = [C.c_void_p, C.c_void_p, C.c_int, C.c_void_p, C.c_int64, C.c_int64, C.c_void_p, C.c_void_p, C.c_void_p, C.c_void_p,
                                             C.c_void_p, C.c_void_p]
    lib.gdmix_re_feature_scale_expand.argtypes = [C.c_void_p, C.POINTER(_Packed), C.c_int, C.c_void_p, C.c_int64, C.c_void_p, C.c_void_p]
    lib.gdmix_re_downsample_workspace_bytes.argtypes = [C.c_int64, C.c_int64]
    lib.gdmix_re_downsample_workspace_bytes.restype = C.c_size_t
    lib.gdmix_re_downsample_plan.argtypes = [C.c_void_p, C.POINTER(_RawBatch), C.c_void_p, C.POINTER(_DownsampleOpts), C.c_void_p, C.c_size_t,
                                             C.POINTER(_DownsampleCounts), C.c_void_p]
    lib.gdmix_re_downsample_apply.argtypes = [C.c_void_p, C.POINTER(_RawBatch), C.POINTER(_DownsampleOpts), C.c_void_p, C.c_size_t,
                                              C.POINTER(_DownsampleOut), C.c_void_p, C.c_void_p]
    lib.gdmix_re_select_workspace_bytes.argtypes = [C.c_int64, C.c_int64, C.c_int64]
    lib.gdmix_re_select_workspace_bytes.restype = C.c_size_t
    lib.gdmix_re_select_plan.argtypes = [C.c_void_p, C.POINTER(_Packed), C.c_double, C.c_void_p, C.c_size_t, C.c_void_p, C.c_void_p,
                                         C.POINTER(_SelectCounts), C.c_void_p]
    lib.gdmix_re_select_apply.argtypes = [C.c_void_p, C.POINTER(_RawBatch), C.POINTER(_Packed), C.c_void_p, C.POINTER(_SelectOut), C.c_void_p]
    lib.gdmix_re_set_select_small_max.argtypes = [C.c_void_p, C.c_int]
    lib.gdmix_re_cap_workspace_bytes.argtypes = [C.c_int64, C.c_int64]
    lib.gdmix_re_cap_workspace_bytes.restype = C.c_size_t
    lib.gdmix_re_cap_plan.argtypes = [C.c_void_p, C.POINTER(_RawBatch), C.c_void_p, C.POINTER(_CapOpts), C.c_void_p, C.c_size_t, C.POINTER(_CapCounts),
                                      C.c_void_p]
    lib.gdmix_re_cap_apply.argtypes = [C.c_void_p, C.POINTER(_RawBatch), C.POINTER(_CapOpts), C.c_void_p, C.c_size_t, C.POINTER(_DownsampleOut),
                                       C.c_void_p, C.c_void_p]
    lib.gdmix_re_set_cap_small_max.argtypes = [C.c_void_p, C.c_int]
    lib.gdmix_re_group_workspace_bytes.argtypes = [C.c_int64, C.c_int64]
    lib.gdmix_re_group_workspace_bytes.restype = C.c_size_t
    lib.gdmix_re_group_rows.argtypes = [C.c_void_p, C.c_int64, C.c_int64, C.c_int64, C.c_void_p, C.c_void_p, C.c_void_p, C.c_void_p, C.c_void_p, C.c_size_t,
                                        C.POINTER(_GroupOut), C.POINTER(_GroupCounts), C.c_void_p]
    lib.gdmix_re_rows_gather_f32.argtypes = [C.c_void_p, C.c_void_p, C.c_int64, C.c_void_p, C.c_int64, C.c_void_p, C.c_void_p]
    lib.gdmix_re_rows_scatter_f32.argtypes = [C.c_void_p, C.c_void_p, C.c_int64, C.c_void_p, C.c_int64, C.c_void_p, C.c_int, C.c_void_p]
    lib.gdmix_re_offsets_combine.argtypes = [C.c_void_p, C.c_void_p, C.c_int64, C.c_void_p, C.POINTER(C.c_void_p), C.c_int, C.c_int, C.c_void_p, C.c_int64,
                                             C.c_void_p]
    if lib.gdmix_re_abi_version() != 27:
        raise GdmixReError("libgdmix_re.so ABI version mismatch")
    _lib = lib
    return lib


def _check(rc, what):
    if rc != 0:
        msg = load_library().gdmix_re_last_error().decode("utf-8", "replace")
        raise GdmixReError(f"{what} failed ({rc}): {msg}")


LOSS_CODES = {"logistic": 0, "squared": 1, "poisson": 2}


@dataclass
class SolverOptions:
    l2: float = 1.0
    regularize_bias: bool = True
    has_intercept: bool = True
    m: int = 10
    max_iter: int = 100
    maxfun: int = 15000
    maxls: int = 20
    ftol: float = 1e-12
    pgtol: float = 1e-5
    variance_mode: int = VAR_NONE
    threshold: float = 1e-4
    sum_loss: bool = False
    linear: bool = False
    loss: str = None

    def loss_name(self):
        if self.loss is None:
            return "squared" if self.linear else "logistic"
        if self.linear:
            raise ValueError("SolverOptions: give either linear=True or loss=..., not both")
        if self.loss not in LOSS_CODES:
            raise ValueError(f"SolverOptions.loss must be one of {sorted(LOSS_CODES)}, not {self.loss!r}")
        return self.loss

    def loss_code(self):
        return LOSS_CODES[self.loss_name()]

    def to_c(self):
        return _Opts(float(self.l2), int(bool(self.regularize_bias)), int(bool(self.has_intercept)),
                     int(self.m), int(self.max_iter), int(self.maxfun), int(self.maxls), float(self.ftol),
                     float(self.pgtol), int(VARIANCE_MODES[self.variance_mode]), float(self.threshold),
                     int(bool(self.sum_loss)), self.loss_code())


def java_string_hash(s: str) -> int:
    cu = np.frombuffer(s.encode("utf-16-le"), dtype=np.uint16).copy()
    return int(load_library().gdmix_java_string_hash(cu.ctypes.data_as(C.c_void_p), cu.size))


def java_partition_id(s: str, num_partitions: int) -> int:
    cu = np.frombuffer(s.encode("utf-16-le"), dtype=np.uint16).copy()
    return int(load_library().gdmix_java_partition_id(cu.ctypes.data_as(C.c_void_p), cu.size, num_partitions))


class PackedBatch:

    def __init__(self, c_struct, tensors, raw_dev, has_intercept, join=None, parent=None):
        self.c = c_struct
        self._join = join
        self._parent = parent
        self._tensors = tensors
        self._raw_dev = raw_dev
        self.has_intercept = bool(has_intercept)
        self.E, self.N, self.Z, self.D = int(c_struct.E), int(c_struct.N), int(c_struct.Z), int(c_struct.D)
        self.P = self.D + (self.E if has_intercept else 0)
        self.max_p, self.max_n, self.max_nnz = int(c_struct.max_p), int(c_struct.max_n), int(c_struct.max_nnz)

    def _view(self, ptr, count, dtype):
        import torch
        ws = self._tensors["workspace"]
        own = self._tensors.get("prior_workspace")
        if own is not None and own.data_ptr() <= ptr < own.data_ptr() + own.numel():
# ... 60 lines not shown
        return fp + (np.arange(self.E + 1, dtype=np.int64) if self.has_intercept else 0)


def host_array(t):
    if not getattr(t, "is_cuda", False):
        return t.cpu().numpy()
    if t.numel() * t.element_size() < (1 << 20):
        return t.cpu().numpy()
    import torch
    h = torch.empty(t.shape, dtype=t.dtype, pin_memory=True)
    h.copy_(t, non_blocking=True)
    torch.cuda.current_stream().synchronize()
    return h.numpy()


class SolveResult:
    def __init__(self, tensors, E, P):
        self._t = tensors
        self.E, self.P = E, P

    def __getattr__(self, k):
        t = self.__dict__.get("_t", {})
        if k in t:
            return t[k]
        raise AttributeError(k)

    def to_host(self, keys=None):
        out, staged = {}, []
        for k, v in self._t.items():
            if keys is not None and k not in keys:
                continue
            if v is None:
                out[k] = None
            elif v.is_cuda and v.numel() * v.element_size() >= (1 << 20):
                import torch
                h = torch.empty(v.shape, dtype=v.dtype, pin_memory=True)
                h.copy_(v, non_blocking=True)
                staged.append((k, h))
            else:
                out[k] = v.cpu().numpy()
        if staged:
            import torch
            torch.cuda.current_stream().synchronize()
            for k, h in staged:
                out[k] = h.numpy()
        return out


def _serialised(fn):
    import functools

    @functools.wraps(fn)
    def wrapper(self, *a, **k):
        with self._ctx_lock:
            return fn(self, *a, **k)
    return wrapper


class REDeviceSolver:

    def __init__(self, device: int = 0):
        import torch
        if not torch.cuda.is_available():
            raise GdmixReError("no HIP device visible: the random-effect solve runs on MI355X only "
                               "(there is no CPU fallback)")
        self.torch = torch
        self.lib = load_library()
        self.tall_team_n = self.TALL_TEAM_N_DEFAULT
        self.device_index = int(device)
        self.device = torch.device("cuda", self.device_index)
        torch.cuda.set_device(self.device)
        torch.zeros(1, device=self.device)
        h = C.c_void_p()
        import threading
        self._ctx_lock = threading.RLock()
        _check(self.lib.gdmix_re_create(self.device_index, C.byref(h)), "gdmix_re_create")
        self._h = h
        self._scratch = None
        self._pack_gen = 0
        self.set_defer_unique(os.environ.get("GDMIX_RE_DEFER_UNIQUE", "1") != "0")

    @_serialised
    def set_defer_unique(self, enabled: bool):
        _check(self.lib.gdmix_re_set_defer_unique(self._h, int(bool(enabled))), "gdmix_re_set_defer_unique")

    @_serialised
    def pack_join(self, stream=None):
        if getattr(self, "_h", None):
            _check(self.lib.gdmix_re_pack_join(self._h, self._stream() if stream is None else stream), "gdmix_re_pack_join")

    @_serialised
    def _pack_join_of(self, gen, pack_stream, dropping=False):
        if gen == self._pack_gen:
            self.pack_join(pack_stream if dropping else None)

    @_serialised
    def close(self):
        if getattr(self, "_h", None):
            self.lib.gdmix_re_destroy(self._h)
            self._h = None

    def __del__(self):
        try:
            self.close()
        except Exception:
            pass

    def set_wave_lds_limit(self, nbytes: int):
        _check(self.lib.gdmix_re_set_wave_lds_limit(self._h, int(nbytes)), "set_wave_lds_limit")

    def set_kernel_mask(self, mask: int):
        _check(self.lib.gdmix_re_set_kernel_mask(self._h, int(mask)), "set_kernel_mask")

    def set_giant_nnz(self, nnz: int):
        _check(self.lib.gdmix_re_set_giant_nnz(self._h, int(nnz)), "set_giant_nnz")

    def set_team_nnz(self, nnz: int):
        _check(self.lib.gdmix_re_set_team_nnz(self._h, int(nnz)), "set_team_nnz")

    TALL_MIN_N_DEFAULT = 32

    def set_tall_min_n(self, min_n: int):
        _check(self.lib.gdmix_re_set_tall_min_n(self._h, int(min_n)), "set_tall_min_n")

    def set_tall_split_n(self, split_n: int):
        _check(self.lib.gdmix_re_set_tall_split_n(self._h, int(split_n)), "set_tall_split_n")

    TALL_TEAM_N_DEFAULT = 8192
    TALL_SPLIT_N_DEFAULT = 4096

    def pin_routing(self):
        self.set_tall_split_n(self.TALL_SPLIT_N_DEFAULT)
        self.set_tall_team_n(-self.TALL_TEAM_N_DEFAULT)

    def set_tall_team_n(self, team_n: int):
        _check(self.lib.gdmix_re_set_tall_team_n(self._h, int(team_n)), "set_tall_team_n")
        self.tall_team_n = int(team_n)

    def device_shared(self) -> bool:
        rc = self.lib.gdmix_re_device_shared(self._h)
        if rc < 0:
            _check(rc, "gdmix_re_device_shared")
        return bool(rc)

    def set_tall_mid_n(self, mid_n: int):
        _check(self.lib.gdmix_re_set_tall_mid_n(self._h, int(mid_n)), "set_tall_mid_n")

    def set_spread(self, queues: int):
        _check(self.lib.gdmix_re_set_spread(self._h, int(queues)), "set_spread")

    def set_narrow(self, on: bool):
        _check(self.lib.gdmix_re_set_narrow(self._h, int(bool(on))), "set_narrow")

    NARROW_COUNT_WORD = 15

    def narrow_count(self, packed: PackedBatch) -> int:
        row3 = packed._view(packed.c.class_count, 4 * NUM_CLASSES, self.torch.int32)[3 * NUM_CLASSES:].cpu().numpy()
        return int(row3[self.NARROW_COUNT_WORD])

    def set_timing(self, enabled: bool):
        _check(self.lib.gdmix_re_set_timing(self._h, int(bool(enabled))), "set_timing")

    def last_solve_ms(self):
        ms = (C.c_float * NUM_CLASSES)()
        _check(self.lib.gdmix_re_last_solve_ms(self._h, ms), "last_solve_ms")
        return [float(x) for x in ms]

    def _stream(self):
        return C.c_void_p(self.torch.cuda.current_stream(self.device).cuda_stream)

    def upload(self, raw: RawBatch):
        t = self.torch
        dev = self.device
        d = dict(ent_row_ptr=t.from_numpy(raw.ent_row_ptr).to(dev), row_nnz_ptr=t.from_numpy(raw.row_nnz_ptr).to(dev),
                 col_global=t.from_numpy(raw.col_global).to(dev), val=t.from_numpy(raw.val).to(dev),
                 y=t.from_numpy(raw.y).to(dev), offset=t.from_numpy(raw.offset).to(dev),
                 weight=None if raw.weight is None else t.from_numpy(raw.weight).to(dev))
        d["E"], d["N"], d["Z"] = raw.E, raw.N, raw.Z
        return d

    WIRE_ARRAYS = ("ent_n", "row_nnz", "col_global", "val", "y", "offset", "weight")

    def upload_wire(self, wire, pinned=None):
        t = self.torch
        d = {k: wire[k] for k in ("E", "N", "Z", "row_nnz_width", "y_width", "col_width")}
        for k in self.WIRE_ARRAYS:
            a = wire[k]
            if a is None:
                d[k] = None
                continue
            if isinstance(a, t.Tensor):
                d[k] = a.to(self.device, non_blocking=True)
                continue
            if pinned is not None:
                h = pinned[k][:a.size]
                h.numpy()[...] = a
                d[k] = h.to(self.device, non_blocking=True)
            else:
                d[k] = t.from_numpy(a).to(self.device)
        return d

    def wire_stage(self, wire):
        t = self.torch
        st = self.__dict__.setdefault("_wire_stage", {})
        for k in self.WIRE_ARRAYS:
            a = wire[k]
            if a is None or isinstance(a, t.Tensor):
                continue
            tdt = t.from_numpy(a[:0]).dtype
            cur = st.get(k)
            if cur is None or cur.dtype != tdt or cur.numel() < a.size:
                st[k] = t.empty(int(a.size * 1.25) + 1024, dtype=tdt, pin_memory=True)
        return st

    @_serialised
    def widen(self, wd):
        t = self.torch
        E, N, Z = wd["E"], wd["N"], wd["Z"]
        ptr = lambda x: None if x is None or x.numel() == 0 else x.data_ptr()
        c_wire = _WireBatch(E, N, Z, ptr(wd["ent_n"]), ptr(wd["row_nnz"]), wd["row_nnz_width"], wd["y_width"], wd["col_width"], 0, ptr(wd["col_global"]),
                            ptr(wd["val"]), ptr(wd["y"]), ptr(wd["offset"]), ptr(wd["weight"]))
        nbytes = self.lib.gdmix_re_widen_workspace_bytes(E, N, Z)
        ws = t.empty(nbytes, dtype=t.uint8, device=self.device)
        c_raw = _RawBatch()
        _check(self.lib.gdmix_re_widen(self._h, C.byref(c_wire), ws.data_ptr(), nbytes, C.byref(c_raw), self._stream()), "gdmix_re_widen")

        def view(p, count, dtype):
            if not p or count == 0:
                return t.empty(0, dtype=dtype, device=self.device)
            off = p - ws.data_ptr()
            return ws[off:off + count * t.empty(0, dtype=dtype).element_size()].view(dtype)
        y = wd["y"] if wd["y_width"] == 4 else view(c_raw.y, N, t.float32)
        rd = dict(E=E, N=N, Z=Z, ent_row_ptr=view(c_raw.ent_row_ptr, E + 1, t.int64), row_nnz_ptr=view(c_raw.row_nnz_ptr, N + 1, t.int64),
                  col_global=view(c_raw.col_global, Z, t.int64), val=wd["val"], y=y, offset=wd["offset"], weight=wd["weight"],
                  _keep=(ws, wd))
        return rd

    @_serialised
    def pack(self, raw, has_intercept=True) -> PackedBatch:
        t = self.torch
        if isinstance(raw, WireRawBatch):
            rd = self.widen(self.upload_wire(raw.to_wire()))
        else:
            rd = self.upload(raw) if isinstance(raw, RawBatch) else raw
        E, N, Z = rd["E"], rd["N"], rd["Z"]
        ptr = lambda x: None if x is None or x.numel() == 0 else x.data_ptr()
        c_raw = _RawBatch(E, N, Z, rd["ent_row_ptr"].data_ptr(), rd["row_nnz_ptr"].data_ptr(), ptr(rd["col_global"]),
                          ptr(rd["val"]), ptr(rd["y"]), ptr(rd["offset"]), ptr(rd["weight"]))
        nbytes = self.lib.gdmix_re_pack_workspace_bytes(E, N, Z)
        ws = t.empty(nbytes, dtype=t.uint8, device=self.device)
        c_packed = _Packed()
        st = self._stream()
        _check(self.lib.gdmix_re_pack(self._h, C.byref(c_raw), int(bool(has_intercept)), ws.data_ptr(), nbytes,
                                      C.byref(c_packed), st), "gdmix_re_pack")
        self._pack_gen += 1
        return PackedBatch(c_packed, {"workspace": ws}, rd, has_intercept, join=functools.partial(self._pack_join_of, self._pack_gen, st))

    @_serialised
    def downsample(self, raw, uid, rate, seed=0, negatives_only=True):
        t = self.torch
        E, N, Z = int(raw["E"]), int(raw["N"]), int(raw["Z"])
        if isinstance(uid, np.ndarray):
            uid = t.from_numpy(np.ascontiguousarray(uid, np.int64)).to(self.device)
        if uid.dtype != t.int64 or uid.numel() != N or not uid.is_cuda or not uid.is_contiguous():
            raise GdmixReError(f"downsample: uid must be a contiguous int64 array of {N} entries")
        ptr = lambda x: None if x is None or x.numel() == 0 else x.data_ptr()
        c_raw = _RawBatch(E, N, Z, raw["ent_row_ptr"].data_ptr(), raw["row_nnz_ptr"].data_ptr(), ptr(raw["col_global"]),
                          ptr(raw["val"]), ptr(raw["y"]), ptr(raw["offset"]), ptr(raw["weight"]))
        c_opts = _DownsampleOpts(float(rate), int(seed) & 0xFFFFFFFFFFFFFFFF, int(bool(negatives_only)), 0)
        nbytes = int(self.lib.gdmix_re_downsample_workspace_bytes(E, N))
        ws = t.empty(max(nbytes, 1), dtype=t.uint8, device=self.device)
        c_counts = _DownsampleCounts()
        st = self._stream()
        _check(self.lib.gdmix_re_downsample_plan(self._h, C.byref(c_raw), ptr(uid), C.byref(c_opts), ws.data_ptr(), nbytes, C.byref(c_counts), st),
               "gdmix_re_downsample_plan")
        n_out, z_out = int(c_counts.kept), int(c_counts.kept_nnz)
        new = lambda count, dtype: t.empty(count, dtype=dtype, device=self.device)
        d = dict(E=E, N=n_out, Z=z_out, ent_row_ptr=new(E + 1, t.int64), row_nnz_ptr=new(n_out + 1, t.int64), col_global=new(z_out, t.int64),
                 val=new(z_out, t.float32), y=new(n_out, t.float32), offset=new(n_out, t.float32), weight=new(n_out, t.float32),
                 kept_rows=new(n_out, t.int32))
        c_out = _DownsampleOut(n_out, z_out, d["ent_row_ptr"].data_ptr(), d["row_nnz_ptr"].data_ptr(), ptr(d["col_global"]), ptr(d["val"]),
                               ptr(d["y"]), ptr(d["offset"]), ptr(d["weight"]))
        _check(self.lib.gdmix_re_downsample_apply(self._h, C.byref(c_raw), C.byref(c_opts), ws.data_ptr(), nbytes, C.byref(c_out),
                                                  ptr(d["kept_rows"]), st), "gdmix_re_downsample_apply")
        counts = {k: int(getattr(c_counts, k)) for k in ("rows", "kept", "kept_nnz", "positives", "negatives_kept")}
        return d, counts

    CAP_SMALL_MAX_DEFAULT, CAP_SMALL_MAX_LIMIT = 128, 1024

    def set_cap_small_max(self, small_max: int):
        _check(self.lib.gdmix_re_set_cap_small_max(self._h, int(small_max)), "set_cap_small_max")

    @_serialised
    def cap_samples(self, raw, uid, upper_bound, seed=0):
        t = self.torch
        E, N, Z = int(raw["E"]), int(raw["N"]), int(raw["Z"])
        if isinstance(uid, np.ndarray):
            uid = t.from_numpy(np.ascontiguousarray(uid, np.int64)).to(self.device)
        if uid.dtype != t.int64 or uid.numel() != N or not uid.is_cuda or not uid.is_contiguous():
            raise GdmixReError(f"cap_samples: uid must be a contiguous int64 array of {N} entries")
        ptr = lambda x: None if x is None or x.numel() == 0 else x.data_ptr()
        c_raw = _RawBatch(E, N, Z, raw["ent_row_ptr"].data_ptr(), raw["row_nnz_ptr"].data_ptr(), ptr(raw["col_global"]),
                          ptr(raw["val"]), ptr(raw["y"]), ptr(raw["offset"]), ptr(raw["weight"]))
        c_opts = _CapOpts(int(upper_bound), int(seed) & 0xFFFFFFFFFFFFFFFF)
        nbytes = int(self.lib.gdmix_re_cap_workspace_bytes(E, N))
        ws = t.empty(max(nbytes, 1), dtype=t.uint8, device=self.device)
# ... 366 lines not shown
```

include/gdmix_re.h:

```cpp
#ifndef GDMIX_RE_H_
#define GDMIX_RE_H_

#include <stdint.h>
#include <stddef.h>

#ifdef __cplusplus
extern "C" {
#endif

#define GDMIX_RE_ABI_VERSION 27

#if defined(__GNUC__)
#define GDMIX_API __attribute__((visibility("default")))
#else
#define GDMIX_API
#endif

#define GDMIX_RE_OK          0
#define GDMIX_RE_EINVAL    (-1)
#define GDMIX_RE_EHIP      (-2)
#define GDMIX_RE_ENOMEM    (-3)
#define GDMIX_RE_ERANGE    (-4)

#define GDMIX_RE_ST_PGTOL     0
#define GDMIX_RE_ST_FACTR     1
#define GDMIX_RE_ST_MAXITER   2
#define GDMIX_RE_ST_MAXFUN    3
#define GDMIX_RE_ST_ABNORMAL  4
#define GDMIX_RE_ST_ABORTED   9
#define GDMIX_RE_ST_ABORTED_PEER 10

#define GDMIX_RE_VAR_NONE    0
#define GDMIX_RE_VAR_SIMPLE  1
#define GDMIX_RE_VAR_FULL    2

typedef struct gdmix_re_ctx gdmix_re_ctx;

typedef struct {
  int64_t E, N, Z;
  const int64_t* ent_row_ptr;
  const int64_t* row_nnz_ptr;
  const int64_t* col_global;
  const float*   val;
  const float*   y;
  const float*   offset;
  const float*   weight;
} gdmix_re_raw_batch;

typedef struct {
  int64_t E, N, Z;
  const int32_t* ent_n;
  const void*    row_nnz;
  int32_t        row_nnz_width;
  int32_t        y_width;
  int32_t        col_width;
  int32_t        reserved;
  const void*    col_global;
  const float*   val;
  const void*    y;
  const float*   offset;
  const float*   weight;
} gdmix_re_wire_batch;

typedef struct {
  int64_t E, N, Z, D;
  const int64_t* ent_row_ptr;
  int64_t*       ent_nnz_ptr;
  int64_t*       ent_feat_ptr;
  int32_t*       row_ptr;
  int32_t*       csr_col;
  float*         csr_val;
  int32_t*       col_ptr;
  int32_t*       csc_row;
  float*         csc_val;
  int32_t*       unique_global;
  const float*   y;
  const float*   offset;
  const float*   weight;
  int32_t*       order;
  int32_t*       cls_tmp;
  int32_t*       class_count;
  void*          scratch;
  size_t         scratch_bytes;
  int32_t        max_p, max_n, max_nnz;
} gdmix_re_packed;

#define GDMIX_RE_NUM_CLASSES 40

typedef struct {
  double  l2;
  int32_t regularize_bias;
  int32_t has_intercept;
  int32_t m;
  int32_t max_iter;
  int32_t maxfun;
  int32_t maxls;
  double  ftol;
  double  pgtol;
  int32_t variance_mode;
  double  threshold;
  int32_t sum_loss;
  int32_t loss;
} gdmix_re_opts;

#define GDMIX_RE_LOSS_LOGISTIC 0
#define GDMIX_RE_LOSS_SQUARED  1
#define GDMIX_RE_LOSS_POISSON  2

GDMIX_API void gdmix_re_default_opts(gdmix_re_opts* o);

typedef struct {
  double*  theta;
  double*  theta_thr;
  double*  variance;
  double*  fval;
  double*  gnorm;
  int32_t* nit;
  int32_t* nfev;
  int32_t* status;
} gdmix_re_result;

GDMIX_API int  gdmix_re_abi_version(void);
GDMIX_API const char* gdmix_re_build_id(void);
GDMIX_API const char* gdmix_re_last_error(void);

GDMIX_API int gdmix_re_device_shared(gdmix_re_ctx* ctx);
GDMIX_API int gdmix_re_grid_lock_acquire(const char* key);
GDMIX_API int gdmix_re_grid_lock_release(const char* key);
GDMIX_API int gdmix_re_grid_lock_stats(const char* key, int64_t* takes, int64_t* rides);

GDMIX_API int  gdmix_re_create(int hip_device, gdmix_re_ctx** out);
GDMIX_API void gdmix_re_destroy(gdmix_re_ctx* ctx);

GDMIX_API size_t gdmix_re_pack_workspace_bytes(int64_t E, int64_t N, int64_t Z);

GDMIX_API int gdmix_re_pack(gdmix_re_ctx* ctx, const gdmix_re_raw_batch* raw_dev, int has_intercept,
                  void* workspace, size_t workspace_bytes, gdmix_re_packed* out, void* stream);

GDMIX_API int gdmix_re_set_defer_unique(gdmix_re_ctx* ctx, int enabled);
GDMIX_API int gdmix_re_pack_join(gdmix_re_ctx* ctx, void* stream);

GDMIX_API size_t gdmix_re_widen_workspace_bytes(int64_t E, int64_t N, int64_t Z);
GDMIX_API int gdmix_re_widen(gdmix_re_ctx* ctx, const gdmix_re_wire_batch* wire_dev, void* workspace, size_t workspace_bytes,
                   gdmix_re_raw_batch* out, void* stream);

GDMIX_API int gdmix_re_solve(gdmix_re_ctx* ctx, const gdmix_re_packed* batch, const gdmix_re_opts* opts,
                   const double* theta0, const gdmix_re_result* out, void* stream);

GDMIX_API size_t gdmix_re_solve_scratch_bytes(const gdmix_re_packed* batch, const gdmix_re_opts* opts);
GDMIX_API int    gdmix_re_set_scratch(gdmix_re_ctx* ctx, void* scratch, size_t bytes);

GDMIX_API int gdmix_re_variance_full(gdmix_re_ctx* ctx, const gdmix_re_packed* batch, const gdmix_re_opts* opts, const double* theta,
                                     double* variance, void* stream);

GDMIX_API int gdmix_re_solve_l1(gdmix_re_ctx* ctx, const gdmix_re_packed* batch, const gdmix_re_opts* opts, double l1,
                                const double* theta0, const gdmix_re_result* out, void* stream);
GDMIX_API size_t gdmix_re_solve_l1_scratch_bytes(const gdmix_re_packed* batch, const gdmix_re_opts* opts);

GDMIX_API int gdmix_re_score(gdmix_re_ctx* ctx, const gdmix_re_packed* batch, int has_intercept,
                   const double* theta, const uint8_t* has_model,
                   float* logit, float* logit_per_coord, void* stream);

GDMIX_API int gdmix_re_set_wave_lds_limit(gdmix_re_ctx* ctx, int bytes);

GDMIX_API int gdmix_re_set_kernel_mask(gdmix_re_ctx* ctx, int mask);

GDMIX_API int gdmix_re_set_giant_nnz(gdmix_re_ctx* ctx, int64_t giant_nnz);
GDMIX_API int gdmix_re_set_team_nnz(gdmix_re_ctx* ctx, int64_t team_nnz);

#define GDMIX_RE_TALL_MIN_N_DEFAULT 32
GDMIX_API int gdmix_re_set_tall_min_n(gdmix_re_ctx* ctx, int min_n);
#define GDMIX_RE_TALL_SPLIT_N_DEFAULT 4096
GDMIX_API int gdmix_re_set_tall_split_n(gdmix_re_ctx* ctx, int split_n);
#define GDMIX_RE_TALL_TEAM_N_DEFAULT 8192
GDMIX_API int gdmix_re_set_tall_team_n(gdmix_re_ctx* ctx, int team_n);
GDMIX_API int gdmix_re_set_tall_mid_n(gdmix_re_ctx* ctx, int mid_n);

#define GDMIX_RE_NARROW_COUNT_WORD 15
GDMIX_API int gdmix_re_set_narrow(gdmix_re_ctx* ctx, int on);

GDMIX_API int gdmix_re_set_spread(gdmix_re_ctx* ctx, int queues);

GDMIX_API int gdmix_re_set_timing(gdmix_re_ctx* ctx, int enabled);
GDMIX_API int gdmix_re_last_solve_ms(gdmix_re_ctx* ctx, float* ms_out);

GDMIX_API const char* gdmix_re_class_kernel_name(int c);

typedef struct {
  uint64_t* two_u;
  int32_t*  n_pos;
  int32_t*  n_neg;
  int32_t*  n_nan;
  double*   sse;
  double*   auc;
} gdmix_re_eval_out;

typedef struct {
  uint64_t two_u;
  int64_t  n;
  int64_t  n_pos, n_neg, n_nan;
  double   sse;
} gdmix_re_eval_totals;

GDMIX_API size_t gdmix_re_eval_workspace_bytes(int64_t E, int64_t N);
GDMIX_API int gdmix_re_eval_entities(gdmix_re_ctx* ctx, const int64_t* ent_row_ptr, int64_t E, int64_t N, const float* score, const float* label,
                                     const gdmix_re_eval_out* out, void* workspace, size_t workspace_bytes, void* stream);
GDMIX_API int gdmix_re_set_eval_small_max(gdmix_re_ctx* ctx, int small_max);

#define GDMIX_RE_EVAL_ACC_STATE_BYTES 33024
typedef struct {
  uint64_t* keys;
  int64_t   capacity;
  int64_t   count;
  void*     state;
} gdmix_re_eval_acc;
GDMIX_API int gdmix_re_eval_acc_reset(gdmix_re_ctx* ctx, gdmix_re_eval_acc* acc, void* stream);
GDMIX_API int gdmix_re_eval_acc_add(gdmix_re_ctx* ctx, gdmix_re_eval_acc* acc, const float* score, const float* label, int64_t N, void* stream);
GDMIX_API size_t gdmix_re_eval_acc_workspace_bytes(int64_t N);
GDMIX_API int gdmix_re_eval_acc_finish(gdmix_re_ctx* ctx, const gdmix_re_eval_acc* acc, void* workspace, size_t workspace_bytes,
                                       gdmix_re_eval_totals* host_out, void* stream);

typedef struct {
  double*  pl;
  int32_t* n;
  int32_t* n_nan;
} gdmix_re_eval_pl_out;
typedef struct {
  double  pl;
  int64_t n;
  int64_t n_nan;
} gdmix_re_eval_pl_totals;
GDMIX_API int gdmix_re_eval_pl_entities(gdmix_re_ctx* ctx, const int64_t* ent_row_ptr, int64_t E, int64_t N, const float* score, const float* label,
                                        const gdmix_re_eval_pl_out* out, void* stream);
#define GDMIX_RE_EVAL_PL_STATE_BYTES 33024
typedef struct {
  void*   state;
  int64_t count;
} gdmix_re_eval_pl_acc;
GDMIX_API int gdmix_re_eval_pl_acc_reset(gdmix_re_ctx* ctx, gdmix_re_eval_pl_acc* acc, void* stream);
GDMIX_API int gdmix_re_eval_pl_acc_add(gdmix_re_ctx* ctx, gdmix_re_eval_pl_acc* acc, const float* score, const float* label, int64_t N, void* stream);
GDMIX_API int gdmix_re_eval_pl_acc_finish(gdmix_re_ctx* ctx, const gdmix_re_eval_pl_acc* acc, gdmix_re_eval_pl_totals* host_out, void* stream);

typedef struct {
  int32_t* hits_sure;
  int32_t* slots;
  int32_t* tie_pos;
  int32_t* tie_size;
} gdmix_re_eval_topk_out;
GDMIX_API size_t gdmix_re_eval_topk_workspace_bytes(int64_t E, int64_t N);
GDMIX_API int gdmix_re_eval_topk_entities(gdmix_re_ctx* ctx, const int64_t* ent_row_ptr, int64_t E, int64_t N, const float* score, const float* label,
                                          const int32_t* ks , int nk , const gdmix_re_eval_topk_out* out,
                                          const gdmix_re_eval_out* auc_out , void* workspace, size_t workspace_bytes, void* stream);

#define GDMIX_RE_EVAL_LL_TERM_EPS 1.5e-16
#define GDMIX_RE_EVAL_LL_STATE_BYTES GDMIX_RE_EVAL_PL_STATE_BYTES
typedef gdmix_re_eval_pl_out    gdmix_re_eval_ll_out;
typedef gdmix_re_eval_pl_totals gdmix_re_eval_ll_totals;
typedef gdmix_re_eval_pl_acc    gdmix_re_eval_ll_acc;
GDMIX_API int gdmix_re_eval_ll_entities(gdmix_re_ctx* ctx, const int64_t* ent_row_ptr, int64_t E, int64_t N, const float* score, const float* label,
                                        const gdmix_re_eval_ll_out* out, void* stream);
GDMIX_API int gdmix_re_eval_ll_acc_reset(gdmix_re_ctx* ctx, gdmix_re_eval_ll_acc* acc, void* stream);
GDMIX_API int gdmix_re_eval_ll_acc_add(gdmix_re_ctx* ctx, gdmix_re_eval_ll_acc* acc, const float* score, const float* label, int64_t N, void* stream);
GDMIX_API int gdmix_re_eval_ll_acc_finish(gdmix_re_ctx* ctx, const gdmix_re_eval_ll_acc* acc, gdmix_re_eval_ll_totals* host_out, void* stream);

#define GDMIX_RE_SWEEP_MODELS_PER_PASS 8
GDMIX_API int gdmix_re_join_features(gdmix_re_ctx* ctx, const gdmix_re_packed* eval, const gdmix_re_packed* train, int has_intercept,
                                     const int32_t* train_entity, int64_t* coef_pos, uint8_t* has_model, void* stream);
GDMIX_API size_t gdmix_re_score_models_workspace_bytes(int64_t P_train, int K);
GDMIX_API int gdmix_re_score_models(gdmix_re_ctx* ctx, const gdmix_re_packed* eval, int has_intercept, const double* const* thetas, int K,
                                    int64_t P_train, const int64_t* coef_pos, const uint8_t* has_model, float* logit, float* logit_per_coord,
                                    void* workspace, size_t workspace_bytes, void* stream);

GDMIX_API size_t gdmix_re_prior_workspace_bytes(const gdmix_re_packed* packed);
GDMIX_API int gdmix_re_prior_apply(gdmix_re_ctx* ctx, const gdmix_re_packed* packed, int has_intercept, const double* mean, const double* scale,
                                   void* workspace, size_t workspace_bytes, gdmix_re_packed* out, void* stream);
GDMIX_API int gdmix_re_prior_restore(gdmix_re_ctx* ctx, const gdmix_re_packed* packed, int has_intercept, const double* mean, const double* scale,
                                     double threshold, const double* phi, const double* var_phi, double* theta, double* theta_thr,
                                     double* variance, void* stream);

GDMIX_API int gdmix_re_feature_extent(gdmix_re_ctx* ctx, const void* col, int col_width, const float* val, int64_t Z, int64_t num_features,
                                      uint64_t* count, uint32_t* max_abs_bits, int64_t* bad, void* stream);
GDMIX_API int gdmix_re_feature_moments(gdmix_re_ctx* ctx, const void* col, int col_width, const float* val, int64_t Z, int64_t num_features,
                                       const int32_t* limb_bits, const int32_t* shift1, const int32_t* shift2, int64_t* limbs, int64_t* bad,
                                       void* stream);
GDMIX_API int gdmix_re_feature_scale_expand(gdmix_re_ctx* ctx, const gdmix_re_packed* packed, int has_intercept, const double* factor,
                                            int64_t num_features, double* scale, void* stream);

typedef struct {
  double   rate;
  uint64_t seed;
  int32_t  negatives_only;
  int32_t  reserved;
} gdmix_re_downsample_opts;
typedef struct {
  int64_t rows;
  int64_t kept;
  int64_t kept_nnz;
  int64_t positives;
  int64_t negatives_kept;
} gdmix_re_downsample_counts;
typedef struct {
  int64_t  N, Z;
  int64_t* ent_row_ptr;
  int64_t* row_nnz_ptr;
  int64_t* col_global;
  float*   val;
  float*   y;
  float*   offset;
  float*   weight;
} gdmix_re_downsample_out;
GDMIX_API size_t gdmix_re_downsample_workspace_bytes(int64_t E, int64_t N);
GDMIX_API int gdmix_re_downsample_plan(gdmix_re_ctx* ctx, const gdmix_re_raw_batch* raw_dev, const int64_t* uid_dev, const gdmix_re_downsample_opts* opts,
                                       void* workspace, size_t workspace_bytes, gdmix_re_downsample_counts* counts, void* stream);
GDMIX_API int gdmix_re_downsample_apply(gdmix_re_ctx* ctx, const gdmix_re_raw_batch* raw_dev, const gdmix_re_downsample_opts* opts, void* workspace,
                                        size_t workspace_bytes, const gdmix_re_downsample_out* out_dev, int32_t* kept_rows, void* stream);

typedef struct {
  int64_t entities;
  int64_t affected;
  int64_t features;
  int64_t kept;
  int64_t dropped;
  int64_t kept_nnz;
} gdmix_re_select_counts;
typedef struct {
  int64_t  Z;
  int64_t* row_nnz_ptr;
  int64_t* col_global;
  float*   val;
} gdmix_re_select_out;
GDMIX_API size_t gdmix_re_select_workspace_bytes(int64_t E, int64_t N, int64_t Z);
GDMIX_API int gdmix_re_select_plan(gdmix_re_ctx* ctx, const gdmix_re_packed* packed, double R, void* workspace, size_t workspace_bytes, float* keys_out,
// ... 60 lines not shown
```

Measured before the change: 128.3 million entities/s.

## Pre-route entities during pack and reuse cached route counts in solve

Adds an opt-in preroute mode that runs the classification/routing kernels at the end of pack and posts the class counts to a new mailbox, so solve can reuse a stored route record instead of rerunning routing and its host readback. Route records are validated by a signature and a global generation ledger. It also restructures pack's stats readbacks so they always use the mailbox, posts the tail stats earlier with an event-based fallback, and removes the separate stream-synchronising fetch on the no-side-stream path. Preroute is off by default, so the default path only sees the readback reordering. The packed struct also grows by a large route buffer.

```diff
diff --git a/gdmix_amd/csrc/re_api.hip b/gdmix_amd/csrc/re_api.hip
--- a/gdmix_amd/csrc/re_api.hip
+++ b/gdmix_amd/csrc/re_api.hip
@@ -55,8 +55,8 @@
 }
 
 hipError_t post_small(gdmix_ctx_impl* ctx, int box, const void* dev_src, size_t bytes, void* host_dst, hipStream_t s, SmallFetch* f) {
-  f->box = -1; f->seq = 0; f->bytes = bytes; f->host_dst = host_dst; f->s = s;
-  if (!mailbox_on() || bytes % 4 || bytes > MAILBOX_BYTES - MAILBOX_DATA || box < 0 || box >= 4)
+  f->box = -1; f->seq = 0; f->bytes = bytes; f->host_dst = host_dst; f->s = s; f->ev = nullptr;
+  if (!mailbox_on() || bytes % 4 || bytes > MAILBOX_BYTES - MAILBOX_DATA || box < 0 || box >= MAILBOXES)
     return hipMemcpyAsync(host_dst, dev_src, bytes, hipMemcpyDeviceToHost, s);
   char* const base = reinterpret_cast<char*>(ctx->host_pinned) + MAILBOX_OFFSET + (size_t)box * MAILBOX_BYTES;
   uint32_t seq = ++ctx->mail_seq[box];
@@ -68,7 +68,7 @@
 }
 
 hipError_t wait_small(gdmix_ctx_impl* ctx, const SmallFetch& f) {
-  if (f.box < 0) return hipStreamSynchronize(f.s);
+  if (f.box < 0) return f.ev ? hipEventSynchronize(f.ev) : hipStreamSynchronize(f.s);
   char* const base = reinterpret_cast<char*>(ctx->host_pinned) + MAILBOX_OFFSET + (size_t)f.box * MAILBOX_BYTES;
   uint32_t* const flag = reinterpret_cast<uint32_t*>(base);
   timespec t0, t1;
@@ -77,7 +77,7 @@
     for (int k = 0; k < 16; ++k) cpu_relax();
     clock_gettime(CLOCK_MONOTONIC, &t1);
     if ((t1.tv_sec - t0.tv_sec) * 1000000L + (t1.tv_nsec - t0.tv_nsec) / 1000L > FETCH_SPIN_US) {
-      hipError_t rc = hipStreamSynchronize(f.s);
+      hipError_t rc = f.ev ? hipEventSynchronize(f.ev) : hipStreamSynchronize(f.s);
       if (rc != hipSuccess) return rc;
       if (__atomic_load_n(flag, __ATOMIC_ACQUIRE) != f.seq) return hipErrorUnknown;
       break;
@@ -358,6 +358,10 @@
   c->impl.spread = spread_default();
   c->impl.narrow = 1;
   if (const char* e = getenv("GDMIX_RE_NARROW")) c->impl.narrow = atoi(e) != 0 ? 1 : 0;
+  c->impl.preroute = 0;
+  if (const char* e = getenv("GDMIX_RE_PREROUTE")) c->impl.preroute = atoi(e) != 0 ? 1 : 0;
+  c->impl.routes_run = c->impl.routes_reused = 0;
+  c->impl.preroute_gen = 0;
   c->impl.grid_sync = nullptr;
   c->impl.big_tmp = nullptr;
   c->impl.big_tmp_bytes = 0;
@@ -367,6 +371,7 @@
   c->impl.cap_small_set = 0; c->impl.cap_small_max = 128; c->impl.cap_plan_ws = nullptr;
   c->impl.n_side = 0; c->impl.side_fork = nullptr;
   c->impl.aux_ev[0] = c->impl.aux_ev[1] = nullptr;
+  c->impl.mail_ev = nullptr;
   c->impl.defer_unique = 0; c->impl.unique_pending = false; c->impl.unique_ev = nullptr;
   for (int k = 0; k < gdmix_ctx_impl::MAX_SIDE; ++k) { c->impl.side[k] = nullptr; c->impl.side_join[k] = nullptr; }
   for (int k = 0; k < GDMIX_RE_NUM_CLASSES; ++k) { c->impl.ev0[k] = nullptr; c->impl.ev1[k] = nullptr; c->impl.ev_used[k] = false; }
@@ -398,6 +403,12 @@
       }
     }
   }
+  rc = hipEventCreateWithFlags(&c->impl.mail_ev, hipEventDisableTiming);
+  if (rc != hipSuccess) {
+    set_error("hipEventCreateWithFlags failed: %s", hipGetErrorString(rc));
+    gdmix_re_destroy(c);
+    return GDMIX_RE_EHIP;
+  }
   rc = hipMalloc(&c->impl.grid_sync, GridSyncLayout::BYTES);
   if (rc != hipSuccess) {
     set_error("hipMalloc failed: %s", hipGetErrorString(rc));
@@ -418,6 +429,7 @@
   if (ctx->impl.eval_tmp) (void)hipFree(ctx->impl.eval_tmp);
   if (ctx->impl.host_pinned) (void)hipHostFree(ctx->impl.host_pinned);
   if (ctx->impl.side_fork) (void)hipEventDestroy(ctx->impl.side_fork);
+  if (ctx->impl.mail_ev) (void)hipEventDestroy(ctx->impl.mail_ev);
   for (int k = 0; k < 2; ++k) if (ctx->impl.aux_ev[k]) (void)hipEventDestroy(ctx->impl.aux_ev[k]);
   for (int k = 0; k < gdmix_ctx_impl::MAX_SIDE; ++k) {
     if (ctx->impl.side_join[k]) (void)hipEventDestroy(ctx->impl.side_join[k]);
@@ -538,6 +550,19 @@
 GDMIX_API int gdmix_re_set_narrow(gdmix_re_ctx* ctx, int on) {
   if (!ctx) { set_error("ctx is NULL"); return GDMIX_RE_EINVAL; }
   ctx->impl.narrow = on ? 1 : 0;
+  return GDMIX_RE_OK;
+}
+
+GDMIX_API int gdmix_re_set_preroute(gdmix_re_ctx* ctx, int on) {
+  if (!ctx) { set_error("ctx is NULL"); return GDMIX_RE_EINVAL; }
+  ctx->impl.preroute = on ? 1 : 0;
+  return GDMIX_RE_OK;
+}
+
+GDMIX_API int gdmix_re_route_counts(gdmix_re_ctx* ctx, int64_t* routed, int64_t* reused) {
+  if (!ctx || !routed || !reused) { set_error("NULL argument"); return GDMIX_RE_EINVAL; }
+  *routed = ctx->impl.routes_run;
+  *reused = ctx->impl.routes_reused;
   return GDMIX_RE_OK;
 }
 
diff --git a/gdmix_amd/csrc/re_internal.hpp b/gdmix_amd/csrc/re_internal.hpp
--- a/gdmix_amd/csrc/re_internal.hpp
+++ b/gdmix_amd/csrc/re_internal.hpp
@@ -235,13 +235,27 @@
   int32_t* status;
 };
 
+constexpr size_t HOST_PINNED_BYTES = 16384;
+constexpr size_t MAILBOX_OFFSET = 4096, MAILBOX_BYTES = 1024, MAILBOX_DATA = 64;
+constexpr int MAILBOXES = 5, PREROUTE_BOX = 4;
+constexpr int FETCH_SPIN_US = 400;
+constexpr size_t COUNTS_READBACK_WORDS = 256;
+constexpr size_t PREROUTE_READBACK_WORDS = 512;
+static_assert(sizeof(ClassCounts) <= MAILBOX_BYTES - MAILBOX_DATA, "a larger count record falls back to copy + synchronise in post_small");
+static_assert(COUNTS_READBACK_WORDS * sizeof(int32_t) + sizeof(ClassCounts) <= PREROUTE_READBACK_WORDS * sizeof(int32_t) &&
+              PREROUTE_READBACK_WORDS * sizeof(int32_t) + sizeof(ClassCounts) <= MAILBOX_OFFSET, "the read-back areas end where the mailboxes begin");
+static_assert(MAILBOX_OFFSET + MAILBOXES * MAILBOX_BYTES <= HOST_PINNED_BYTES, "the mailboxes end inside the pinned buffer");
+struct SmallFetch { int box; uint32_t seq; size_t bytes; void* host_dst; hipStream_t s; hipEvent_t ev; };
+
 struct gdmix_ctx_impl {
   int device;
   int num_cus;
   void* scratch;
   size_t scratch_bytes;
   int32_t* host_pinned;
-  uint32_t mail_seq[4];
+  uint32_t mail_seq[MAILBOXES];
+  SmallFetch preroute_fetch;
+  uint64_t preroute_gen;
   int wave_lds_limit;
   int kernel_mask;
   int timing;
@@ -256,6 +270,8 @@
   int tall_mid_n;
   int narrow;
   int spread;
+  int preroute;
+  int64_t routes_run, routes_reused;
   void* grid_sync;
   void* big_tmp;
   size_t big_tmp_bytes;
@@ -264,6 +280,7 @@
   int n_side;
   hipEvent_t side_fork, side_join[MAX_SIDE];
   hipEvent_t aux_ev[2];
+  hipEvent_t mail_ev;
   int defer_unique;
   bool unique_pending;
   hipEvent_t unique_ev;
@@ -282,13 +299,6 @@
   int64_t cap_plan_rows, cap_plan_entities, cap_plan_bound, cap_plan_kept, cap_plan_nnz;
 };
 
-constexpr size_t HOST_PINNED_BYTES = 8192;
-constexpr size_t MAILBOX_OFFSET = 4096, MAILBOX_BYTES = 1024, MAILBOX_DATA = 64;
-constexpr int FETCH_SPIN_US = 400;
-constexpr size_t COUNTS_READBACK_WORDS = 256;
-static_assert(sizeof(ClassCounts) <= MAILBOX_BYTES - MAILBOX_DATA, "a larger count record falls back to copy + synchronise in post_small");
-static_assert(COUNTS_READBACK_WORDS * sizeof(int32_t) + sizeof(ClassCounts) <= MAILBOX_OFFSET, "the read-back areas end where the mailboxes begin");
-struct SmallFetch { int box; uint32_t seq; size_t bytes; void* host_dst; hipStream_t s; };
 hipError_t post_small(gdmix_ctx_impl* ctx, int box, const void* dev_src, size_t bytes, void* host_dst, hipStream_t s, SmallFetch* f);
 hipError_t wait_small(gdmix_ctx_impl* ctx, const SmallFetch& f);
 inline hipError_t fetch_small(gdmix_ctx_impl* ctx, int box, const void* dev_src, size_t bytes, void* host_dst, hipStream_t s) {
@@ -336,6 +346,24 @@
 
 int make_class_table(const gdmix_ctx_impl* ci, const gdmix_re_opts* opts, ClassTable* out);
 int route(gdmix_ctx_impl* ci, const gdmix_re_packed* b, const ClassTable& tab, const gdmix_re_opts* opts, hipStream_t s, const ClassCounts** host);
+struct RouteSig {
+  ClassTable tab;
+  int32_t has_intercept, m, has_w, kernel_mask, num_cus, spread;
+  int32_t base_args[5];
+  int32_t pad;
+  int64_t E;
+  const void* arrays[6];
+};
+struct RouteRecord { RouteSig sig; ClassCounts counts; };
+static_assert(sizeof(RouteRecord) <= GDMIX_RE_ROUTE_WORDS * sizeof(uint64_t) && alignof(RouteRecord) <= alignof(uint64_t), "gdmix_re_packed::route holds a RouteRecord");
+void route_signature(const gdmix_ctx_impl* ci, const gdmix_re_packed* b, int has_intercept, int m, const ClassTable& tab, RouteSig* out);
+hipError_t launch_routing(const gdmix_ctx_impl* ci, const gdmix_re_packed* b, int ic, int m, const ClassTable& tab, hipStream_t s, bool zeroed = false);
+uint64_t route_ledger_stamp(const void* class_count);
+bool route_ledger_current(const void* class_count, uint64_t gen);
+enum { ROUTE_NONE = 0, ROUTE_STORED = 1, ROUTE_PENDING = 2 };
+void route_store(gdmix_re_packed* b, const RouteSig& sig, const ClassCounts& counts, uint64_t gen);
+void route_store_pending(gdmix_re_packed* b, const RouteSig& sig, uint64_t gen);
+inline void route_clear(gdmix_re_packed* b) { b->route_valid = 0; b->route_gen = 0; }
 struct Launch { int c, begin, count, stream, narrow; };
 struct LaunchPlan {
   Launch launch[GDMIX_RE_NUM_CLASSES];
diff --git a/gdmix_amd/csrc/re_owlqn.hip b/gdmix_amd/csrc/re_owlqn.hip
--- a/gdmix_amd/csrc/re_owlqn.hip
+++ b/gdmix_amd/csrc/re_owlqn.hip
@@ -249,6 +249,8 @@
 
   const int ic = opts->has_intercept ? 1 : 0;
   int32_t* const counts = b->class_count;
+  route_clear(const_cast<gdmix_re_packed*>(b));
+  (void)route_ledger_stamp(b->class_count);
   const int small_lds = ci->wave_lds_limit < OWL_SMALL_LDS ? ci->wave_lds_limit : OWL_SMALL_LDS;
   HIP_TRY(hipMemsetAsync(counts, 0, sizeof(ClassCounts), s));
   hipLaunchKernelGGL(re_owlqn_route_kernel, dim3(grid_for(b->E, 256, 2048)), dim3(256), 0, s, b->ent_row_ptr, b->ent_nnz_ptr, b->ent_feat_ptr, b->E, ic,
diff --git a/gdmix_amd/csrc/re_pack.hip b/gdmix_amd/csrc/re_pack.hip
--- a/gdmix_amd/csrc/re_pack.hip
+++ b/gdmix_amd/csrc/re_pack.hip
@@ -721,6 +721,8 @@
   out->scratch = base + L.sort_key;
   out->scratch_bytes = (size_t)(Z + 1) * 8;
   out->max_p = ic; out->max_n = 0; out->max_nnz = 0;
+  route_clear(out);
+  (void)route_ledger_stamp(out->class_count);
   if (E == 0) return GDMIX_RE_OK;
 
   int32_t* d_cnt = reinterpret_cast<int32_t*>(base + L.d_cnt);
@@ -729,6 +731,7 @@
   unsigned long long* sort_key = reinterpret_cast<unsigned long long*>(base + L.sort_key);
 
   HIP_TRY(hipMemsetAsync(stats, 0, sizeof(PackStats), s));
+  if (ctx->preroute) HIP_TRY(hipMemsetAsync(out->class_count, 0, sizeof(ClassCounts), s));
   int32_t* uniq_sparse = reinterpret_cast<int32_t*>(base + L.uniq_sparse);
   int32_t* big_list = reinterpret_cast<int32_t*>(base + L.big_list);
   int32_t* mid_list = reinterpret_cast<int32_t*>(base + L.mid_list);
@@ -751,6 +754,8 @@
     HIP_TRY(post_small(ctx, 3, stats, sizeof(PackStats), hs, s, &counts));
     HIP_TRY(hipEventRecord(ctx->side_fork, s));
     HIP_TRY(side_join.use(0));
+  } else {
+    HIP_TRY(post_small(ctx, 3, stats, sizeof(PackStats), hs, s, &counts));
   }
   static int pack_occupancy = 0;
   if (pack_occupancy == 0) {
@@ -765,8 +770,8 @@
                      raw->row_nnz_ptr, out->ent_nnz_ptr, raw->col_global, raw->val, E, ic, out->row_ptr, sort_key,
                      out->csr_col, out->col_ptr, out->csc_row, out->csc_val, uniq_sparse, d_cnt, stats, pack_bitmap_on());
   DBG_STAGE("pack_entity_kernel<256>");
-  if (ns >= 1) HIP_TRY(wait_small(ctx, counts));
-  if (ns == 0 || hs->n_mid > 0) {
+  HIP_TRY(wait_small(ctx, counts));
+  if (hs->n_mid > 0) {
     if (ns >= 2) HIP_TRY(side_join.use(1));
     hipLaunchKernelGGL((pack_entity_kernel<PACK_CAP2, 4>), dim3(ctx->num_cus * 4), dim3(WAVE * 4), 0, s2,
                        (const int32_t*)mid_list, (const int*)&stats->n_mid, raw->ent_row_ptr,
@@ -774,7 +779,7 @@
                        out->csr_col, out->col_ptr, out->csc_row, out->csc_val, uniq_sparse, d_cnt, stats, pack_bitmap_on());
   }
   DBG_STAGE("pack_entity_kernel<512>");
-  if (ns == 0 || hs->n_mid2 > 0) {
+  if (hs->n_mid2 > 0) {
     if (ns >= 2) HIP_TRY(side_join.use(ns >= 3 ? 2 : 1));
     hipLaunchKernelGGL((pack_entity_kernel<PACK_CAP3, 2>), dim3(ctx->num_cus * 4), dim3(WAVE * 2), 0, s3,
                        (const int32_t*)mid2_list, (const int*)&stats->n_mid2, raw->ent_row_ptr,
@@ -783,7 +788,6 @@
   }
   DBG_STAGE("pack_entity_kernel<1024>");
   {
-    if (ns == 0) HIP_TRY(fetch_small(ctx, 1, stats, sizeof(PackStats), hs, s));
     if (hs->n_big > 0) {
       BigPackArgs A{raw->ent_row_ptr, out->ent_nnz_ptr, raw->row_nnz_ptr, raw->col_global, raw->val, ic, out->row_ptr, out->csr_col,
                     out->col_ptr, out->csc_row, out->csc_val, uniq_sparse, d_cnt, big_list, hs->n_big,
@@ -795,19 +799,20 @@
   side_join.join();
   DBG_STAGE("pack_big_entities");
   const int nb = (int)((E + SCAN_CHUNK - 1) / SCAN_CHUNK);
-  hipLaunchKernelGGL(scan_reduce_kernel, dim3(nb), dim3(256), 0, s, d_cnt, E, block_sums);
-  hipLaunchKernelGGL(scan_blocksums_kernel, dim3(1), dim3(1024), 0, s, block_sums, nb, stats);
-  hipLaunchKernelGGL(scan_apply_kernel, dim3(nb), dim3(256), 0, s, d_cnt, E, block_sums, out->ent_feat_ptr);
-  DBG_STAGE("scan kernels");
   const bool defer = ctx->defer_unique && ctx->n_side > 0;
   hipStream_t const sc = defer ? ctx->side[ctx->n_side - 1] : s;
   SmallFetch tail_fetch;
-  if (defer) {
-    HIP_TRY(post_small(ctx, 1, stats, sizeof(PackStats), hs, s, &tail_fetch));
-    HIP_TRY(hipEventRecord(ctx->side_fork, s));
-    HIP_TRY(hipStreamWaitEvent(sc, ctx->side_fork, 0));
-  }
-  {
+  const auto post_stats = [&]() -> hipError_t {
+    hipError_t rc = post_small(ctx, 1, stats, sizeof(PackStats), hs, s, &tail_fetch);
+    if (rc == hipSuccess && ctx->mail_ev) { rc = hipEventRecord(ctx->mail_ev, s); tail_fetch.ev = ctx->mail_ev; }
+    return rc;
+  };
+  hipLaunchKernelGGL(scan_reduce_kernel, dim3(nb), dim3(256), 0, s, d_cnt, E, block_sums);
+  hipLaunchKernelGGL(scan_blocksums_kernel, dim3(1), dim3(1024), 0, s, block_sums, nb, stats);
+  if (defer) HIP_TRY(post_stats());
+  hipLaunchKernelGGL(scan_apply_kernel, dim3(nb), dim3(256), 0, s, d_cnt, E, block_sums, out->ent_feat_ptr);
+  DBG_STAGE("scan kernels");
+  const auto compact = [&]() -> hipError_t {
     static int defer_wgs = 0;
     if (defer_wgs == 0) { const char* e = getenv("GDMIX_RE_DEFER_WGS"); defer_wgs = (e && atoi(e) > 0) ? atoi(e) : 4; }
     const int per_cu = defer ? defer_wgs : 16;
@@ -815,17 +820,43 @@
     if (grid > ctx->num_cus * per_cu) grid = ctx->num_cus * per_cu;
     hipLaunchKernelGGL(pack_compact_unique_kernel, dim3(grid), dim3(256), 0, sc, out->ent_nnz_ptr, out->ent_feat_ptr, E,
                        uniq_sparse, out->unique_global);
-  }
-  DBG_STAGE("pack_compact_unique_kernel");
-  HIP_TRY(hipGetLastError());
+    return hipGetLastError();
+  };
   if (defer) {
+    HIP_TRY(hipEventRecord(ctx->side_fork, s));
+    HIP_TRY(hipStreamWaitEvent(sc, ctx->side_fork, 0));
+  } else {
+    HIP_TRY(compact());
+    DBG_STAGE("pack_compact_unique_kernel");
+    HIP_TRY(post_stats());
+  }
+  ctx->preroute_gen = 0;
+  if (ctx->preroute) {
+    ClassTable tab;
+    gdmix_re_opts ro;
+    gdmix_re_default_opts(&ro);
+    ro.has_intercept = ic;
+    if (make_class_table(ctx, &ro, &tab) == GDMIX_RE_OK) {
+      RouteSig sig;
+      route_signature(ctx, out, ic, ro.m, tab, &sig);
+      const uint64_t gen = route_ledger_stamp(out->class_count);
+      HIP_TRY(launch_routing(ctx, out, ic, ro.m, tab, s, true));
+      HIP_TRY(post_small(ctx, PREROUTE_BOX, out->class_count, sizeof(ClassCounts), ctx->host_pinned + PREROUTE_READBACK_WORDS, s, &ctx->preroute_fetch));
+      route_store_pending(out, sig, gen);
+      ctx->preroute_gen = gen;
+    }
+  }
+  DBG_STAGE("routing kernels");
+  if (defer) {
+    HIP_TRY(compact());
+    DBG_STAGE("pack_compact_unique_kernel");
     HIP_TRY(hipEventRecord(ctx->unique_ev, sc));
     ctx->unique_pending = true;
-    HIP_TRY(wait_small(ctx, tail_fetch));
-  } else {
-    HIP_TRY(fetch_small(ctx, 1, stats, sizeof(PackStats), hs, s));
-  }
+  }
+  HIP_TRY(wait_small(ctx, tail_fetch));
   if (hs->err) {
+    route_clear(out);
+    ctx->preroute_gen = 0;
     if (defer) HIP_TRY(join_unique(ctx, s));
     set_error("pack: an entity exceeds a per-entity int32 limit or a feature index is outside [0, 2^31)");
     return hs->err;
diff --git a/gdmix_amd/csrc/re_prior.hip b/gdmix_amd/csrc/re_prior.hip
--- a/gdmix_amd/csrc/re_prior.hip
+++ b/gdmix_amd/csrc/re_prior.hip
@@ -189,6 +189,7 @@
   result.csr_val = csr_out;
   result.csc_val = csc_out;
   result.offset = off_out;
+  route_clear(&result);
   if (E > 0 && N > 0) {
     HIP_TRY(hipSetDevice(ctx->impl.device));
     hipStream_t s = static_cast<hipStream_t>(stream);
diff --git a/gdmix_amd/csrc/re_route.hip b/gdmix_amd/csrc/re_route.hip
--- a/gdmix_amd/csrc/re_route.hip
+++ b/gdmix_amd/csrc/re_route.hip
@@ -1,4 +1,7 @@
 #include <stdlib.h>
+#include <string.h>
+
+#include <mutex>
 
 #include "re_internal.hpp"
 #include "re_solve_team.hpp"
@@ -210,16 +213,106 @@
   return hipGetLastError();
 }
 
+hipError_t launch_routing(const gdmix_ctx_impl* ci, const gdmix_re_packed* b, int ic, int m, const ClassTable& tab, hipStream_t s, bool zeroed) {
+  ClassCounts* const cc = reinterpret_cast<ClassCounts*>(b->class_count);
+  hipError_t rc = zeroed ? hipSuccess : hipMemsetAsync(cc, 0, sizeof(ClassCounts), s);
+  if (rc != hipSuccess) return rc;
+  rc = launch_classify(b, ic, m, tab, cc, s);
+  if (rc != hipSuccess) return rc;
+  hipLaunchKernelGGL(class_base_kernel, dim3(1), dim3(1), 0, s, cc, tab.tall_adapt_limit, 16 * ci->num_cus, tab.tall_team_n, tab.tall_team_limit, tab.tall_mid_n);
+  rc = hipGetLastError();
+  if (rc != hipSuccess) return rc;
+  return launch_order(b, cc, s);
+}
+
+void route_signature(const gdmix_ctx_impl* ci, const gdmix_re_packed* b, int has_intercept, int m, const ClassTable& tab, RouteSig* out) {
+  memset(out, 0, sizeof(RouteSig));
+  ClassTable& t = out->tab;
+  memcpy(t.kind, tab.kind, sizeof(t.kind)); memcpy(t.lds_bytes, tab.lds_bytes, sizeof(t.lds_bytes));
+  memcpy(t.ncap, tab.ncap, sizeof(t.ncap)); memcpy(t.zcap, tab.zcap, sizeof(t.zcap));
+  t.giant_nnz = tab.giant_nnz; t.team_nnz = tab.team_nnz; t.tall_min_n = tab.tall_min_n; t.tall_split_n = tab.tall_split_n;
+  t.tall_adapt_limit = tab.tall_adapt_limit; t.tall_team_n = tab.tall_team_n; t.tall_team_limit = tab.tall_team_limit;
+  t.narrow = tab.narrow; t.tall_mid_n = tab.tall_mid_n;
+  out->has_intercept = has_intercept ? 1 : 0; out->m = m; out->has_w = b->weight != nullptr ? 1 : 0;
+  out->kernel_mask = ci->kernel_mask; out->num_cus = ci->num_cus; out->spread = ci->spread;
+  const int32_t base_args[5] = {tab.tall_adapt_limit, 16 * ci->num_cus, tab.tall_team_n, tab.tall_team_limit, tab.tall_mid_n};
+  memcpy(out->base_args, base_args, sizeof(base_args));
+  out->E = b->E;
+  const void* const arrays[6] = {b->ent_row_ptr, b->ent_nnz_ptr, b->ent_feat_ptr, b->order, b->cls_tmp, b->class_count};
+  memcpy(out->arrays, arrays, sizeof(arrays));
+}
+
+namespace {
+constexpr int LEDGER_SLOTS = 256;
+struct LedgerSlot { const void* cc; uint64_t gen; };
+std::mutex g_ledger_mu;
+LedgerSlot g_ledger[LEDGER_SLOTS] = {};
+uint64_t g_ledger_gen = 0;
+inline int ledger_slot(const void* cc) { return (int)(((uintptr_t)cc >> 8) * 0x9E3779B97F4A7C15ull >> 56) % LEDGER_SLOTS; }
+}
+
+uint64_t route_ledger_stamp(const void* class_count) {
+  std::lock_guard<std::mutex> g(g_ledger_mu);
+  LedgerSlot& L = g_ledger[ledger_slot(class_count)];
+  L.cc = class_count;
+  L.gen = ++g_ledger_gen;
+  return L.gen;
+}
+
+bool route_ledger_current(const void* class_count, uint64_t gen) {
+  std::lock_guard<std::mutex> g(g_ledger_mu);
+  const LedgerSlot& L = g_ledger[ledger_slot(class_count)];
+  return gen != 0 && L.cc == class_count && L.gen == gen;
+}
+
+void route_store(gdmix_re_packed* b, const RouteSig& sig, const ClassCounts& counts, uint64_t gen) {
+  RouteRecord* const r = reinterpret_cast<RouteRecord*>(b->route);
+  memcpy(&r->sig, &sig, sizeof(RouteSig));
+  memcpy(&r->counts, &counts, sizeof(ClassCounts));
+  b->route_gen = gen;
+  b->route_valid = ROUTE_STORED;
+}
+
+void route_store_pending(gdmix_re_packed* b, const RouteSig& sig, uint64_t gen) {
+  RouteRecord* const r = reinterpret_cast<RouteRecord*>(b->route);
+  memcpy(&r->sig, &sig, sizeof(RouteSig));
+  memset(&r->counts, 0, sizeof(ClassCounts));
+  b->route_gen = gen;
+  b->route_valid = ROUTE_PENDING;
+}
+
 int route(gdmix_ctx_impl* ci, const gdmix_re_packed* b, const ClassTable& tab, const gdmix_re_opts* opts, hipStream_t s,
           const ClassCounts** host) {
+  gdmix_re_packed* const mb = const_cast<gdmix_re_packed*>(b);
+  RouteSig sig;
+  route_signature(ci, b, opts->has_intercept, opts->m, tab, &sig);
+  if (ci->preroute && (b->route_valid == ROUTE_STORED || b->route_valid == ROUTE_PENDING)) {
+    RouteRecord* const r = reinterpret_cast<RouteRecord*>(mb->route);
+    if (memcmp(&r->sig, &sig, sizeof(RouteSig)) == 0 && route_ledger_current(b->class_count, b->route_gen)) {
+      bool have = b->route_valid == ROUTE_STORED;
+      if (!have && ci->preroute_gen == b->route_gen) {
+        HIP_TRY(wait_small(ci, ci->preroute_fetch));
+        memcpy(&r->counts, ci->host_pinned + PREROUTE_READBACK_WORDS, sizeof(ClassCounts));
+        ci->preroute_gen = 0;
+        mb->route_valid = ROUTE_STORED;
+        have = true;
+      }
+      if (have) {
+        ++ci->routes_reused;
+        *host = &r->counts;
+        return GDMIX_RE_OK;
+      }
+    }
+  }
+  if (b->route_gen != 0 && ci->preroute_gen == b->route_gen) ci->preroute_gen = 0;
+  route_clear(mb);
+  const uint64_t gen = route_ledger_stamp(b->class_count);
+  ++ci->routes_run;
+  HIP_TRY(launch_routing(ci, b, opts->has_intercept ? 1 : 0, opts->m, tab, s));
   ClassCounts* const cc = reinterpret_cast<ClassCounts*>(b->class_count);
-  HIP_TRY(hipMemsetAsync(cc, 0, sizeof(ClassCounts), s));
-  HIP_TRY(launch_classify(b, opts->has_intercept ? 1 : 0, opts->m, tab, cc, s));
-  hipLaunchKernelGGL(class_base_kernel, dim3(1), dim3(1), 0, s, cc, tab.tall_adapt_limit, 16 * ci->num_cus, tab.tall_team_n, tab.tall_team_limit, tab.tall_mid_n);
-  HIP_TRY(hipGetLastError());
-  HIP_TRY(launch_order(b, cc, s));
   ClassCounts* const hc = reinterpret_cast<ClassCounts*>(ci->host_pinned + COUNTS_READBACK_WORDS);
   HIP_TRY(fetch_small(ci, 0, cc, sizeof(ClassCounts), hc, s));
+  if (ci->preroute) route_store(mb, sig, *hc, gen);
   *host = hc;
   return GDMIX_RE_OK;
 }
diff --git a/gdmix_amd/solver.py b/gdmix_amd/solver.py
--- a/gdmix_amd/solver.py
+++ b/gdmix_amd/solver.py
@@ -43,7 +43,8 @@
                 ("unique_global", C.c_void_p), ("y", C.c_void_p), ("offset", C.c_void_p), ("weight", C.c_void_p),
                 ("order", C.c_void_p), ("cls_tmp", C.c_void_p), ("class_count", C.c_void_p),
                 ("scratch", C.c_void_p), ("scratch_bytes", C.c_size_t),
-                ("max_p", C.c_int32), ("max_n", C.c_int32), ("max_nnz", C.c_int32)]
+                ("max_p", C.c_int32), ("max_n", C.c_int32), ("max_nnz", C.c_int32),
+                ("route_valid", C.c_int32), ("route_gen", C.c_uint64), ("route", C.c_uint64 * 224)]
 
 
 class _Opts(C.Structure):
@@ -144,7 +145,7 @@
     "gdmix_re_destroy", "gdmix_re_pack_workspace_bytes", "gdmix_re_pack", "gdmix_re_set_defer_unique", "gdmix_re_pack_join", "gdmix_re_solve",
     "gdmix_re_solve_l1", "gdmix_re_solve_l1_scratch_bytes",
     "gdmix_re_solve_scratch_bytes", "gdmix_re_set_scratch", "gdmix_re_variance_full", "gdmix_re_set_wave_lds_limit", "gdmix_re_score",
-    "gdmix_re_widen_workspace_bytes", "gdmix_re_widen", "gdmix_re_set_timing", "gdmix_re_last_solve_ms", "gdmix_re_set_kernel_mask", "gdmix_re_set_giant_nnz", "gdmix_re_set_team_nnz", "gdmix_re_set_tall_min_n", "gdmix_re_set_tall_split_n", "gdmix_re_set_tall_team_n", "gdmix_re_set_tall_mid_n", "gdmix_re_set_spread", "gdmix_re_set_narrow",
+    "gdmix_re_widen_workspace_bytes", "gdmix_re_widen", "gdmix_re_set_timing", "gdmix_re_last_solve_ms", "gdmix_re_set_kernel_mask", "gdmix_re_set_giant_nnz", "gdmix_re_set_team_nnz", "gdmix_re_set_tall_min_n", "gdmix_re_set_tall_split_n", "gdmix_re_set_tall_team_n", "gdmix_re_set_tall_mid_n", "gdmix_re_set_spread", "gdmix_re_set_narrow", "gdmix_re_set_preroute", "gdmix_re_route_counts",
     "gdmix_fe_create", "gdmix_fe_destroy", "gdmix_fe_eval", "gdmix_fe_reduce_buffer", "gdmix_fe_step", "gdmix_fe_step_async", "gdmix_fe_step_status", "gdmix_fe_solve", "gdmix_fe_result",
     "gdmix_fe_last_eval_ms", "gdmix_fe_stream_bytes", "gdmix_fe_score", "gdmix_fe_hessian_diag", "gdmix_fe_hessian_dense_scratch_bytes", "gdmix_fe_hessian_dense", "gdmix_fe_hessian_dense_loss",
     "gdmix_fe_variance_of_hessian", "gdmix_fe_restart", "gdmix_fe_set_prior", "gdmix_fe_set_l1", "gdmix_fe_set_optimizer", "gdmix_fe_set_bounds", "gdmix_fe_products", "gdmix_fe_hessian_vec", "gdmix_fe_score_models_workspace_bytes", "gdmix_fe_score_models",
@@ -259,6 +260,8 @@
     lib.gdmix_re_set_tall_mid_n.argtypes = [C.c_void_p, C.c_int]
     lib.gdmix_re_set_spread.argtypes = [C.c_void_p, C.c_int]
     lib.gdmix_re_set_narrow.argtypes = [C.c_void_p, C.c_int]
+    lib.gdmix_re_set_preroute.argtypes = [C.c_void_p, C.c_int]
+    lib.gdmix_re_route_counts.argtypes = [C.c_void_p, C.POINTER(C.c_int64), C.POINTER(C.c_int64)]
     lib.gdmix_re_set_timing.argtypes = [C.c_void_p, C.c_int]
     lib.gdmix_re_last_solve_ms.argtypes = [C.c_void_p, C.POINTER(C.c_float)]
     lib.gdmix_re_score.argtypes = [C.c_void_p, C.POINTER(_Packed), C.c_int, C.c_void_p, C.c_void_p,
@@ -625,6 +628,14 @@
     def set_narrow(self, on: bool):
         _check(self.lib.gdmix_re_set_narrow(self._h, int(bool(on))), "set_narrow")
 
+    def set_preroute(self, on: bool):
+        _check(self.lib.gdmix_re_set_preroute(self._h, int(bool(on))), "set_preroute")
+
+    def route_counts(self):
+        routed, reused = C.c_int64(), C.c_int64()
+        _check(self.lib.gdmix_re_route_counts(self._h, C.byref(routed), C.byref(reused)), "route_counts")
+        return int(routed.value), int(reused.value)
+
     NARROW_COUNT_WORD = 15
 
     def narrow_count(self, packed: PackedBatch) -> int:
diff --git a/include/gdmix_re.h b/include/gdmix_re.h
--- a/include/gdmix_re.h
+++ b/include/gdmix_re.h
@@ -62,6 +62,7 @@
   const float*   weight;
 } gdmix_re_wire_batch;
 
+#define GDMIX_RE_ROUTE_WORDS 224
 typedef struct {
   int64_t E, N, Z, D;
   const int64_t* ent_row_ptr;
@@ -83,6 +84,9 @@
   void*          scratch;
   size_t         scratch_bytes;
   int32_t        max_p, max_n, max_nnz;
+  int32_t        route_valid;
+  uint64_t       route_gen;
+  uint64_t       route[GDMIX_RE_ROUTE_WORDS];
 } gdmix_re_packed;
 
 #define GDMIX_RE_NUM_CLASSES 40
@@ -178,6 +182,9 @@
 
 #define GDMIX_RE_NARROW_COUNT_WORD 15
 GDMIX_API int gdmix_re_set_narrow(gdmix_re_ctx* ctx, int on);
+
+GDMIX_API int gdmix_re_set_preroute(gdmix_re_ctx* ctx, int on);
+GDMIX_API int gdmix_re_route_counts(gdmix_re_ctx* ctx, int64_t* routed, int64_t* reused);
 
 GDMIX_API int gdmix_re_set_spread(gdmix_re_ctx* ctx, int queues);
 
```

New measurement: 128.6 million entities/s (median of 6 runs). Within noise of the previous version (+0.2%).
